# XiYe20/NPVP

Measured on AMD Instinct MI355X. Metric: predictor train frames/sec, higher is better.
Workload: dtype f32 (two-term fp16 split of amax-scaled operands, 3 MFMAs per product, fp32 accumulate: fp32-grade; small GEMMs: three-term bf16 split)

## Files before the change

include/npvp_hip.h:

```cpp
#ifndef NPVP_HIP_H
#define NPVP_HIP_H
#include <stddef.h>
#ifdef __cplusplus
extern "C" {
#endif

typedef struct ihipStream_t* npvp_stream_t;

int npvp_version(void);
const char* npvp_last_error(void);
long long npvp_launch_count(void);
void* npvp_stream_create_low_priority(int* least, int* greatest);
int npvp_stream_destroy(void* stream);
void* npvp_event_create(void);
int npvp_event_record(void* event, void* stream);
float npvp_event_elapsed_ms(void* event0, void* event1);
int npvp_event_destroy(void* event);

long long npvp_graph_node_counts(void* graph, long long* counts, long long* memset_bytes, int max_memsets);

long long npvp_gemm_workspace_bytes(int M, int N, int K);
int npvp_gemm_kernel_id(int a_kc, int b_kc, int M, int N, int K, int precision, int has_planes);
int npvp_gemm_route(int a_kc, int b_kc, int M, int N, int K, int precision, int has_planes, int plain_epilogue, int* out4);
int npvp_gemm_f32(int a_kc, int b_kc, int M, int N, int K, const float* A, long long lda, const float* B, long long ldb,
                  float* C, long long ldc, const float* bias, int act, const float* aux_in, float* aux_out,
                  const float* residual, long long ldr, float drop_p, int drop_mode, int drop_g1, int drop_g2,
                  const unsigned long long* seed, unsigned int salt, float alpha, int precision, float* colsum_a,
                  const void* b_pre, int accumulate, float* rowstats, const float* a_amax, const float* b_amax,
                  float* c_amax, unsigned int* range_flag, float adrop_p, int adrop_g1, int adrop_g2, unsigned int adrop_salt,
                  void* workspace, long long ws_bytes, npvp_stream_t stream);
int npvp_gemm_f32_skip(int a_kc, int b_kc, int M, int N, int K, const float* A, long long lda, const float* B, long long ldb,
                       float* C, long long ldc, const float* bias, int act, const float* aux_in, float* aux_out,
                       const float* residual, long long ldr, float drop_p, int drop_mode, int drop_g1, int drop_g2,
                       const unsigned long long* seed, unsigned int salt, float alpha, int precision, float* colsum_a,
                       const void* b_pre, int accumulate, float* rowstats, const float* a_amax, const float* b_amax,
                       float* c_amax, unsigned int* range_flag, float adrop_p, int adrop_g1, int adrop_g2, unsigned int adrop_salt,
                       float skip_p, int skip_g1, int skip_g2, unsigned int skip_salt, void* workspace, long long ws_bytes,
                       npvp_stream_t stream);
int npvp_frame_stats_finalize(const float* part, int parts_per_frame, float values_per_part, float* mean, float* rstd,
                              int frames, float eps, npvp_stream_t stream);
int npvp_split_weight(const float* w, long long ld, int N, int K, void* F, void* D, npvp_stream_t stream);
int npvp_split_weights_batched(const void* desc, int count, npvp_stream_t stream);
int npvp_amax(const float* x, long long rows, long long cols, long long ld, float* slot, npvp_stream_t stream);

typedef struct npvp_reduce_job {
  const float* ws; float* out; long long ldc; int M, N, splits, accum; float alpha; int blocks; const float* cs_part; float* cs_out;
} npvp_reduce_job_t;
int npvp_wgrad_f16_chainable(int M, int N, int K);
long long npvp_wgrad_f16_chain_workspace_bytes(int M, int N, int K);
int npvp_wgrad_f16_chained(int M, int N, int K, const float* dy, long long lda, const float* x, long long ldb, float* dw,
                           long long ldc, float* db, int accumulate, const float* a_amax, const float* b_amax,
                           unsigned int* range_flag, float adrop_p, int adrop_g1, int adrop_g2, unsigned int adrop_salt,
                           const unsigned long long* seed, const void* prev_job, void* my_job, void* workspace,
                           long long ws_bytes, npvp_stream_t stream);
int npvp_splitk_reduce_job(const void* job, npvp_stream_t stream);
int npvp_splitk_reduce_multi(const void* jobs, int n, npvp_stream_t stream);
int npvp_linear_bwd_f16_takes(int R, int N, int K);
int npvp_linear_bwd_f16(int R, int N, int K, const float* dy, long long ldy, const float* dy_amax, const void* w_planes_d,
                        const float* w_amax, float* dx, long long ldx, int act, const float* aux_in, const float* residual,
                        long long ldr, float drop_p, int drop_mode, int drop_g1, int drop_g2, unsigned int drop_salt, float* dx_amax,
                        const float* x, long long ldxx, const float* x_amax, float* dw, long long ldw, float* db,
                        unsigned int* range_flag, float adrop_p, int adrop_g1, int adrop_g2, unsigned int adrop_salt,
                        const unsigned long long* seed, const void* prev_job, void* my_job, void* workspace, long long ws_bytes,
                        npvp_stream_t stream);
int npvp_linear_bwd_f16_skip(int R, int N, int K, const float* dy, long long ldy, const float* dy_amax, const void* w_planes_d,
                             const float* w_amax, float* dx, long long ldx, int act, const float* aux_in, const float* residual,
                             long long ldr, float drop_p, int drop_mode, int drop_g1, int drop_g2, unsigned int drop_salt,
                             float* dx_amax, const float* x, long long ldxx, const float* x_amax, float* dw, long long ldw, float* db,
                             unsigned int* range_flag, float adrop_p, int adrop_g1, int adrop_g2, unsigned int adrop_salt,
                             float skip_p, int skip_g1, int skip_g2, unsigned int skip_salt, const unsigned long long* seed,
                             const void* prev_job, void* my_job, void* workspace, long long ws_bytes, npvp_stream_t stream);
int npvp_split_weight_f16(const float* w, long long ld, int N, int K, void* F, void* D, float* amax_slot, npvp_stream_t stream);
int npvp_split_weights_f16(const void* desc, int count, void* amax_table, long long amax_bytes, npvp_stream_t stream);

int npvp_layernorm_fwd(const float* x, const float* w, const float* b, float* y, float* mean, float* rstd, long long rows,
                       int C, float eps, int relu, float* y_amax, npvp_stream_t stream);
long long npvp_layernorm_bwd_workspace_bytes(long long rows, int C);
int npvp_layernorm_bwd(const float* dy, const float* x, const float* w, const float* b, const float* mean,
                       const float* rstd, float* dx, float* dw, float* db, long long rows, int C, int relu,
                       const float* dres ,
                       int accumulate , float* dx_amax,
                       void* workspace, long long ws_bytes, npvp_stream_t stream);
int npvp_layernorm_bwd_reduce(const void* workspace, float* dw, float* db, long long rows, int C, int accumulate,
                              npvp_stream_t stream);

int npvp_layernorm_bwd_reduce_job(const void* workspace, float* dw, float* db, long long rows, int C, int accumulate, void* job);
int npvp_frameln_act_bwd_reduce_job(const void* workspace, float* dw, float* db, int frames, int per_frame, int accumulate, void* job);
int npvp_mlpdw_mid_bwd_reduce_job(const void* workspace, float* gw, float* gb, int frames, int Ch, void* job);
int npvp_sum_rows_multi(const void* jobs, int n, npvp_stream_t stream);

int npvp_layernorm_nchw_fwd(const float* x, const float* w, const float* b, float* out_nchw, float* mean, float* rstd, int frames,
                            int P, int C, float eps, int relu, npvp_stream_t stream);

int npvp_frame_stats(const float* x, const float* add, float* mean, float* rstd, int frames, int T, int per_frame,
                     float eps, npvp_stream_t stream);
int npvp_posfuse_fwd(const float* x, const float* add, const float* beta, const float* gamma, float* y, float* mean,
                     float* rstd, int N, int T, int per_frame, float eps, float* y_amax, npvp_stream_t stream);
int npvp_ln_posfuse_fwd(const float* x, const float* lw, const float* lb, float ln_eps, float* y1, float* ln_mean, float* ln_rstd,
                        const float* add, const float* beta, const float* gamma, float* fused, float* pf_mean, float* pf_rstd,
                        int N, int T, int P, int C, float pf_eps, float* y1_amax, float* fused_amax, npvp_stream_t stream);
int npvp_posfuse_bwd_fused(int N, int T, int per_frame);
int npvp_posfuse_bwd(const float* dy, const float* x, const float* add, const float* gamma, const float* mean,
                     const float* rstd, float* du, float* dyxh, float* dbeta, float* dgamma, int N, int T, int per_frame,
                     int accumulate, void* workspace, long long ws_bytes , npvp_stream_t stream);

int npvp_posfuse_instance_fwd(const float* x, const float* add, const float* beta, const float* gamma, float* y, float* mean,
                              float* rstd, int N, int T, int P, int C, float eps, float* y_amax, npvp_stream_t stream);
int npvp_posfuse_instance_bwd(const float* dy, const float* x, const float* add, const float* gamma, const float* mean,
                              const float* rstd, float* du, float* dyxh, int N, int T, int P, int C, npvp_stream_t stream);

int npvp_frameln_act_fwd(const float* h, const float* mean, const float* rstd, const float* w, const float* b,
                         const float* res, float* out, int frames, int per_frame, float drop_p, unsigned int salt,
                         float dp_p, unsigned int dp_salt, int frames_per_sample, const unsigned long long* seed,
                         float* out_amax, npvp_stream_t stream);
long long npvp_frameln_act_bwd_workspace_bytes(int frames, int per_frame);
int npvp_frameln_act_bwd(const float* dout, const float* h, const float* mean, const float* rstd, const float* w,
                         const float* b, float* dh, float* dw, float* db, int frames, int per_frame, float drop_p,
                         unsigned int salt, float dp_p, unsigned int dp_salt, int frames_per_sample,
                         const unsigned long long* seed, int accumulate ,
                         float* dh_amax, void* workspace, long long ws_bytes, npvp_stream_t stream);
int npvp_frameln_act_bwd_reduce(const void* workspace, float* dw, float* db, int frames, int per_frame, int accumulate,
                                npvp_stream_t stream);
int npvp_dwconv3x3(const float* a, const float* wt, const float* bias, float* out, int frames, int H, int W, int Ch,
                   int flip, npvp_stream_t stream);
int npvp_dwconv3x3_stats(const float* a, const float* wt, const float* bias, float* out, float* mean, float* rstd, int frames,
                         int H, int W, int Ch, float eps, void* workspace, long long ws_bytes, npvp_stream_t stream);
int npvp_mlpdw_mid_fwd(const float* h1, const float* mean1, const float* rstd1, const float* w1n, const float* b1n,
                       const float* wt, const float* bias, float* h2, float* mean2, float* rstd2, int frames, int H, int W,
                       int Ch, float eps, void* workspace, long long ws_bytes, npvp_stream_t stream);
int npvp_mlpdw_mid_fwd_parts(const float* h1, const float* part1, int J1, float nb1, float* mean1, float* rstd1, const float* w1n,
                             const float* b1n, const float* wt, const float* bias, float* h2, float* part2, int frames, int H,
                             int W, int Ch, float eps, npvp_stream_t stream);
int npvp_frameln_act_fwd_parts(const float* h, const float* part, int J, float nb, float eps, float* mean, float* rstd,
                               const float* w, const float* b, const float* res, float* out, int frames, int per_frame,
                               float drop_p, unsigned int salt, float dp_p, unsigned int dp_salt, int frames_per_sample,
                               const unsigned long long* seed, float* out_amax, npvp_stream_t stream);
long long npvp_mlpdw_mid_bwd_workspace_bytes(int frames, int Ch);
int npvp_mlpdw_mid_bwd(const float* dh2, const float* h1, const float* mean1, const float* rstd1, const float* w1n,
                       const float* b1n, const float* wt, float* da1, float* dwt_db, float* psum, int frames, int H, int W,
                       int Ch, int accumulate, void* workspace, long long ws_bytes, npvp_stream_t stream);
int npvp_mlpdw_mid_bwd_reduce(const void* workspace, float* dwt_db, int frames, int Ch, int accumulate, npvp_stream_t stream);
int npvp_mlpdw_mid_bwd_reduce_into(const void* workspace, float* gw, float* gb, int frames, int Ch, npvp_stream_t stream);
int npvp_mlpdw_mid_bwd_n2(const float* da2, const float* h2, const float* mean2, const float* rstd2, const float* w2n,
                          const float* b2n, const float* psum2, int nparts2, float drop_p, unsigned int salt,
                          const unsigned long long* seed, const float* h1, const float* mean1, const float* rstd1,
                          const float* w1n, const float* b1n, const float* wt, float* da1, float* dwt_db, float* psum, int frames,
                          int H, int W, int Ch, int accumulate, void* workspace, long long ws_bytes, npvp_stream_t stream);
int npvp_frameln_act_bwd_pgrad(const float* dout, const float* h, const float* mean, const float* rstd, const float* w,
                               const float* b, float* psum, float* dw, float* db, int frames, int per_frame, float drop_p,
                               unsigned int salt, float dp_p, unsigned int dp_salt, int frames_per_sample,
                               const unsigned long long* seed, int accumulate, void* workspace, long long ws_bytes,
                               npvp_stream_t stream);
int npvp_frameln_act_bwd_apply(const float* dout, const float* h, const float* mean, const float* rstd, const float* w,
                               const float* b, const float* psum, int nparts, float* dh, float* dw, float* db, int frames,
                               int per_frame, int accumulate, float* dh_amax, void* workspace, long long ws_bytes,
                               npvp_stream_t stream);
int npvp_mlpdw_mid_fwd_parts_skip(const float* h1, const float* part1, int J1, float nb1, float* mean1, float* rstd1,
                                  const float* w1n, const float* b1n, const float* wt, const float* bias, float* h2, float* part2,
                                  int frames, int H, int W, int Ch, float eps, float skip_p, unsigned int skip_salt, int skip_fps,
                                  const unsigned long long* seed, npvp_stream_t stream);
int npvp_frameln_act_fwd_parts_skip(const float* h, const float* part, int J, float nb, float eps, float* mean, float* rstd,
                                    const float* w, const float* b, const float* res, float* out, int frames, int per_frame,
                                    float drop_p, unsigned int salt, float dp_p, unsigned int dp_salt, int frames_per_sample,
                                    const unsigned long long* seed, float* out_amax, float skip_p, unsigned int skip_salt,
                                    int skip_fps, npvp_stream_t stream);
int npvp_frameln_act_bwd_apply_skip(const float* dout, const float* h, const float* mean, const float* rstd, const float* w,
                                    const float* b, const float* psum, int nparts, float* dh, float* dw, float* db, int frames,
                                    int per_frame, int accumulate, float* dh_amax, void* workspace, long long ws_bytes,
                                    float skip_p, unsigned int skip_salt, int skip_fps, const unsigned long long* seed,
                                    npvp_stream_t stream);

int npvp_im2col3x3(const float* in, float* out, int frames, int H, int W, int C, int col2im, npvp_stream_t stream);
long long npvp_dwconv3x3_wgrad_workspace_bytes(int frames, int Ch);
int npvp_dwconv3x3_wgrad(const float* a, const float* dout, float* dwt_db, int frames, int H, int W, int Ch,
                         void* workspace, long long ws_bytes, npvp_stream_t stream);

int npvp_attn_fwd(const float* q, long long ld_q, const float* k, long long ld_k, const float* v, long long ld_v, float* o,
                  long long ld_o, int mode, int dim0, int P, int W, int ws, int Tq, int Tk, int heads, int head_dim,
                  int mask_mode, float drop_p, const unsigned long long* seed, unsigned int salt, float* o_amax,
                  npvp_stream_t stream);
int npvp_attn_bwd(const float* q, long long ld_q, const float* k, long long ld_k, const float* v, long long ld_v,
                  const float* go, long long ld_o, float* dq, long long ld_dq, float* dk, long long ld_dk, float* dv,
                  long long ld_dv, int mode, int dim0, int P, int W, int ws, int Tq, int Tk, int heads, int head_dim,
                  int mask_mode, float drop_p, const unsigned long long* seed, unsigned int salt, float* dq_amax,
                  float* dk_amax , float* dv_amax,
                  npvp_stream_t stream);
int npvp_attn_long_fwd(const float* q, long long ld_q, const float* k, long long ld_k, const float* v, long long ld_v, float* o,
                       long long ld_o, int mode, int dim0, int P, int W, int ws, int Tq, int Tk, int heads, int head_dim,
                       int mask_mode, float drop_p, const unsigned long long* seed, unsigned int salt, float* o_amax,
                       npvp_stream_t stream);
long long npvp_attn_long_bwd_workspace_bytes(int mode, int dim0, int P, int W, int ws, int Tq, int Tk, int heads);
int npvp_attn_long_bwd(const float* q, long long ld_q, const float* k, long long ld_k, const float* v, long long ld_v,
                       const float* go, long long ld_o, float* dq, long long ld_dq, float* dk, long long ld_dk, float* dv,
                       long long ld_dv, int mode, int dim0, int P, int W, int ws, int Tq, int Tk, int heads, int head_dim,
                       int mask_mode, float drop_p, const unsigned long long* seed, unsigned int salt, float* dq_amax,
                       float* dk_amax , float* dv_amax, void* workspace, long long ws_bytes,
                       npvp_stream_t stream);

int npvp_reparam_samples(const float* mu, const float* logvar, float* z, float* eps_out, long long numel, int S,
                         long long sample_base, const unsigned long long* seed, unsigned int salt, npvp_stream_t stream);
int npvp_attn_samples_fwd(const float* q, long long ld_q, const float* k, long long ld_k, const float* v, long long ld_v, float* o,
                          long long ld_o, int S, int N, int P, int Tq, int Tk, int heads, int head_dim, int sample_chunk,
                          float* o_amax, npvp_stream_t stream);

int npvp_drop_apply(const float* x, float* out, long long rows, int ncols, float p, int mode, int g1, int g2,
                    const unsigned long long* seed, unsigned int salt, float* out_amax, npvp_stream_t stream);
int npvp_transpose(const float* in, float* out, int batch, int R, int C, npvp_stream_t stream);
int npvp_dwtb_accumulate(const float* dwtb, float* gw, float* gb, int C, npvp_stream_t stream);
int npvp_dwtb_build(const float* w, const float* b, float* wtb, int C, npvp_stream_t stream);
int npvp_reduce_mid(const float* in, float* out, int A, int B, long long Cc, float scale, int accumulate, npvp_stream_t stream);
int npvp_broadcast_mid(const float* in, float* out, int A, int B, long long Cc, float scale, npvp_stream_t stream);
int npvp_grid_center_pad(const float* src, long long ld_src, float* dst, long long ld_dst, int F, int H, int W, int Hp, int Wp, int top,
                         int left, int C, long long rows_out, float* dst_amax, npvp_stream_t stream);
int npvp_grid_center_cut(const float* src, long long ld_src, const float* addend, long long ld_add, float* dst, long long ld_dst, int F,
                         int H, int W, int Hp, int Wp, int top, int left, int C, float* dst_amax, npvp_stream_t stream);

long long npvp_colsum_workspace_bytes(long long rows, int N);
int npvp_colsum(const float* x, long long rows, int N, long long ld, float* out, int accumulate ,
                void* workspace, long long ws_bytes, npvp_stream_t stream);

int npvp_l1_mean(const float* a, const float* b, long long n, float lam, float* out, void* workspace, long long ws_bytes,
                 npvp_stream_t stream);
int npvp_l1_mean_bwd(const float* a, const float* b, long long n, const float* gout, float lam, float* da, npvp_stream_t stream);
int npvp_sum_all(const float* x, long long n, float* out, void* workspace, long long ws_bytes, npvp_stream_t stream);
// ... 65 lines not shown
```

npvp_amd/csrc/gemm.h:

```cpp
#pragma once
#include <type_traits>
#include "common.h"

namespace npvp {

typedef float f32x16 __attribute__((ext_vector_type(16)));
typedef __bf16 bf16x8 __attribute__((ext_vector_type(8)));
typedef __bf16 bf16x4 __attribute__((ext_vector_type(4)));

struct ReduceJob {
  const float* ws; float* out; long long ldc; int M, N, splits, accum; float alpha; int blocks; const float* cs_part; float* cs_out;
};

struct GemmParams {
  const float* A; const float* B; float* C;
  const float* bias;
  const float* residual;
  float* aux_out;
  const float* aux_in;
  float* rowstats;
  float* colsum;
  const unsigned long long* seed;
  long long lda, ldb, ldc, ldr;
  int M, N, K;
  int act;
  DropSpec drop;
  DropSpec adrop;
  DropSpec rskip;
  int tiles_m, tiles_n;
  int splits;
  float alpha;
  const void* b_pre;
  long long b_pre_plane;
  int colgroups;
  int accum;
  const float* a_amax; const float* b_amax; float* c_amax;
  unsigned int* range_flag;
  ReduceJob prev;
};

__device__ __forceinline__ void splitk_reduce_body(const ReduceJob& j, int bid, int nblocks, float& cmax) {
  const long long total4 = (long long)j.M * j.N / 4, cs4 = j.cs_out ? j.M / 4 : 0;
  for (long long i = (long long)bid * 256 + threadIdx.x; i < total4 + cs4; i += (long long)nblocks * 256) {
    if (i >= total4) {
      const long long e = (i - total4) * 4;
      float4 s = make_float4(0.f, 0.f, 0.f, 0.f);
      for (int zz = 0; zz < j.splits; ++zz) {
        const float4 v = ld4(j.cs_part + (long long)zz * j.M + e);
        s.x += v.x; s.y += v.y; s.z += v.z; s.w += v.w;
      }
      if (j.accum) { const float4 o = ld4(j.cs_out + e); s.x += o.x; s.y += o.y; s.z += o.z; s.w += o.w; }
      st4(j.cs_out + e, s);
      continue;
    }
    const long long e = i * 4;
    const int m = (int)(e / j.N), n = (int)(e - (long long)m * j.N);
    float4 s = make_float4(0.f, 0.f, 0.f, 0.f);
    for (int zz = 0; zz < j.splits; ++zz) {
      const float4 v = ld4(j.ws + (long long)zz * j.M * j.N + e);
      s.x += v.x; s.y += v.y; s.z += v.z; s.w += v.w;
    }
    s.x *= j.alpha; s.y *= j.alpha; s.z *= j.alpha; s.w *= j.alpha;
    if (j.accum) { const float4 o = ld4(j.out + (long long)m * j.ldc + n); s.x += o.x; s.y += o.y; s.z += o.z; s.w += o.w; }
    st4(j.out + (long long)m * j.ldc + n, s);
    cmax = amax4(cmax, s);
  }
}

__device__ __forceinline__ void store_colsum(const GemmParams& p, long long idx, float v) {
  p.colsum[idx] = (p.accum && p.splits == 1) ? p.colsum[idx] + v : v;
}

constexpr int EPI_LD = 36;
constexpr int EPI_FLOATS = 32 * EPI_LD;

__device__ __forceinline__ void epi_transpose(const f32x16& acc, float* scr, int lane, float4 (&v)[4]) {
  const int r = lane & 31, h = lane >> 5;
#pragma unroll
  for (int g = 0; g < 16; ++g) scr[(((g & 3) + 8 * (g >> 2)) + 4 * h) * EPI_LD + r] = acc[g];
  const int rr = lane >> 3, cq = lane & 7;
#pragma unroll
  for (int k = 0; k < 4; ++k) v[k] = *reinterpret_cast<const float4*>(scr + (rr + 8 * k) * EPI_LD + 4 * cq);
}

__device__ __forceinline__ float4 f4_mad(const float4& a, float s, const float4& b) {
  return make_float4(a.x * s + b.x, a.y * s + b.y, a.z * s + b.z, a.w * s + b.w);
}
__device__ __forceinline__ void f4_add(float4& a, const float4& b) { a.x += b.x; a.y += b.y; a.z += b.z; a.w += b.w; }

template <int I, int N, class F>
__device__ __forceinline__ void static_for(F&& f) {
  if constexpr (I < N) {
    f(std::integral_constant<int, I>{});
    static_for<I + 1, N>(f);
  }
}

__device__ __forceinline__ float4 epilogue_row_scales(const GemmParams& p, unsigned long long seed, int row0, int lane) {
  float4 sc = make_float4(1.f, 1.f, 1.f, 1.f);
  if (p.drop.thresh && p.drop.mode != 0) {
    const int r = row0 + (lane >> 3);
    sc.x = drop_spec_scale(p.drop, seed, r, 0, 1); sc.y = drop_spec_scale(p.drop, seed, r + 8, 0, 1);
    sc.z = drop_spec_scale(p.drop, seed, r + 16, 0, 1); sc.w = drop_spec_scale(p.drop, seed, r + 24, 0, 1);
  }
  return sc;
}

template <bool CHECK>
__device__ __forceinline__ void epilogue_rows(const GemmParams& p, float4 (&v)[4], int row0, int col0, int lane, int z,
                                              unsigned long long seed, float& cmax, float4 rowsc, float alpha) {
  const int rb = row0 + (lane >> 3), col = col0 + 4 * (lane & 7);
  if (CHECK && col >= p.N) return;
#define NPVP_ROW(k) (rb + 8 * (k))
#define NPVP_INB(k) (!CHECK || NPVP_ROW(k) < p.M)
  float* cp = p.C + (p.splits > 1 ? (long long)z * p.M * p.ldc : 0ll) + col;
  const long long ld = p.ldc;
  if (p.splits > 1) {
#pragma unroll
    for (int k = 0; k < 4; ++k) if (NPVP_INB(k)) st4(cp + NPVP_ROW(k) * ld, v[k]);
    return;
  }
  const float4 bv = p.bias ? ld4(p.bias + col) : make_float4(0.f, 0.f, 0.f, 0.f);
#pragma unroll
  for (int k = 0; k < 4; ++k) v[k] = f4_mad(v[k], alpha, bv);
  if (p.aux_out) {
#pragma unroll
    for (int k = 0; k < 4; ++k) if (NPVP_INB(k)) st4(p.aux_out + NPVP_ROW(k) * ld + col, v[k]);
  }
  if (p.act == 1) {
#pragma unroll
    for (int k = 0; k < 4; ++k) v[k] = make_float4(gelu_f(v[k].x), gelu_f(v[k].y), gelu_f(v[k].z), gelu_f(v[k].w));
  } else if (p.act == 2) {
#pragma unroll
    for (int k = 0; k < 4; ++k) v[k] = make_float4(fmaxf(v[k].x, 0.f), fmaxf(v[k].y, 0.f), fmaxf(v[k].z, 0.f), fmaxf(v[k].w, 0.f));
  } else if (p.act == 3 || p.act == 4) {
    float4 u[4];
#pragma unroll
    for (int k = 0; k < 4; ++k) u[k] = NPVP_INB(k) ? ld4(p.aux_in + NPVP_ROW(k) * ld + col) : make_float4(0.f, 0.f, 0.f, 0.f);
    if (p.act == 3) {
#pragma unroll
      for (int k = 0; k < 4; ++k) {
        v[k].x *= gelu_grad_f(u[k].x); v[k].y *= gelu_grad_f(u[k].y); v[k].z *= gelu_grad_f(u[k].z); v[k].w *= gelu_grad_f(u[k].w);
      }
    } else {
#pragma unroll
      for (int k = 0; k < 4; ++k) {
        v[k].x = u[k].x > 0.f ? v[k].x : 0.f; v[k].y = u[k].y > 0.f ? v[k].y : 0.f;
        v[k].z = u[k].z > 0.f ? v[k].z : 0.f; v[k].w = u[k].w > 0.f ? v[k].w : 0.f;
      }
    }
  }
  if (p.drop.thresh) {
    if (p.drop.mode == 0) {
#pragma unroll
      for (int k = 0; k < 4; ++k) {
        const unsigned long long key = (unsigned long long)NPVP_ROW(k) * (unsigned long long)p.N + (unsigned long long)col;
        v[k].x *= drop_scale(seed, p.drop.salt, key + 0, p.drop.thresh, p.drop.inv_keep);
        v[k].y *= drop_scale(seed, p.drop.salt, key + 1, p.drop.thresh, p.drop.inv_keep);
        v[k].z *= drop_scale(seed, p.drop.salt, key + 2, p.drop.thresh, p.drop.inv_keep);
        v[k].w *= drop_scale(seed, p.drop.salt, key + 3, p.drop.thresh, p.drop.inv_keep);
      }
    } else {
#pragma unroll
      for (int k = 0; k < 4; ++k) {
        const float f = k == 0 ? rowsc.x : k == 1 ? rowsc.y : k == 2 ? rowsc.z : rowsc.w;
        v[k].x *= f; v[k].y *= f; v[k].z *= f; v[k].w *= f;
      }
    }
  }
  if (p.residual) {
#pragma unroll
    for (int k = 0; k < 4; ++k) if (NPVP_INB(k)) f4_add(v[k], ld4(p.residual + NPVP_ROW(k) * p.ldr + col));
  }
  if (p.accum) {
#pragma unroll
    for (int k = 0; k < 4; ++k) if (NPVP_INB(k)) f4_add(v[k], ld4(cp + NPVP_ROW(k) * ld));
  }
#pragma unroll
  for (int k = 0; k < 4; ++k) if (NPVP_INB(k)) st4(cp + NPVP_ROW(k) * ld, v[k]);
  if (p.c_amax) {
#pragma unroll
    for (int k = 0; k < 4; ++k) if (NPVP_INB(k)) cmax = amax4(cmax, v[k]);
  }
#undef NPVP_INB
#undef NPVP_ROW
}

__device__ __forceinline__ void epilogue_rows_bias(const GemmParams& p, float4 (&v)[4], int row0, int col0, int lane, float& cmax, float alpha) {
  const int col = col0 + 4 * (lane & 7);
  float* cp = p.C + (long long)(row0 + (lane >> 3)) * p.ldc + col;
  const long long ld8 = 8 * p.ldc;
  const float4 bv = p.bias ? ld4(p.bias + col) : make_float4(0.f, 0.f, 0.f, 0.f);
#pragma unroll
  for (int k = 0; k < 4; ++k) {
    const float4 x = f4_mad(v[k], alpha, bv);
    st4(cp + k * ld8, x);
    if (p.c_amax) cmax = amax4(cmax, x);
  }
}

__device__ __forceinline__ void epilogue_tile(const GemmParams& p, const f32x16& acc, int row0, int col0, int lane, float* scr, int z,
                                              unsigned long long seed, float& cmax, float4 rowsc, float alpha) {
  if (row0 >= p.M || col0 >= p.N) return;
  float4 v[4];
  epi_transpose(acc, scr, lane, v);
  const bool inside = row0 + 32 <= p.M && col0 + 32 <= p.N;
  const bool simple = p.splits == 1 && !p.aux_out && p.act == 0 && !p.drop.thresh && !p.residual && !p.accum;
  if (simple && inside) epilogue_rows_bias(p, v, row0, col0, lane, cmax, alpha);
  else if (inside) epilogue_rows<false>(p, v, row0, col0, lane, z, seed, cmax, rowsc, alpha);
  else epilogue_rows<true>(p, v, row0, col0, lane, z, seed, cmax, rowsc, alpha);
}

__device__ __forceinline__ void epilogue_rowstats_block(const GemmParams& p, const f32x16& a00, const f32x16& a01,
                                                        const f32x16& a10, const f32x16& a11, int row0, int col0, int lane,
                                                        float* scr, float& cmax, float alpha) {
  if (row0 >= p.M || col0 >= p.N) return;
  const int r = lane & 31;
  float shift = 0.f, s1 = 0.f, s2 = 0.f;
#pragma unroll
  for (int tm = 0; tm < 2; ++tm) {
#pragma unroll
    for (int tn = 0; tn < 2; ++tn) {
      const f32x16& acc = tm == 0 ? (tn == 0 ? a00 : a01) : (tn == 0 ? a10 : a11);
      const float bv = p.bias ? p.bias[col0 + tn * 32 + r] : 0.f;
#pragma unroll
      for (int g = 0; g < 16; ++g) {
        const float v = acc[g] * alpha + bv;
        if (tm == 0 && tn == 0 && g == 0) shift = v;
        const float d = v - shift;
        s1 += d; s2 += d * d;
      }
    }
  }
  __builtin_amdgcn_sched_barrier(0);
#pragma unroll
  for (int tm = 0; tm < 2; ++tm) {
#pragma unroll
    for (int tn = 0; tn < 2; ++tn) {
      const f32x16& acc = tm == 0 ? (tn == 0 ? a00 : a01) : (tn == 0 ? a10 : a11);
      float4 v[4];
      epi_transpose(acc, scr, lane, v);
      epilogue_rows_bias(p, v, row0 + tm * 32, col0 + tn * 32, lane, cmax, alpha);
      __builtin_amdgcn_sched_barrier(0);
    }
  }
  const float n = 64.f, m1 = s1 / n, mean_l = shift + m1, m2_l = s2 - s1 * m1;
  const float mean_w = wave_sum(mean_l) * (1.f / 64.f);
  const float dl = mean_l - mean_w;
  const float m2_w = wave_sum(m2_l + n * dl * dl);
  if ((lane & 63) == 0) {
    const long long frame = row0 >> 6;
    const int cb = col0 >> 6, ncb = p.N >> 6;
    p.rowstats[(frame * ncb + cb) * 2] = mean_w;
    p.rowstats[(frame * ncb + cb) * 2 + 1] = m2_w;
  }
}

__device__ __forceinline__ void tile_of_block_unsplit(const GemmParams& p, const int nwg, const int bid, int& tile_m, int& tile_n) {
  const int xcd = bid & 7, loc = bid >> 3;
  if (p.colgroups > 1) {
    const int G = p.colgroups, tn_g = p.tiles_n / G, tm_g = p.tiles_m / (8 / G);
    const int lm = loc / tn_g;
    tile_m = (xcd / G) * tm_g + lm;
    tile_n = (xcd % G) * tn_g + (loc - lm * tn_g);
  } else {
    const int q = nwg >> 3, rr = nwg & 7;
    const int nid = (xcd < rr ? xcd * (q + 1) : rr * (q + 1) + (xcd - rr) * q) + loc;
    tile_m = nid / p.tiles_n;
    tile_n = nid - tile_m * p.tiles_n;
  }
}

__device__ __forceinline__ void tile_of_block_unsplit(const GemmParams& p, int& tile_m, int& tile_n) {
  tile_of_block_unsplit(p, (int)gridDim.x, (int)blockIdx.x, tile_m, tile_n);
}

inline int pick_colgroups(long long b_bytes, int tiles_m, int tiles_n) {
  for (int G = 1; G <= 8; G *= 2) {
    if (b_bytes / G > (2ll << 20)) continue;
    if (G > 1 && (tiles_n % G == 0) && (tiles_m % (8 / G) == 0) && ((tiles_m * tiles_n) % 8 == 0)) return G;
    break;
  }
  return 1;
}

inline long long splitk_workspace_bytes(int splits, int M, int N) {
  return ((long long)splits * M * N + (long long)splits * M) * 4;
}

inline void aim_at_workspace(GemmParams& p, int K, int splits, void* workspace, bool colsum) {
  p.K = K / splits; p.C = (float*)workspace; p.ldc = p.N;
  p.colsum = colsum ? (float*)workspace + (long long)splits * p.M * p.N : nullptr;
}

inline int wgrad_splits(int M, int N, int K, int min_rows) {
  if ((K & 15) || M < 64 || N < 128 || K < min_rows) return 0;
  const int tiles = ((M + 127) / 128) * ((N + 255) / 256);
  int s = (512 + tiles - 1) / tiles;
  const int maxs = K / 256;
  if (s > maxs) s = maxs;
  if (s > 64) s = 64;
  if (s >= 8) s &= ~7;
  while (s > 1 && (K % (s * 16)) != 0) --s;
  return s < 1 ? 1 : s;
}
inline int wide_wgrad_splits(int M, int N, int K) { return wgrad_splits(M, N, K, 32768); }
inline int f16_wgrad_splits(int M, int N, int K) { return wgrad_splits(M, N, K, 1024); }

inline bool adrop_args_ok(float p, int g1, int g2, const unsigned long long* seed, bool rows16) {
  return p >= 0.f && p < 0.5f && (p == 0.f || (seed && g1 > 0 && g2 > 0 && (!rows16 || g1 % 16 == 0)));
}

int wide_variant(int M, int N, int K);
void launch_gemm_wide(GemmParams& p, int variant, hipStream_t stream);
void launch_gemm_wgrad_wide(GemmParams& p, hipStream_t stream);
int gemm_f16_variant(int M, int N, int K);
void launch_gemm_f16(GemmParams& p, int variant, hipStream_t stream);
void launch_gemm_wgrad_f16(GemmParams& p, hipStream_t stream);

}
```

npvp_amd/csrc/gemm.hip:

```cpp
#include "gemm.h"
#include "partials.h"
#include <type_traits>

namespace npvp {

constexpr int BM = 128, BN = 128, BK = 32, GEMM_THREADS = 256;

template <bool KC> struct Stager;

template <> struct Stager<true> {
  static constexpr int LD = 129;
  float4 r[4];
  __device__ __forceinline__ void load(const float* src, long long ld, int row0, int nrows, int k0) {
    const int t = threadIdx.x;
    const int kc = (t & 7) * 4;
#pragma unroll
    for (int i = 0; i < 4; ++i) {
      const int row = row0 + (t >> 3) + 32 * i;
      r[i] = (row < nrows) ? ld4(src + (long long)row * ld + k0 + kc) : make_float4(0.f, 0.f, 0.f, 0.f);
    }
  }
  __device__ __forceinline__ void store(float* s) const {
    const int t = threadIdx.x;
    const int kc = (t & 7) * 4;
// ... 343 lines not shown
  if constexpr (ROWSTATS) {
    float cmax = 0.f;
    epilogue_rowstats_block(p, acc00, acc01, acc10, acc11, m0 + wm * 64, n0 + wn * 64, lane, scr0 + wave * EPI_FLOATS, cmax, p.alpha);
    amax_slot_commit(p.c_amax, cmax, 0u);
  } else gemm_epilogue(p, acc00, acc01, acc10, acc11, m0, n0, wm, wn, scr0, z);
}

struct SplitDesc { const float* w; long long ld; long long N; long long K; __bf16* F; __bf16* D; };
__global__ void split_weights_batched_kernel(const SplitDesc* __restrict__ desc) {
  const SplitDesc d = desc[blockIdx.y];
  const int N = (int)d.N, K = (int)d.K;
  const long long slots = (long long)N * K / 8, plane = (long long)N * K;
  for (long long i = (long long)blockIdx.x * blockDim.x + threadIdx.x; i < 2 * slots; i += (long long)gridDim.x * blockDim.x) {
    float v[8];
    __bf16* out;
    if (i < slots) {
      const int n = (int)(i % N), kb = (int)(i / N);
      const float4 a = ld4(d.w + (long long)n * d.ld + kb * 8), b = ld4(d.w + (long long)n * d.ld + kb * 8 + 4);
      v[0] = a.x; v[1] = a.y; v[2] = a.z; v[3] = a.w; v[4] = b.x; v[5] = b.y; v[6] = b.z; v[7] = b.w;
      out = d.F + i * 8;
    } else {
      const long long j = i - slots;
      const int k = (int)(j % K), nb = (int)(j / K);
#pragma unroll
      for (int e = 0; e < 8; ++e) v[e] = d.w[(long long)(nb * 8 + e) * d.ld + k];
      out = d.D + j * 8;
    }
#pragma unroll
    for (int s_ = 0; s_ < 3; ++s_) {
      bf16x8 q;
#pragma unroll
      for (int e = 0; e < 8; ++e) { q[e] = (__bf16)v[e]; v[e] -= (float)q[e]; }
      *reinterpret_cast<bf16x8*>(out + (long long)s_ * plane) = q;
    }
  }
}

__global__ void splitk_reduce_kernel(const float* __restrict__ ws, float* __restrict__ out, int M, int N,
                                     long long ldc, int splits, float alpha, int accum, const float* __restrict__ cs_part,
                                     float* __restrict__ cs_out, float* c_amax) {
  __shared__ float ared[4];
  const unsigned int cpeek = amax_peek_block(c_amax);
  float cmax = 0.f;
  const ReduceJob j = {ws, out, ldc, M, N, splits, accum, alpha, 0, cs_part, cs_out};
  splitk_reduce_body(j, blockIdx.x, gridDim.x, cmax);
  amax_slot_commit_block(c_amax, cmax, ared, cpeek);
}

static int pick_splits(int M, int N, int K) {
  const int tiles = ((M + BM - 1) / BM) * ((N + BN - 1) / BN);
  if (tiles >= 256 || K < 2048) return 1;
  int s = (512 + tiles - 1) / tiles;
  const int maxs = K / (BK * 8);
  if (s > maxs) s = maxs;
  if (s > 64) s = 64;
  while (s > 1 && (K % (s * BK)) != 0) --s;
  return s < 1 ? 1 : s;
}

}

using namespace npvp;

extern "C" long long npvp_gemm_workspace_bytes(int M, int N, int K) {
  const int s = pick_splits(M, N, K), sw = wide_wgrad_splits(M, N, K), sh = f16_wgrad_splits(M, N, K);
  const int m = (s > sw ? s : sw) > sh ? (s > sw ? s : sw) : sh;
  return m > 1 ? splitk_workspace_bytes(m, M, N) : 0;
}

extern "C" int npvp_split_weight(const float* w, long long ld, int N, int K, void* F, void* D, hipStream_t stream) {
  NPVP_CHECK_ARG(N > 0 && K > 0 && N % 8 == 0 && K % 8 == 0 && ld % 4 == 0, "split_weight: N, K must be multiples of 8");
  NPVP_CHECK_ARG(((uintptr_t)w % 16) == 0, "split_weight: w must be 16-byte aligned");
  const long long total = (long long)N * K / 8;
  int blocks = (int)((total + 255) / 256); if (blocks > 4096) blocks = 4096;
  if (F) { NPVP_LAUNCH(split_weight_fwd_kernel, dim3(blocks), dim3(256), 0, stream, w, ld, N, K, (__bf16*)F); NPVP_CHECK_LAUNCH(); }
  if (D) { NPVP_LAUNCH(split_weight_dgrad_kernel, dim3(blocks), dim3(256), 0, stream, w, ld, N, K, (__bf16*)D); NPVP_CHECK_LAUNCH(); }
  return NPVP_OK;
}

extern "C" int npvp_split_weights_batched(const void* desc, int count, hipStream_t stream) {
  NPVP_CHECK_ARG(desc && count > 0, "split_weights_batched: empty table");
  NPVP_LAUNCH(split_weights_batched_kernel, dim3(128, count), dim3(256), 0, stream, (const SplitDesc*)desc);
  NPVP_CHECK_LAUNCH();
  return NPVP_OK;
}

struct GemmFacts {
  int a_kc, b_kc, M, N, K, precision;
  bool planes;
  bool plain;
  bool amax;
  bool rowstats;
  long long ws_bytes;
};
struct GemmPlan {
  int id, variant, splits, steps;
  bool planes;
};

static GemmPlan plan_gemm(const GemmFacts& f) {
  const int M = f.M, N = f.N, K = f.K;
  const bool want_h = f.precision == 6;
  const int precision = want_h ? 4 : f.precision;
  int s128 = pick_splits(M, N, K);
  if (s128 > 1 && (!f.plain || f.ws_bytes < npvp_gemm_workspace_bytes(M, N, K))) s128 = 1;
  const bool planes_ok = f.planes && f.a_kc && K % 16 == 0 && N % 8 == 0;
  const bool wgrad = !f.a_kc && !f.b_kc && f.plain && !f.rowstats;
  auto fits = [&](int s) { return s == 1 || (s > 1 && f.ws_bytes >= splitk_workspace_bytes(s, M, N)); };
  GemmPlan pl = {precision == 0 ? 0 : 1, 0, s128, 0, false};
  int v = 0, s = 0;
  if (want_h && planes_ok && f.amax && (v = gemm_f16_variant(M, N, K)) != 0) {
    pl.id = v == 1 ? 5 : 7; pl.variant = v; pl.splits = 1; pl.planes = true;
  } else if (want_h && wgrad && f.amax && fits(s = f16_wgrad_splits(M, N, K))) {
    pl.id = 6; pl.splits = s;
  } else if (!want_h && precision == 4 && planes_ok && s128 == 1 && (v = wide_variant(M, N, K)) != 0) {
    pl.id = v == 1 ? 2 : 4; pl.variant = v; pl.planes = true;
  } else if (precision == 4 && wgrad && fits(s = wide_wgrad_splits(M, N, K))) {
    pl.id = 3; pl.splits = s;
  } else {
    pl.planes = !want_h && precision == 4 && planes_ok && s128 == 1 && !f.rowstats;
  }
  pl.steps = K / pl.splits / (precision == 0 ? BK : 16);
  return pl;
}

static GemmPlan plan_query(int a_kc, int b_kc, int M, int N, int K, int precision, int has_planes, bool plain) {
  return plan_gemm(GemmFacts{a_kc, b_kc, M, N, K, precision, has_planes != 0, plain, true, false, npvp_gemm_workspace_bytes(M, N, K)});
}

extern "C" int npvp_gemm_kernel_id(int a_kc, int b_kc, int M, int N, int K, int precision, int has_planes) {
  return plan_query(a_kc, b_kc, M, N, K, precision, has_planes, true).id;
}

extern "C" int npvp_gemm_route(int a_kc, int b_kc, int M, int N, int K, int precision, int has_planes, int plain_epilogue, int* out4) {
  NPVP_CHECK_ARG(out4 && M > 0 && N > 0 && K > 0, "gemm_route: empty problem or no result array");
  NPVP_CHECK_ARG(precision == 0 || precision == 4 || precision == 5 || precision == 6, "gemm_route: precision must be 0, 4, 5 or 6");
  NPVP_CHECK_ARG(K % BK == 0 && M % 4 == 0 && N % 4 == 0 && !(a_kc == 0 && b_kc == 1), "gemm_route: not a problem npvp_gemm_f32 accepts");
  const GemmPlan r = plan_query(a_kc, b_kc, M, N, K, precision, has_planes, plain_epilogue != 0);
  out4[0] = r.id; out4[1] = r.variant; out4[2] = r.splits; out4[3] = r.steps;
  return NPVP_OK;
}

static int finish_splitk(const GemmParams& p, float* C, long long ldc, float* colsum_a, hipStream_t stream) {
  const long long total4 = (long long)p.M * p.N / 4;
  int blocks = (int)((total4 + 255) / 256); if (blocks > 2048) blocks = 2048;
  const bool cs_here = colsum_a && ((uintptr_t)colsum_a % 16) == 0;
  NPVP_LAUNCH(splitk_reduce_kernel, dim3(blocks), dim3(256), 0, stream, (const float*)p.C, C, p.M, p.N, ldc, p.splits, p.alpha,
              p.accum, cs_here ? (const float*)p.colsum : nullptr, cs_here ? colsum_a : nullptr, p.c_amax);
  NPVP_CHECK_LAUNCH();
  if (!colsum_a || cs_here) return NPVP_OK;
  return finish_partials(make_partials(p.colsum, 0, p.splits, p.splits, p.M, colsum_a, p.accum).job, 0, stream, "gemm: column-sum reduce launch failed");
}

extern "C" int npvp_gemm_f32_skip(int a_kc, int b_kc, int M, int N, int K, const float* A, long long lda, const float* B,
                                  long long ldb, float* C, long long ldc, const float* bias, int act, const float* aux_in,
                                  float* aux_out, const float* residual, long long ldr, float drop_p, int drop_mode,
                                  int drop_g1, int drop_g2, const unsigned long long* seed, unsigned int salt, float alpha,
                                  int precision, float* colsum_a, const void* b_pre, int accumulate, float* rowstats,
                                  const float* a_amax, const float* b_amax, float* c_amax, unsigned int* range_flag,
                                  float adrop_p, int adrop_g1, int adrop_g2, unsigned int adrop_salt,
                                  float skip_p, int skip_g1, int skip_g2, unsigned int skip_salt,
                                  void* workspace, long long ws_bytes, hipStream_t stream) {
  NPVP_CHECK_ARG(skip_p >= 0.f && skip_p < 1.f && (skip_p == 0.f || (seed && skip_g1 > 0 && skip_g2 > 0 && a_kc)),
                 "gemm: the row skip needs a device seed, row groups and a row-major A");
  NPVP_CHECK_ARG(M > 0 && N > 0 && K > 0, "gemm: empty problem");
  NPVP_CHECK_ARG(precision == 0 || precision == 4 || precision == 5 || precision == 6,
                 "gemm: precision must be 0 (exact fp32-input MFMA), 4 (three-term bf16 split, 6 MFMAs per product: "
                 "fp32-grade), 5 (two-term bf16 split, 3 MFMAs per product, ~2^-16) or 6 (two-term fp16 split with amax-scaled "
                 "operands, 3 MFMAs per product: fp32-grade; shapes it does not take run as 4)");
  const bool want_h = precision == 6;
  NPVP_CHECK_ARG(K % BK == 0, "gemm: K must be a multiple of 32");
  NPVP_CHECK_ARG(M % 4 == 0 && N % 4 == 0, "gemm: M and N must be multiples of 4");
  NPVP_CHECK_ARG(((uintptr_t)A % 16) == 0 && ((uintptr_t)B % 16) == 0 && ((uintptr_t)C % 16) == 0, "gemm: pointers must be 16-byte aligned");
  NPVP_CHECK_ARG(lda % 4 == 0 && ldb % 4 == 0, "gemm: lda/ldb must be multiples of 4 floats");
  NPVP_CHECK_ARG(ldc % 4 == 0 && (!residual || (ldr % 4 == 0 && ((uintptr_t)residual % 16) == 0)) && (!bias || ((uintptr_t)bias % 16) == 0) &&
                 (!aux_in || ((uintptr_t)aux_in % 16) == 0) && (!aux_out || ((uintptr_t)aux_out % 16) == 0),
                 "gemm: ldc / ldr must be multiples of 4 floats and bias / aux / residual 16-byte aligned (float4 epilogue)");
  NPVP_CHECK_ARG(!(a_kc == 0 && b_kc == 1), "gemm: (a_kc=0,b_kc=1) is not used by the path");
  NPVP_CHECK_ARG((act != 3 && act != 4) || aux_in, "gemm: act 3/4 need aux_in");
  NPVP_CHECK_ARG(drop_p >= 0.f && drop_p < 1.f, "gemm: dropout p out of range");
  NPVP_CHECK_ARG(drop_p == 0.f || seed, "gemm: dropout needs a device seed");
  NPVP_CHECK_ARG(!colsum_a || a_kc == 0, "gemm: colsum_a is the column sum of a [K][M] operand (a_kc = 0)");
  NPVP_CHECK_ARG(!b_pre || ((uintptr_t)b_pre % 16) == 0, "gemm: b_pre must be 16-byte aligned");

  NPVP_CHECK_ARG(adrop_p >= 0.f && adrop_p < 0.5f, "gemm: adrop_p must be in [0, 0.5) (the masked operand must stay inside its amax scale)");
  NPVP_CHECK_ARG(adrop_p == 0.f || (want_h && adrop_args_ok(adrop_p, adrop_g1, adrop_g2, seed, !a_kc)),
                 "gemm: adrop needs precision 6, a device seed and (for a weight gradient) groups of a multiple of 16 rows");
  NPVP_CHECK_ARG(!rowstats || ((precision == 4 || want_h) && a_kc && b_kc && M % 64 == 0 && N % 128 == 0 && act == 0 && !aux_out && !residual &&
                               drop_p == 0.f && !accumulate),
                 "gemm: rowstats needs the default (bf16x6) forward layout, M % 64 == 0, N % 128 == 0 and a bias-only epilogue");

  const bool plain = !bias && act == 0 && !aux_out && !residual && drop_p == 0.f;
  const GemmPlan plan = plan_gemm(GemmFacts{a_kc, b_kc, M, N, K, precision, b_pre != nullptr, plain,
                                            a_amax && b_amax, rowstats != nullptr, workspace ? ws_bytes : 0});
  NPVP_CHECK_ARG(adrop_p == 0.f || plan.id >= 5, "gemm: adrop was requested but this shape does not run on the fp16 kernels (npvp_gemm_kernel_id tells)");

  GemmParams p;
  p.A = A; p.B = B; p.bias = bias; p.residual = residual; p.aux_out = aux_out; p.aux_in = aux_in;
  p.seed = seed; p.lda = lda; p.ldb = ldb; p.ldr = ldr; p.M = M; p.N = N; p.act = act;
  p.drop = make_drop_spec(drop_p, salt, drop_mode, drop_g1, drop_g2);
  p.adrop = make_drop_spec(adrop_p, adrop_salt, 1, adrop_g1, adrop_g2);
  p.rskip = make_drop_spec(skip_p, skip_salt, 1, skip_g1, skip_g2);
  p.alpha = alpha;
  p.rowstats = rowstats;
  p.a_amax = a_amax; p.b_amax = b_amax; p.c_amax = c_amax; p.range_flag = range_flag;
  p.prev = ReduceJob{};
  p.accum = accumulate ? 1 : 0;
  p.b_pre = plan.planes ? b_pre : nullptr;
  p.b_pre_plane = (long long)N * K;
  p.splits = plan.splits;
  if (plan.splits > 1) aim_at_workspace(p, K, plan.splits, workspace, colsum_a != nullptr);
  else { p.K = K; p.C = C; p.ldc = ldc; p.colsum = colsum_a; }
  p.tiles_m = (M + BM - 1) / BM; p.tiles_n = (N + BN - 1) / BN;
  p.colgroups = (plan.id <= 1 && plan.splits == 1) ? pick_colgroups((long long)N * K * 4, p.tiles_m, p.tiles_n) : 1;

  const dim3 grid(p.tiles_m * p.tiles_n, plan.splits), block(GEMM_THREADS);
  switch (plan.id) {
    case 5: case 7: launch_gemm_f16(p, plan.variant, stream); break;
    case 6: launch_gemm_wgrad_f16(p, stream); break;
    case 2: case 4: launch_gemm_wide(p, plan.variant, stream); break;
    case 3: launch_gemm_wgrad_wide(p, stream); break;
    case 0:
      if (a_kc && b_kc) NPVP_LAUNCH((gemm_f32_kernel<true, true>), grid, block, 0, stream, p);
      else if (a_kc) NPVP_LAUNCH((gemm_f32_kernel<true, false>), grid, block, 0, stream, p);
      else NPVP_LAUNCH((gemm_f32_kernel<false, false>), grid, block, 0, stream, p);
      break;
    default:
      if (precision == 5) {
        if (a_kc && b_kc) NPVP_LAUNCH((gemm_split_db_kernel<2, true, true, false>), grid, block, 0, stream, p);
        else if (a_kc) NPVP_LAUNCH((gemm_split_db_kernel<2, true, false, false>), grid, block, 0, stream, p);
        else NPVP_LAUNCH((gemm_split_db_kernel<2, false, false, false>), grid, block, 0, stream, p);
      } else if (rowstats) NPVP_LAUNCH((gemm_split_db_kernel<3, true, true, false, true>), grid, block, 0, stream, p);
      else if (plan.planes) NPVP_LAUNCH((gemm_split_db_kernel<3, true, true, true>), grid, block, 0, stream, p);
      else if (a_kc && b_kc) NPVP_LAUNCH((gemm_split_db_kernel<3, true, true, false>), grid, block, 0, stream, p);
      else if (a_kc) NPVP_LAUNCH((gemm_split_db_kernel<3, true, false, false>), grid, block, 0, stream, p);
      else NPVP_LAUNCH((gemm_split_db_kernel<3, false, false, false>), grid, block, 0, stream, p);
  }
  NPVP_CHECK_LAUNCH();
  return plan.splits > 1 ? finish_splitk(p, C, ldc, colsum_a, stream) : NPVP_OK;
}

extern "C" int npvp_gemm_f32(int a_kc, int b_kc, int M, int N, int K, const float* A, long long lda, const float* B,
                             long long ldb, float* C, long long ldc, const float* bias, int act, const float* aux_in,
                             float* aux_out, const float* residual, long long ldr, float drop_p, int drop_mode,
                             int drop_g1, int drop_g2, const unsigned long long* seed, unsigned int salt, float alpha,
                             int precision, float* colsum_a, const void* b_pre, int accumulate, float* rowstats,
                             const float* a_amax, const float* b_amax, float* c_amax, unsigned int* range_flag,
                             float adrop_p, int adrop_g1, int adrop_g2, unsigned int adrop_salt,
                             void* workspace, long long ws_bytes, hipStream_t stream) {
  return npvp_gemm_f32_skip(a_kc, b_kc, M, N, K, A, lda, B, ldb, C, ldc, bias, act, aux_in, aux_out, residual, ldr, drop_p, drop_mode,
                            drop_g1, drop_g2, seed, salt, alpha, precision, colsum_a, b_pre, accumulate, rowstats, a_amax, b_amax, c_amax,
                            range_flag, adrop_p, adrop_g1, adrop_g2, adrop_salt, 0.f, 1, 1, 0u, workspace, ws_bytes, stream);
}
```

npvp_amd/csrc/gemm_f16.hip:

```cpp
#include "gemm.h"
#include <cstdio>
#include <cstdlib>

namespace npvp {

typedef _Float16 f16x8 __attribute__((ext_vector_type(8)));
typedef _Float16 f16x4 __attribute__((ext_vector_type(4)));
typedef __attribute__((address_space(1))) const void* gptr_t;
typedef __attribute__((address_space(3))) void* lptr_t;
typedef float f32x4 __attribute__((ext_vector_type(4)));

__device__ __forceinline__ void split_f16_scaled(const f32x4 v, const float s, f16x4& hi, f16x4& lo) {
  unsigned int h01, h23, l01, l23;
  asm("v_fma_mixlo_f16 %0, %1, %2, 0" : "=v"(h01) : "v"(v[0]), "v"(s));
  asm("v_fma_mixlo_f16 %0, %1, %2, 0" : "=v"(h23) : "v"(v[2]), "v"(s));
  asm("v_fma_mixhi_f16 %0, %1, %2, 0" : "+v"(h01) : "v"(v[1]), "v"(s));
  asm("v_fma_mixhi_f16 %0, %1, %2, 0" : "+v"(h23) : "v"(v[3]), "v"(s));
  asm("v_fma_mixlo_f16 %0, %1, %2, -%3 op_sel_hi:[0,0,1]" : "=v"(l01) : "v"(v[0]), "v"(s), "v"(h01));
  asm("v_fma_mixlo_f16 %0, %1, %2, -%3 op_sel_hi:[0,0,1]" : "=v"(l23) : "v"(v[2]), "v"(s), "v"(h23));
  asm("v_fma_mixhi_f16 %0, %1, %2, -%3 op_sel:[0,0,1] op_sel_hi:[0,0,1]" : "+v"(l01) : "v"(v[1]), "v"(s), "v"(h01));
  asm("v_fma_mixhi_f16 %0, %1, %2, -%3 op_sel:[0,0,1] op_sel_hi:[0,0,1]" : "+v"(l23) : "v"(v[3]), "v"(s), "v"(h23));
  typedef unsigned int u32x2 __attribute__((ext_vector_type(2)));
  const u32x2 hp = {h01, h23}, lp = {l01, l23};
  hi = __builtin_bit_cast(f16x4, hp);
// ... 137 lines not shown
    const char* st_ = lds + (CUR) * STAGE;                                                                 \
    char* nx_ = lds + (NXT) * STAGE;                                                                       \
    NPVP_H_BLOAD(lds + (B2) * STAGE, (KT) + (NST - 1))                                                     \
    f16x8 fb_[2][TN];                                                                                      \
    _Pragma("unroll") for (int s_ = 0; s_ < 2; ++s_)                                                       \
      _Pragma("unroll") for (int j_ = 0; j_ < TN; ++j_)                                                    \
        fb_[s_][j_] = *reinterpret_cast<const f16x8*>(st_ + fb_off + s_ * B_PLANE + j_ * 512);             \
    _Pragma("unroll") for (int i_ = 0; i_ < TM; ++i_) {                                                    \
      f16x8 fa_[2];                                                                                        \
      _Pragma("unroll") for (int s_ = 0; s_ < 2; ++s_)                                                     \
        fa_[s_] = *reinterpret_cast<const f16x8*>(st_ + fa_off + s_ * A_PLANE + i_ * 512);                 \
      if (i_ == 0) { NPVP_H_ASTORE(nx_, R0, 0) if constexpr (APASS == 2) NPVP_H_ASTORE(nx_, R1, (BM / 2) * 16) } \
      if (i_ == TM - 1) { NPVP_H_ALOAD(R0, R1, (KT) + 3) }                                                 \
                                                                                 \
      _Pragma("unroll") for (int j_ = 0; j_ < TN; ++j_) acc[i_][j_] = __builtin_amdgcn_mfma_f32_32x32x16_f16(fa_[1], fb_[0][j_], (FIRST) ? zero16 : acc[i_][j_], 0, 0, 0); \
      _Pragma("unroll") for (int j_ = 0; j_ < TN; ++j_) acc[i_][j_] = __builtin_amdgcn_mfma_f32_32x32x16_f16(fa_[0], fb_[1][j_], acc[i_][j_], 0, 0, 0); \
      _Pragma("unroll") for (int j_ = 0; j_ < TN; ++j_) acc[i_][j_] = __builtin_amdgcn_mfma_f32_32x32x16_f16(fa_[0], fb_[0][j_], acc[i_][j_], 0, 0, 0); \
    }                                                                                                      \
    __builtin_amdgcn_sched_barrier(0);        \
    if constexpr (NST == 3) { NPVP_H_WAIT_BUT_THIS_STEP("+v"(RN0), "+v"(RN1)) }                            \
    else { NPVP_H_WAIT_BUT_NEWEST("+v"(RN0), "+v"(RN1)) }                                                  \
    __builtin_amdgcn_s_barrier();                                                                          \
  }

  if constexpr (NST == 2) {
  NPVP_H_STEP_(0, 0, 1, 1, ea0, ea1, eb0, eb1, true)
  int kt = 1;
  for (; kt + 1 < nk; kt += 2) {
    NPVP_H_STEP(kt, 1, 0, eb0, eb1, ea0, ea1)
    NPVP_H_STEP(kt + 1, 0, 1, ea0, ea1, eb0, eb1)
  }
  if (kt < nk) NPVP_H_STEP(kt, 1, 0, eb0, eb1, ea0, ea1)
  } else {
  NPVP_H_STEP_(0, 0, 1, 2, ea0, ea1, eb0, eb1, true)
  int kt = 1;
  for (; kt + 5 < nk; kt += 6) {
    NPVP_H_STEP3(kt, 1, 2, 0, eb0, eb1, ea0, ea1)
    NPVP_H_STEP3(kt + 1, 2, 0, 1, ea0, ea1, eb0, eb1)
    NPVP_H_STEP3(kt + 2, 0, 1, 2, eb0, eb1, ea0, ea1)
    NPVP_H_STEP3(kt + 3, 1, 2, 0, ea0, ea1, eb0, eb1)
    NPVP_H_STEP3(kt + 4, 2, 0, 1, eb0, eb1, ea0, ea1)
    NPVP_H_STEP3(kt + 5, 0, 1, 2, ea0, ea1, eb0, eb1)
  }
  if (kt < nk) NPVP_H_STEP3(kt, 1, 2, 0, eb0, eb1, ea0, ea1)
  if (kt + 1 < nk) NPVP_H_STEP3(kt + 1, 2, 0, 1, ea0, ea1, eb0, eb1)
  if (kt + 2 < nk) NPVP_H_STEP3(kt + 2, 0, 1, 2, eb0, eb1, ea0, ea1)
  if (kt + 3 < nk) NPVP_H_STEP3(kt + 3, 1, 2, 0, ea0, ea1, eb0, eb1)
  if (kt + 4 < nk) NPVP_H_STEP3(kt + 4, 2, 0, 1, eb0, eb1, ea0, ea1)
  }
  asm volatile("s_waitcnt vmcnt(0)" : "+v"(ea0), "+v"(ea1), "+v"(eb0), "+v"(eb1) :: "memory");
  if constexpr (NST == 3) __builtin_amdgcn_s_barrier();
  };
  if (skipped) {
#pragma unroll
    for (int i = 0; i < TM; ++i)
#pragma unroll
      for (int j = 0; j < TN; ++j) acc[i][j] = zero16;
  } else {
  run_tile();
    rm0 = fmaxf(rm0, __shfl_xor(rm0, 1)); rm0 = fmaxf(rm0, __shfl_xor(rm0, 2));
    rm1 = fmaxf(rm1, __shfl_xor(rm1, 1)); rm1 = fmaxf(rm1, __shfl_xor(rm1, 2));
    const int et = (int)((__float_as_uint(sa) >> 23) & 0xffu);
    const int e0 = (int)((__float_as_uint(rm0) >> 23) & 0xffu), e1 = (int)((__float_as_uint(rm1) >> 23) & 0xffu);
    const int d0 = 268 - et - e0, d1 = 268 - et - e1;
    const bool ok0 = e0 >= 16 && e0 != 255 && d0 > 0 && d0 <= 120, ok1 = e1 >= 16 && e1 != 255 && d1 > 0 && d1 <= 120;
    if (block_any<NW>((ok0 && d0 >= 18) || (ok1 && d1 >= 18), guard_flags, wave)) {
      const float g0 = sa0 * pow2_recip(sa), g1 = sa1 * pow2_recip(sa);
      rf0 = ok0 ? __uint_as_float((unsigned int)(127 - d0) << 23) : 1.f;
      rf1 = ok1 ? __uint_as_float((unsigned int)(127 - d1) << 23) : 1.f;
      sa0 = (ok0 ? amax_scale(rm0) : sa) * g0;
      sa1 = (ok1 ? amax_scale(rm1) : sa) * g1;
      rescued = true;
      run_tile();
    }
  }
#undef NPVP_H_STEP
#undef NPVP_H_STEP3
#undef NPVP_H_WAIT_BUT_THIS_STEP
#undef NPVP_H_STEP_
#undef NPVP_H_BLOAD
#undef NPVP_H_ASTORE
#undef NPVP_H_ALOAD
#undef NPVP_H_WAIT_BUT_NEWEST

  const float ia = pow2_recip(sa), ib = pow2_recip(amax_scale(amax_slot_read(p.b_amax)));
  float alpha = p.alpha;
  {
    const float f = ia * ib, af = p.alpha * f, mag = fabsf(af);
    const bool fold = f >= 1.17549435e-38f && f <= 3.0e38f && ((mag >= 1.17549435e-38f && mag <= 3.0e38f) || p.alpha == 0.f);
    if (fold) alpha = af;
    else {
#pragma unroll
      for (int i = 0; i < TM; ++i)
#pragma unroll
        for (int j = 0; j < TN; ++j)
#pragma unroll
          for (int g = 0; g < 16; ++g) acc[i][j][g] = acc[i][j][g] * ia * ib;
    }
  }

  const int row_base = m0 + wm * TM * 32, col_base = n0 + wn * TN * 32;
  float cmax = 0.f;
  float* scr = reinterpret_cast<float*>(lds) + 4 + wave * EPI_FLOATS;
  if (rescued) {
    float* rowfac = reinterpret_cast<float*>(lds) + 4 + NW * EPI_FLOATS;
    if (quad == 0) { rowfac[rl] = rf0; if (APASS == 2) rowfac[rl + BM / 2] = rf1; }
    __syncthreads();
#pragma unroll
    for (int i = 0; i < TM; ++i)
#pragma unroll
      for (int g = 0; g < 16; ++g) {
        const float f = rowfac[wm * TM * 32 + i * 32 + (g & 3) + 8 * (g >> 2) + 4 * h];
#pragma unroll
        for (int j = 0; j < TN; ++j) acc[i][j][g] *= f;
      }
  }
  if constexpr (ROWSTATS) {
    static_assert(!ROWSTATS || (TN % 2 == 0 && TM % 2 == 0), "frame statistics ride on 64 x 64 accumulator blocks");
#pragma unroll
    for (int i = 0; i < TM; i += 2)
#pragma unroll
      for (int j = 0; j < TN; j += 2)
        epilogue_rowstats_block(p, acc[i][j], acc[i][j + 1], acc[i + 1][j], acc[i + 1][j + 1], row_base + i * 32, col_base + j * 32, lane, scr, cmax, alpha);
  } else {
    const unsigned long long seed = (p.seed && p.drop.thresh) ? *p.seed : 0ull;
    static_for<0, TM>([&](auto i) __attribute__((always_inline)) {
      const float4 rowsc = epilogue_row_scales(p, seed, row_base + i * 32, lane);
      static_for<0, TN>([&](auto j) __attribute__((always_inline)) {
        epilogue_tile(p, acc[i][j], row_base + i * 32, col_base + j * 32, lane, scr, 0, seed, cmax, rowsc, alpha);
      });
    });
  }
  amax_slot_commit_block(p.c_amax, cmax, reinterpret_cast<float*>(lds), cpeek);
}

template <int TM, int TN, int WM, int WN, bool ROWSTATS, int MINB = 2, int NST = 2>
__global__ __launch_bounds__(64 * WM * WN, MINB) void gemm_f16_kernel(GemmParams p) {
  __shared__ __attribute__((aligned(16))) char lds[gemm_f16_lds_bytes<TM, TN, WM, WN, NST>()];
  gemm_f16_body<TM, TN, WM, WN, ROWSTATS, NST>(p, lds, blockIdx.x, gridDim.x);
}

typedef short s16x4 __attribute__((ext_vector_type(4)));

__device__ __forceinline__ f16x8 lds_read_tr_pair_h(const char* a, int second_off) {
  const s16x4 lo = __builtin_amdgcn_ds_read_tr16_b64_v4i16((__attribute__((address_space(3))) s16x4*)(a));
  const s16x4 hi = __builtin_amdgcn_ds_read_tr16_b64_v4i16((__attribute__((address_space(3))) s16x4*)(a + second_off));
  typedef short s16x8 __attribute__((ext_vector_type(8)));
  const s16x8 v = __builtin_shufflevector(lo, hi, 0, 1, 2, 3, 4, 5, 6, 7);
  return __builtin_bit_cast(f16x8, v);
}

constexpr int GEMM_WGRAD_F16_LDS_BYTES = 2 * (2 * 16 * 128 * 2 + 2 * 16 * 256 * 2);

template <int TM, int TN, int WM, int WN>
__device__ __forceinline__ void gemm_wgrad_f16_body(const GemmParams& p, char* lds, const int bx, const int by, const int gx) {
  constexpr int NW = WM * WN, THREADS = 64 * NW;
  constexpr int BM = WM * TM * 32, BN = WN * TN * 32;
  static_assert(THREADS == 256 && BM == 128 && BN == 256, "staging maps are written for 256 threads on a 128 x 256 tile");
  constexpr int ROWA = BM * 2, ROWB = BN * 2;
  constexpr int A_PLANE = 16 * ROWA, B_PLANE = 16 * ROWB, A_BYTES = 2 * A_PLANE, B_BYTES = 2 * B_PLANE;
  constexpr int STAGE = A_BYTES + B_BYTES;
  static_assert(2 * STAGE == GEMM_WGRAD_F16_LDS_BYTES, "lds size formula");

  if (by >= p.splits) {
    float cm = 0.f;
    splitk_reduce_body(p.prev, (by - p.splits) * gx + bx, p.prev.blocks, cm);
    return;
  }
  int z, tl;
  {
    const int tiles = gx;
    if (p.splits > 1 && (p.splits & 7) == 0) {
      const int lin = bx + tiles * by, xcd = lin & 7, slot = lin >> 3;
      const int g = slot / tiles;
      tl = slot - g * tiles; z = g * 8 + xcd;
    } else { z = by; tl = bx; }
  }
  const int tile_m = tl / p.tiles_n, tile_n = tl - tile_m * p.tiles_n;
  const int m0 = tile_m * BM, n0 = tile_n * BN;
  const float* A = p.A + (long long)z * p.K * p.lda;
  const float* B = p.B + (long long)z * p.K * p.ldb;
  const int t = threadIdx.x, lane = t & 63, wave = __builtin_amdgcn_readfirstlane(t >> 6);
  const int wm = wave / WN, wn = wave % WN, r = lane & 31, h = lane >> 5;
  const int nk = p.K >> 4;
  const float sa = amax_scale(amax_slot_read(p.a_amax)), sb = amax_scale(amax_slot_read(p.b_amax));

  f32x16 acc[TM][TN];
#pragma unroll
  for (int i = 0; i < TM; ++i)
#pragma unroll
    for (int j = 0; j < TN; ++j)
#pragma unroll
      for (int g = 0; g < 16; ++g) acc[i][j][g] = 0.f;

  const int ka = t >> 5, cqa = t & 31, kb = t >> 6, cqb = t & 63;
  const char* a_base = reinterpret_cast<const char*>(A);
  const char* b_base = reinterpret_cast<const char*>(B);
  const unsigned int a_voff = (unsigned int)(((long long)ka * p.lda + min(m0 + 4 * cqa, p.M - 4)) * 4);
  const unsigned int b_voff = (unsigned int)(((long long)kb * p.ldb + min(n0 + 4 * cqb, p.N - 4)) * 4);
  const long long a_row8 = 32 * p.lda, b_row4 = 16 * p.ldb, a_step = 64 * p.lda, b_step = 64 * p.ldb;
  const int a_dst = ka * ROWA + ((8 * cqa) ^ ((ka & 3) << 6));
  const int b_dst = A_BYTES + kb * ROWB + ((8 * cqb) ^ ((kb & 3) << 6));
  const int q = (lane >> 2) & 3, pp = lane & 3, cg = 16 * ((lane >> 4) & 1) + 4 * pp;
  int fa[TM], fb[TN];
#pragma unroll
  for (int i = 0; i < TM; ++i) fa[i] = (8 * h + q) * ROWA + (((wm * TM * 32 + i * 32 + cg) * 2) ^ (q << 6));
#pragma unroll
  for (int j = 0; j < TN; ++j) fb[j] = A_BYTES + (8 * h + q) * ROWB + (((wn * TN * 32 + j * 32 + cg) * 2) ^ (q << 6));

  const bool want_cs = p.colsum && tile_n == 0;
  f32x4 cs = {0.f, 0.f, 0.f, 0.f};
  f32x4 cm4 = {0.f, 0.f, 0.f, 0.f};
  f32x4 ra[2], rb[4];
#define NPVP_G_LOAD(KT)                                                                                     \
  { const int kt_ = min((KT), nk - 1);                                                                      \
    const char* pa_ = a_base + (long long)kt_ * a_step; const char* pb_ = b_base + (long long)kt_ * b_step;  \
    asm volatile("global_load_dwordx4 %0, %1, %2" : "=v"(ra[0]) : "v"(a_voff), "s"(pa_) : "memory");        \
    asm volatile("global_load_dwordx4 %0, %1, %2" : "=v"(ra[1]) : "v"(a_voff), "s"(pa_ + a_row8) : "memory"); \
    _Pragma("unroll") for (int i_ = 0; i_ < 4; ++i_)                                                        \
      asm volatile("global_load_dwordx4 %0, %1, %2" : "=v"(rb[i_]) : "v"(b_voff), "s"(pb_ + i_ * b_row4) : "memory"); }
#define NPVP_G_WAIT(N, ...) asm volatile("s_waitcnt vmcnt(" #N ")" : __VA_ARGS__ :: "memory");
#define NPVP_G_STORE(DST, V, SC, PLANE)                                                                     \
  { f16x4 hi_, lo_; split_f16_scaled((V), (SC), hi_, lo_);                                                  \
    *reinterpret_cast<f16x4*>(DST) = hi_; *reinterpret_cast<f16x4*>((DST) + (PLANE)) = lo_; }
  const unsigned long long aseed = p.adrop.thresh ? *p.seed : 0ull;
  const long long arow0 = (long long)z * p.K;
  float am_ = 1.f;
#define NPVP_G_AMASK(KT) { if (p.adrop.thresh) am_ = drop_spec_scale(p.adrop, aseed, arow0 + 16ll * min((KT), nk - 1), 0, 1); }
#define NPVP_G_STORE_A(ST) { const float sam_ = sa * am_;                                                                        \
    if (p.range_flag) cm4 = __builtin_elementwise_max(cm4, __builtin_elementwise_max(__builtin_elementwise_abs(ra[0]), __builtin_elementwise_abs(ra[1]))); \
    NPVP_G_STORE((ST) + a_dst, ra[0], sam_, A_PLANE) NPVP_G_STORE((ST) + a_dst + 8 * ROWA, ra[1], sam_, A_PLANE) }
#define NPVP_G_STORE_B(ST, I) NPVP_G_STORE((ST) + b_dst + (I) * 4 * ROWB, rb[I], sb, B_PLANE)

  NPVP_G_LOAD(0)
  NPVP_G_AMASK(0)
  NPVP_G_WAIT(0, "+v"(ra[0]), "+v"(ra[1]), "+v"(rb[0]), "+v"(rb[1]), "+v"(rb[2]), "+v"(rb[3]))
  if (want_cs) cs += (ra[0] + ra[1]) * am_;
  NPVP_G_STORE_A(lds)
  NPVP_G_STORE_B(lds, 0) NPVP_G_STORE_B(lds, 1) NPVP_G_STORE_B(lds, 2) NPVP_G_STORE_B(lds, 3)
  NPVP_G_LOAD(1)
  __syncthreads();

#define NPVP_G_STEP(KT, CUR, NXT)                                                                            \
  {                                                                                                          \
    const char* st_ = lds + (CUR) * STAGE;                                                                   \
    char* nx_ = lds + (NXT) * STAGE;                                                                         \
    NPVP_G_WAIT(3, "+v"(ra[0]), "+v"(ra[1]), "+v"(rb[0]))                                                    \
    NPVP_G_AMASK((KT) + 1)                                                         \
    if (want_cs && (KT) + 1 < nk) { asm volatile("" ::: "memory"); cs += (ra[0] + ra[1]) * am_; }   \
    f16x8 fa_[TM][2];                                                                                        \
    _Pragma("unroll") for (int i_ = 0; i_ < TM; ++i_)                                                        \
      _Pragma("unroll") for (int s_ = 0; s_ < 2; ++s_) fa_[i_][s_] = lds_read_tr_pair_h(st_ + fa[i_] + s_ * A_PLANE, 4 * ROWA); \
    _Pragma("unroll") for (int j_ = 0; j_ < TN; ++j_) {                                                      \
      f16x8 fb_[2];                                                                                          \
      _Pragma("unroll") for (int s_ = 0; s_ < 2; ++s_) fb_[s_] = lds_read_tr_pair_h(st_ + fb[j_] + s_ * B_PLANE, 4 * ROWB); \
      if (j_ == 0) { NPVP_G_STORE_A(nx_) NPVP_G_STORE_B(nx_, 0) }                                            \
      if (j_ == 1) { NPVP_G_WAIT(1, "+v"(rb[1]), "+v"(rb[2])) NPVP_G_STORE_B(nx_, 1) NPVP_G_STORE_B(nx_, 2) } \
      if (j_ == 2) { NPVP_G_WAIT(0, "+v"(rb[3])) NPVP_G_STORE_B(nx_, 3) NPVP_G_LOAD((KT) + 2) __builtin_amdgcn_sched_barrier(0); } \
      _Pragma("unroll") for (int i_ = 0; i_ < TM; ++i_) acc[i_][j_] = __builtin_amdgcn_mfma_f32_32x32x16_f16(fa_[i_][1], fb_[0], acc[i_][j_], 0, 0, 0); \
      _Pragma("unroll") for (int i_ = 0; i_ < TM; ++i_) acc[i_][j_] = __builtin_amdgcn_mfma_f32_32x32x16_f16(fa_[i_][0], fb_[1], acc[i_][j_], 0, 0, 0); \
      _Pragma("unroll") for (int i_ = 0; i_ < TM; ++i_) acc[i_][j_] = __builtin_amdgcn_mfma_f32_32x32x16_f16(fa_[i_][0], fb_[0], acc[i_][j_], 0, 0, 0); \
    }                                                                                                        \
     \
    __builtin_amdgcn_sched_barrier(0);                                                                       \
    asm volatile("s_waitcnt lgkmcnt(0)" ::: "memory");                                                       \
    __builtin_amdgcn_s_barrier();                                                                            \
  }

  int kt = 0;
  for (; kt + 1 < nk; kt += 2) {
    NPVP_G_STEP(kt, 0, 1)
    NPVP_G_STEP(kt + 1, 1, 0)
  }
  if (kt < nk) NPVP_G_STEP(kt, 0, 1)
  asm volatile("s_waitcnt vmcnt(0)" : "+v"(ra[0]), "+v"(ra[1]), "+v"(rb[0]), "+v"(rb[1]), "+v"(rb[2]), "+v"(rb[3]) :: "memory");
  if (p.range_flag) {
    float* red = reinterpret_cast<float*>(lds);
    *reinterpret_cast<f32x4*>(red + ka * BM + 4 * cqa) = cm4;
    __syncthreads();
    bool flag = false;
    if (t < BM) {
      float m = red[t];
#pragma unroll
      for (int i = 1; i < 8; ++i) m = fmaxf(m, red[i * BM + t]);
      const int et = (int)((__float_as_uint(sa) >> 23) & 0xffu), e = (int)((__float_as_uint(m) >> 23) & 0xffu);
      const int d = 268 - et - e;
      flag = e >= 16 && e != 255 && d >= 18 && m0 + t < p.M;
    }
    const bool any = __builtin_amdgcn_ballot_w64(flag) != 0ull;
    if (any && lane == 0) atomicAdd(p.range_flag, 1u);
    __syncthreads();
  }
#undef NPVP_G_STEP
#undef NPVP_G_WAIT
#undef NPVP_G_STORE_B
#undef NPVP_G_STORE_A
#undef NPVP_G_AMASK
#undef NPVP_G_STORE
#undef NPVP_G_LOAD

  if (want_cs) {
    float* red = reinterpret_cast<float*>(lds);
    *reinterpret_cast<f32x4*>(red + (t >> 5) * 128 + cqa * 4) = cs;
    __syncthreads();
    if (t < 128 && m0 + t < p.M) {
      float sum = 0.f;
#pragma unroll
      for (int i = 0; i < 8; ++i) sum += red[i * 128 + t];
      store_colsum(p, (long long)z * p.M + m0 + t, sum);
    }
    __syncthreads();
  }
  float* scr = reinterpret_cast<float*>(lds) + wave * EPI_FLOATS;
  static_assert(2 * STAGE >= NW * EPI_FLOATS * 4, "scratch");
  const float ia = pow2_recip(sa), ib = pow2_recip(sb);
#pragma unroll
  for (int i = 0; i < TM; ++i)
#pragma unroll
    for (int j = 0; j < TN; ++j)
#pragma unroll
      for (int g = 0; g < 16; ++g) acc[i][j][g] = acc[i][j][g] * ia * ib;
  const unsigned long long seed = 0ull;
  const int row_base = m0 + wm * TM * 32, col_base = n0 + wn * TN * 32;
  float cmax = 0.f;
  const float4 no_rowsc = make_float4(1.f, 1.f, 1.f, 1.f);
  static_for<0, TM>([&](auto i) __attribute__((always_inline)) {
    static_for<0, TN>([&](auto j) __attribute__((always_inline)) {
      epilogue_tile(p, acc[i][j], row_base + i * 32, col_base + j * 32, lane, scr, z, seed, cmax, no_rowsc, p.alpha);
    });
  });
}

template <int TM, int TN, int WM, int WN>
__global__ __launch_bounds__(64 * WM * WN, (WM * WN) / 2) void gemm_wgrad_f16_kernel(GemmParams p) {
  __shared__ __attribute__((aligned(16))) char lds[GEMM_WGRAD_F16_LDS_BYTES];
  gemm_wgrad_f16_body<TM, TN, WM, WN>(p, lds, blockIdx.x, blockIdx.y, gridDim.x);
}

struct GemmGroup { GemmParams p[2]; int first[3]; int count[2]; int gx; };

template <int TM, int TN>
__global__ __launch_bounds__(256, 2) void gemm_f16_group_kernel(GemmGroup g) {
  constexpr int L0 = gemm_f16_lds_bytes<TM, TN, 2, 2, 3>();
  __shared__ __attribute__((aligned(16))) char lds[L0 > GEMM_WGRAD_F16_LDS_BYTES ? L0 : GEMM_WGRAD_F16_LDS_BYTES];
  const int b = blockIdx.x;
  if (b < g.first[1]) {
    if (b < g.count[0]) gemm_f16_body<TM, TN, 2, 2, false, 3>(g.p[0], lds, b, g.count[0]);
  } else {
    const int lb = b - g.first[1];
    if (lb < g.count[1]) {
      const int by = lb / g.gx;
      gemm_wgrad_f16_body<2, 4, 2, 2>(g.p[1], lds, lb - by * g.gx, by, g.gx);
    }
  }
}

static int reduce_rows_for(const ReduceJob& j, int tiles) {
  if (!j.ws) return 0;
  const long long total4 = (long long)j.M * j.N / 4;
  long long want = (total4 + 255) / 256;
  if (want > 256) want = 256;
  if (want < 1) want = 1;
  return (int)((want + tiles - 1) / tiles);
}

static dim3 size_gemm_wgrad_f16(GemmParams& p) {
  p.tiles_m = (p.M + 127) / 128;
  p.tiles_n = (p.N + 255) / 256;
  const int tiles = p.tiles_m * p.tiles_n, rr = reduce_rows_for(p.prev, tiles);
  p.prev.blocks = rr * tiles;
  return dim3(tiles, p.splits + rr);
}

void launch_gemm_wgrad_f16(GemmParams& p, hipStream_t stream) {
  const dim3 grid = size_gemm_wgrad_f16(p);
  NPVP_LAUNCH((gemm_wgrad_f16_kernel<2, 4, 2, 2>), grid, dim3(256), 0, stream, p);
}

static bool deferred_wgrad_args_ok(const char* who, const float* dy, long long lda, const float* x, long long ldb, const float* dw, long long ldc, float adrop_p,
                                   int adrop_g1, int adrop_g2, const unsigned long long* seed, const void* workspace, long long ws_bytes, long long ws_need) {
  const char* what = ((((uintptr_t)dy | (uintptr_t)x | (uintptr_t)dw) & 15) || ((lda | ldb | ldc) & 3)) ? "operands must be 16-byte aligned with leading dimensions that are multiples of 4"
                     : !adrop_args_ok(adrop_p, adrop_g1, adrop_g2, seed, true) ? "adrop needs a device seed and groups of a multiple of 16 rows"
                     : (!workspace || ws_bytes < ws_need) ? "workspace too small" : nullptr;
  char msg[192];
  if (what) { snprintf(msg, sizeof(msg), "%s: %s", who, what); npvp_set_error(msg); }
  return !what;
}

static GemmParams deferred_wgrad_params(int M, int N, int K, const float* dy, long long lda, const float* x, long long ldb, const float* a_amax, const float* b_amax,
                                        unsigned int* range_flag, const DropSpec& adrop, const unsigned long long* seed, const void* prev_job, void* workspace,
                                        bool want_db, int accumulate) {
  GemmParams p = {};
  p.A = dy; p.B = x; p.lda = lda; p.ldb = ldb; p.M = M; p.N = N; p.alpha = 1.f;
  p.splits = f16_wgrad_splits(M, N, K); p.colgroups = 1; p.accum = accumulate ? 1 : 0;
  aim_at_workspace(p, K, p.splits, workspace, want_db);
  p.seed = seed; p.drop = make_drop_spec(0.f, 0u, 0, 1, 1); p.adrop = adrop;
  p.a_amax = a_amax; p.b_amax = b_amax; p.range_flag = range_flag;
  if (prev_job) p.prev = *reinterpret_cast<const ReduceJob*>(prev_job);
  return p;
}

static void leave_reduce_job(const GemmParams& p, float* dw, long long ldc, float* db, void* my_job) {
  const ReduceJob mine = {(const float*)p.C, dw, ldc, p.M, p.N, p.splits, p.accum, 1.f, 0, p.colsum, db};
  *reinterpret_cast<ReduceJob*>(my_job) = mine;
}

int gemm_f16_variant(int M, int N, int K) {
  if ((K & 15) || (N & 7) || M < 128) return 0;
  const int tw = ((M + 127) / 128) * ((N + 255) / 256);
  if (N % 128 != 0 || tw >= 512) return 1;
  if (M % 64 == 0 && ((M + 127) / 128) * (N / 128) <= 256) return 4;
  if (N % 64 == 0 && ((M + 127) / 128) * (N / 128) <= 128) return 3;
  return 2;
}

static void prep_gemm_f16(GemmParams& p, int v) {
  const int bn = v == 1 ? 256 : (v == 3 ? 64 : 128);
  p.tiles_m = v == 4 ? (p.M + 63) / 64 : (p.M + 127) / 128;
  p.tiles_n = (p.N + bn - 1) / bn;
  p.colgroups = pick_colgroups((long long)p.N * p.K * 4, p.tiles_m, p.tiles_n);
}

void launch_gemm_f16(GemmParams& p, int v, hipStream_t stream) {
  if (p.rowstats && v != 1) v = 2;
  prep_gemm_f16(p, v);
  dim3 grid(p.tiles_m * p.tiles_n), block(256);
  if (v == 1) {
    if (p.rowstats) NPVP_LAUNCH((gemm_f16_kernel<2, 4, 2, 2, true>), grid, block, 0, stream, p);
    else NPVP_LAUNCH((gemm_f16_kernel<2, 4, 2, 2, false>), grid, block, 0, stream, p);
  } else if (v == 3) {
    NPVP_LAUNCH((gemm_f16_kernel<2, 1, 2, 2, false, 2, 3>), grid, block, 0, stream, p);
  } else if (v == 4) {
    NPVP_LAUNCH((gemm_f16_kernel<1, 2, 2, 2, false, 2, 3>), grid, block, 0, stream, p);
  } else {
    if (p.rowstats) NPVP_LAUNCH((gemm_f16_kernel<2, 2, 2, 2, true, 2, 3>), grid, block, 0, stream, p);
    else NPVP_LAUNCH((gemm_f16_kernel<2, 2, 2, 2, false, 2, 3>), grid, block, 0, stream, p);
  }
}

__global__ __launch_bounds__(256) void amax_kernel(const float* __restrict__ x, long long n4, long long ldq, long long cols4, float* slot) {
  __shared__ float ared[4];
  const unsigned int peek = amax_peek_block(slot);
  float m = 0.f;
  for (long long i = (long long)blockIdx.x * blockDim.x + threadIdx.x; i < n4; i += (long long)gridDim.x * blockDim.x) {
    const long long row = i / cols4, c = i - row * cols4;
    m = amax4(m, ld4(x + 4 * (row * ldq + c)));
  }
  amax_slot_commit_block(slot, m, ared, peek);
}

struct SplitDescH { const float* w; long long ld; long long N; long long K; _Float16* F; _Float16* D; float* amax; long long pad; };

__global__ __launch_bounds__(256) void weights_amax_kernel(const SplitDescH* __restrict__ desc, SplitDescH one) {
  const SplitDescH d = desc ? desc[blockIdx.y] : one;
  const int K4 = (int)d.K / 4;
  const long long total = d.N * K4;
  __shared__ float ared[4];
  const unsigned int peek = amax_peek_block(d.amax);
  float m = 0.f;
  for (long long i = (long long)blockIdx.x * blockDim.x + threadIdx.x; i < total; i += (long long)gridDim.x * blockDim.x) {
    const long long n = i / K4; const int k4 = (int)(i - n * K4);
    m = amax4(m, ld4(d.w + n * d.ld + 4 * k4));
  }
  amax_slot_commit_block(d.amax, m, ared, peek);
}

__global__ __launch_bounds__(256) void split_weights_f16_kernel(const SplitDescH* __restrict__ desc, SplitDescH one) {
  const SplitDescH d = desc ? desc[blockIdx.y] : one;
  const int N = (int)d.N, K = (int)d.K;
  const long long slots = (long long)N * K / 8, plane = (long long)N * K;
  const float s = amax_scale(amax_slot_read(d.amax));
  for (long long i = (long long)blockIdx.x * blockDim.x + threadIdx.x; i < 2 * slots; i += (long long)gridDim.x * blockDim.x) {
    float v[8];
    _Float16* out;
    if (i < slots) {
      if (!d.F) continue;
      const int n = (int)(i % N), kb = (int)(i / N);
      const float4 a = ld4(d.w + (long long)n * d.ld + kb * 8), b = ld4(d.w + (long long)n * d.ld + kb * 8 + 4);
      v[0] = a.x; v[1] = a.y; v[2] = a.z; v[3] = a.w; v[4] = b.x; v[5] = b.y; v[6] = b.z; v[7] = b.w;
      out = d.F + i * 8;
    } else {
      if (!d.D) continue;
      const long long j = i - slots;
      const int k = (int)(j % K), nb = (int)(j / K);
#pragma unroll
      for (int e = 0; e < 8; ++e) v[e] = d.w[(long long)(nb * 8 + e) * d.ld + k];
      out = d.D + j * 8;
    }
    f16x8 hi, lo;
#pragma unroll
    for (int e = 0; e < 8; ++e) { const float x = v[e] * s; hi[e] = (_Float16)x; lo[e] = (_Float16)(x - (float)hi[e]); }
    *reinterpret_cast<f16x8*>(out) = hi;
    *reinterpret_cast<f16x8*>(out + plane) = lo;
  }
}

}

using namespace npvp;

extern "C" int npvp_amax(const float* x, long long rows, long long cols, long long ld, float* slot, hipStream_t stream) {
  NPVP_CHECK_ARG(x && slot && rows > 0 && cols > 0 && cols % 4 == 0 && ld % 4 == 0 && ld >= cols, "amax: cols and ld must be multiples of 4");
  NPVP_CHECK_ARG(((uintptr_t)x % 16) == 0, "amax: x must be 16-byte aligned");
  const long long n4 = rows * (cols / 4);
  long long blocks = (n4 + 256 * 8 - 1) / (256 * 8);
  if (blocks > 2048) blocks = 2048;
  if (blocks < 1) blocks = 1;
  NPVP_LAUNCH(amax_kernel, dim3((unsigned)blocks), dim3(256), 0, stream, x, n4, ld / 4, cols / 4, slot);
  NPVP_CHECK_LAUNCH();
  return NPVP_OK;
}

namespace npvp {
__global__ __launch_bounds__(256) void zero_words_kernel(unsigned* __restrict__ p, long long n) {
  for (long long i = (long long)blockIdx.x * 256 + threadIdx.x; i < n; i += (long long)gridDim.x * 256) p[i] = 0u;
}
}

static hipError_t zero_fill(void* p, size_t bytes, hipStream_t stream) {
  const long long n = (long long)(bytes / 4);
  long long blocks = (n + 255) / 256; if (blocks > 1024) blocks = 1024; if (blocks < 1) blocks = 1;
  NPVP_LAUNCH(zero_words_kernel, dim3((unsigned)blocks), dim3(256), 0, stream, (unsigned*)p, n);
  return hipGetLastError();
}

extern "C" int npvp_split_weights_f16(const void* desc, int count, void* amax_table, long long amax_bytes, hipStream_t stream) {
  NPVP_CHECK_ARG(desc && count > 0, "split_weights_f16: empty table");
  if (amax_table && amax_bytes > 0) {
    if (zero_fill(amax_table, (size_t)amax_bytes, stream) != hipSuccess) { npvp_set_error("split_weights_f16: zero fill failed"); return NPVP_ERR_LAUNCH; }
  }
  SplitDescH none = {};
  NPVP_LAUNCH(weights_amax_kernel, dim3(16, count), dim3(256), 0, stream, (const SplitDescH*)desc, none);
  NPVP_CHECK_LAUNCH();
  NPVP_LAUNCH(split_weights_f16_kernel, dim3(128, count), dim3(256), 0, stream, (const SplitDescH*)desc, none);
  NPVP_CHECK_LAUNCH();
  return NPVP_OK;
}

extern "C" int npvp_split_weight_f16(const float* w, long long ld, int N, int K, void* F, void* D, float* amax_slot, hipStream_t stream) {
  NPVP_CHECK_ARG(N > 0 && K > 0 && N % 8 == 0 && K % 8 == 0 && ld % 4 == 0, "split_weight_f16: N, K must be multiples of 8");
  NPVP_CHECK_ARG(((uintptr_t)w % 16) == 0 && amax_slot, "split_weight_f16: w must be 16-byte aligned, amax_slot non-null");
  if (zero_fill(amax_slot, AMAX_WORDS * AMAX_STRIDE * 4, stream) != hipSuccess) { npvp_set_error("split_weight_f16: zero fill failed"); return NPVP_ERR_LAUNCH; }
  SplitDescH one = {w, ld, N, K, (_Float16*)F, (_Float16*)D, amax_slot, 0};
  NPVP_LAUNCH(weights_amax_kernel, dim3(16, 1), dim3(256), 0, stream, (const SplitDescH*)nullptr, one);
  NPVP_CHECK_LAUNCH();
  NPVP_LAUNCH(split_weights_f16_kernel, dim3(128, 1), dim3(256), 0, stream, (const SplitDescH*)nullptr, one);
  NPVP_CHECK_LAUNCH();
  return NPVP_OK;
}

static_assert(sizeof(ReduceJob) == sizeof(npvp_reduce_job_t), "npvp_reduce_job_t (include/npvp_hip.h) mirrors this layout");

extern "C" int npvp_wgrad_f16_chainable(int M, int N, int K) {
  return (M % 4 == 0 && N % 4 == 0 && f16_wgrad_splits(M, N, K) > 1) ? 1 : 0;
}

extern "C" long long npvp_wgrad_f16_chain_workspace_bytes(int M, int N, int K) {
  const int s = f16_wgrad_splits(M, N, K);
  return s > 1 ? splitk_workspace_bytes(s, M, N) : 0;
}

extern "C" int npvp_wgrad_f16_chained(int M, int N, int K, const float* dy, long long lda, const float* x, long long ldb, float* dw,
                                      long long ldc, float* db, int accumulate, const float* a_amax, const float* b_amax,
                                      unsigned int* range_flag, float adrop_p, int adrop_g1, int adrop_g2, unsigned int adrop_salt,
                                      const unsigned long long* seed, const void* prev_job, void* my_job, void* workspace,
                                      long long ws_bytes, hipStream_t stream) {
  NPVP_CHECK_ARG(npvp_wgrad_f16_chainable(M, N, K), "wgrad_f16_chained: shape not taken (npvp_wgrad_f16_chainable tells)");
  NPVP_CHECK_ARG(dy && x && dw && a_amax && b_amax && my_job, "wgrad_f16_chained: null operand / amax slot / job");
  if (!deferred_wgrad_args_ok("wgrad_f16_chained", dy, lda, x, ldb, dw, ldc, adrop_p, adrop_g1, adrop_g2, seed, workspace, ws_bytes,
                              npvp_wgrad_f16_chain_workspace_bytes(M, N, K))) return NPVP_ERR_ARG;
  NPVP_CHECK_ARG(!db || ((uintptr_t)db % 16) == 0, "wgrad_f16_chained: the bias gradient must be 16-byte aligned");
  GemmParams p = deferred_wgrad_params(M, N, K, dy, lda, x, ldb, a_amax, b_amax, range_flag, make_drop_spec(adrop_p, adrop_salt, 1, adrop_g1, adrop_g2),
                                       seed, prev_job, workspace, db != nullptr, accumulate);
  launch_gemm_wgrad_f16(p, stream);
  NPVP_CHECK_LAUNCH();
  leave_reduce_job(p, dw, ldc, db, my_job);
  return NPVP_OK;
}

extern "C" int npvp_linear_bwd_f16_takes(int R, int N, int K) {
  const int v = gemm_f16_variant(R, K, N);
  return ((v == 2 || v == 3 || v == 4) && npvp_wgrad_f16_chainable(N, K, R)) ? 1 : 0;
}

extern "C" int npvp_linear_bwd_f16_skip(int R, int N, int K, const float* dy, long long ldy, const float* dy_amax, const void* w_planes_d,
                                        const float* w_amax, float* dx, long long ldx, int act, const float* aux_in, const float* residual,
                                        long long ldr, float drop_p, int drop_mode, int drop_g1, int drop_g2, unsigned int drop_salt,
                                        float* dx_amax, const float* x, long long ldxx, const float* x_amax, float* dw, long long ldw, float* db,
                                        unsigned int* range_flag, float adrop_p, int adrop_g1, int adrop_g2, unsigned int adrop_salt,
                                        float skip_p, int skip_g1, int skip_g2, unsigned int skip_salt,
                                        const unsigned long long* seed, const void* prev_job, void* my_job, void* workspace,
                                        long long ws_bytes, hipStream_t stream) {
  NPVP_CHECK_ARG(skip_p >= 0.f && skip_p < 1.f && (skip_p == 0.f || (seed && skip_g1 > 0 && skip_g2 > 0)),
                 "linear_bwd_f16: the row skip needs a device seed and row groups");
  NPVP_CHECK_ARG(npvp_linear_bwd_f16_takes(R, N, K), "linear_bwd_f16: shape not taken (npvp_linear_bwd_f16_takes tells)");
  NPVP_CHECK_ARG(dy && dy_amax && w_planes_d && w_amax && dx && x && x_amax && dw && my_job, "linear_bwd_f16: null operand / amax slot / job");
  if (!deferred_wgrad_args_ok("linear_bwd_f16", dy, ldy, x, ldxx, dw, ldw, adrop_p, adrop_g1, adrop_g2, seed, workspace, ws_bytes,
                              npvp_wgrad_f16_chain_workspace_bytes(N, K, R))) return NPVP_ERR_ARG;
  NPVP_CHECK_ARG(((uintptr_t)dx % 16) == 0 && ((uintptr_t)w_planes_d % 16) == 0 && ldx % 4 == 0,
                 "linear_bwd_f16: operands must be 16-byte aligned with leading dimensions that are multiples of 4");
  NPVP_CHECK_ARG((!db || ((uintptr_t)db % 16) == 0) && (!residual || (((uintptr_t)residual % 16) == 0 && ldr % 4 == 0)) &&
                 (!aux_in || ((uintptr_t)aux_in % 16) == 0), "linear_bwd_f16: db / residual / aux_in must be 16-byte aligned");
  NPVP_CHECK_ARG(act == 0 || ((act == 3 || act == 4) && aux_in), "linear_bwd_f16: act must be 0, or 3 / 4 with aux_in");
  NPVP_CHECK_ARG(drop_p >= 0.f && drop_p < 1.f && (drop_p == 0.f || seed), "linear_bwd_f16: dropout p out of range or no seed");
  GemmGroup g = {};
  GemmParams& d = g.p[0];
  d.A = dy; d.lda = ldy; d.C = dx; d.ldc = ldx; d.M = R; d.N = K; d.K = N; d.alpha = 1.f; d.act = act; d.aux_in = aux_in;
  d.residual = residual; d.ldr = ldr; d.seed = seed; d.splits = 1;
  d.drop = make_drop_spec(drop_p, drop_salt, drop_mode, drop_g1, drop_g2);
  d.adrop = make_drop_spec(adrop_p, adrop_salt, 1, adrop_g1, adrop_g2);
  d.rskip = make_drop_spec(skip_p, skip_salt, 1, skip_g1, skip_g2);
  d.b_pre = w_planes_d; d.b_pre_plane = (long long)N * K;
  d.a_amax = dy_amax; d.b_amax = w_amax; d.c_amax = dx_amax;
  GemmParams& w = g.p[1] = deferred_wgrad_params(N, K, R, dy, ldy, x, ldxx, dy_amax, x_amax, range_flag, d.adrop, seed, prev_job, workspace, db != nullptr, 1);
  const dim3 wgrid = size_gemm_wgrad_f16(w);
  const int t128 = ((R + 127) / 128) * ((K + 127) / 128), wwg = (int)wgrid.x * w.splits;
  int v = gemm_f16_variant(R, K, N);
  if (v == 4 && 2 * t128 + wwg > 512) v = 2;
  prep_gemm_f16(d, v);
  g.count[0] = d.tiles_m * d.tiles_n;
  g.first[0] = 0; g.first[1] = (g.count[0] + 7) & ~7;
  g.count[1] = wgrid.x * wgrid.y;
  g.first[2] = g.first[1] + ((g.count[1] + 7) & ~7);
  g.gx = wgrid.x;
  if (v == 2) NPVP_LAUNCH((gemm_f16_group_kernel<2, 2>), dim3(g.first[2]), dim3(256), 0, stream, g);
  else if (v == 4) NPVP_LAUNCH((gemm_f16_group_kernel<1, 2>), dim3(g.first[2]), dim3(256), 0, stream, g);
  else NPVP_LAUNCH((gemm_f16_group_kernel<2, 1>), dim3(g.first[2]), dim3(256), 0, stream, g);
  NPVP_CHECK_LAUNCH();
  leave_reduce_job(w, dw, ldw, db, my_job);
  return NPVP_OK;
}

extern "C" int npvp_linear_bwd_f16(int R, int N, int K, const float* dy, long long ldy, const float* dy_amax, const void* w_planes_d,
                                   const float* w_amax, float* dx, long long ldx, int act, const float* aux_in, const float* residual,
                                   long long ldr, float drop_p, int drop_mode, int drop_g1, int drop_g2, unsigned int drop_salt,
                                   float* dx_amax, const float* x, long long ldxx, const float* x_amax, float* dw, long long ldw, float* db,
                                   unsigned int* range_flag, float adrop_p, int adrop_g1, int adrop_g2, unsigned int adrop_salt,
                                   const unsigned long long* seed, const void* prev_job, void* my_job, void* workspace,
                                   long long ws_bytes, hipStream_t stream) {
  return npvp_linear_bwd_f16_skip(R, N, K, dy, ldy, dy_amax, w_planes_d, w_amax, dx, ldx, act, aux_in, residual, ldr, drop_p, drop_mode,
                                  drop_g1, drop_g2, drop_salt, dx_amax, x, ldxx, x_amax, dw, ldw, db, range_flag, adrop_p, adrop_g1, adrop_g2,
                                  adrop_salt, 0.f, 1, 1, 0u, seed, prev_job, my_job, workspace, ws_bytes, stream);
}

__global__ __launch_bounds__(256) void splitk_reduce_job_kernel(ReduceJob j) {
  float cm = 0.f;
  splitk_reduce_body(j, blockIdx.x, gridDim.x, cm);
}

constexpr int RJ_MAX = 32;
struct ReduceBatch { ReduceJob j[RJ_MAX]; int first[RJ_MAX + 1]; int n; };
__global__ __launch_bounds__(256) void splitk_reduce_multi_kernel(ReduceBatch b) {
  int lo = 0, hi = b.n - 1;
  while (lo < hi) { const int mid = (lo + hi + 1) >> 1; if (b.first[mid] <= (int)blockIdx.x) lo = mid; else hi = mid - 1; }
  float cm = 0.f;
  splitk_reduce_body(b.j[lo], (int)blockIdx.x - b.first[lo], b.first[lo + 1] - b.first[lo], cm);
}

extern "C" int npvp_splitk_reduce_multi(const void* jobs, int n, hipStream_t stream) {
  NPVP_CHECK_ARG(jobs && n > 0, "splitk_reduce_multi: no jobs");
  const ReduceJob* J = reinterpret_cast<const ReduceJob*>(jobs);
  for (int at = 0; at < n; at += RJ_MAX) {
    ReduceBatch b;
    b.n = n - at < RJ_MAX ? n - at : RJ_MAX;
    int blocks = 0;
    for (int i = 0; i < b.n; ++i) {
      b.j[i] = J[at + i];
      NPVP_CHECK_ARG(b.j[i].ws && b.j[i].out && b.j[i].M > 0 && b.j[i].N > 0 && b.j[i].splits > 0, "splitk_reduce_multi: empty job");
      const long long total4 = (long long)b.j[i].M * b.j[i].N / 4;
      int nb = (int)((total4 + 255) / 256); if (nb > 256) nb = 256;
      b.first[i] = blocks; blocks += nb;
    }
    b.first[b.n] = blocks;
    NPVP_LAUNCH(splitk_reduce_multi_kernel, dim3(blocks), dim3(256), 0, stream, b);
    NPVP_CHECK_LAUNCH();
  }
  return NPVP_OK;
}

extern "C" int npvp_splitk_reduce_job(const void* job, hipStream_t stream) {
  NPVP_CHECK_ARG(job, "splitk_reduce_job: null job");
  const ReduceJob j = *reinterpret_cast<const ReduceJob*>(job);
  NPVP_CHECK_ARG(j.ws && j.out && j.M > 0 && j.N > 0 && j.splits > 0, "splitk_reduce_job: empty job");
  const long long total4 = (long long)j.M * j.N / 4;
  int blocks = (int)((total4 + 255) / 256); if (blocks > 2048) blocks = 2048;
  NPVP_LAUNCH(splitk_reduce_job_kernel, dim3(blocks), dim3(256), 0, stream, j);
  NPVP_CHECK_LAUNCH();
  return NPVP_OK;
}
```

npvp_amd/ops.py:

```python
import functools
import os
from collections import namedtuple

import torch

from ._lib import lib, check
from . import sched as _S
from .sched import (_p, _ptr, _stream, _ws, AmaxSlot, GemmProbe, HbmProbe, ProbeEvent, AuxStream, StepContext, current, use, scoped,
                    remember, rng, GradSink, WgradStream, WgradChain, ReduceQueue, RangeGuard)


def amax_of(t, slot=None):
    if slot is not None:
        return slot
    for cand in (t, t._base):
        tag = getattr(cand, "_npvp_amax", None) if cand is not None else None
        if tag is not None and tag[1] == cand._version:
            return tag[0]
    s = AmaxSlot.new(t.device)
    t2 = t if t.dim() == 2 else t.reshape(-1, t.shape[-1])
    if t2.stride(1) != 1:
        t2 = t2.contiguous()
    check(lib().npvp_amax(_ptr(t2), t2.shape[0], t2.shape[1], t2.stride(0), _ptr(s), _stream()), "npvp_amax")
    t._npvp_amax = (s, t._version)
    return s


def tag_amax(t, slot):
    if slot is not None:
        t._npvp_amax = (slot, t._version)
    return t


def _row(t, i):
    return t.data_ptr() + 4 * i * t.stride(0)


def _chk(*ts):
    for t in ts:
        if t is None:
            continue
        if not t.is_cuda:
            raise RuntimeError("npvp_amd ops need tensors on an MI355X device (no CPU fallback)")
        if t.dtype != torch.float32:
            raise RuntimeError("npvp_amd ops are fp32")


def _c(t):
    return t if t.is_contiguous() else t.contiguous()


class Drop:
    __slots__ = ("p", "mode", "g1", "g2", "salt")

    def __init__(self, p=0.0, mode=0, g1=1, g2=1):
        self.p, self.mode, self.g1, self.g2 = float(p), mode, g1, g2
        self.salt = _S._cur.rng.next_salt() if p > 0 else 0

    @property
    def on(self):
        return self.p > 0.0

    @classmethod
    def _like(cls, other, mode, g1, g2):
        d = cls.__new__(cls)
        d.p, d.mode, d.g1, d.g2, d.salt = other.p, mode, g1, g2, other.salt
        return d


NO_DROP = Drop(0.0)


class DropRecorder:
    sites = None

    @classmethod
    def note(cls, drop, kind, count):
        if cls.sites is not None and drop.on:
            cls.sites.append((drop, kind, int(count)))

    @staticmethod
    def mask(site, dev):
        drop, kind, count = site
        if kind == "elem":
            pad = (-count) % 4
            ones = torch.ones((count + pad) // 4, 4, dtype=torch.float32, device=dev)
            return drop_apply(ones, Drop._like(drop, 0, 1, 1)).reshape(-1)[:count]
        ones = torch.ones(count, 4, dtype=torch.float32, device=dev)
        return drop_apply(ones, Drop._like(drop, 1, 1, count))[:, 0].contiguous()


GEMM_MODES = {"f32": 0, "bf16x6": 4, "bf16x6db": 4, "bf16x3": 5, "bf16x3db": 5, "f16x3": 6}
GEMM_PRECISION = GEMM_MODES[os.environ.get("NPVP_GEMM", "f16x3")]


WGRAD_PRECISION = {"": None, "bf16x6": None, "same": None, "bf16x3": 5}[os.environ.get("NPVP_WGRAD", "")]


def set_gemm_precision(name):
    global GEMM_PRECISION
    GEMM_PRECISION = GEMM_MODES[name]


class WeightPlanes:
    enabled = True
    _owners = []
    _tables = None
    _group_tensors = {}
    _dirty = True
    _gen = object()

    class Entry:
        __slots__ = ("fmt", "version", "planes", "w", "amax", "amax_t", "F", "D")

    @classmethod
    def _owner_died(cls, _ref):
        cls._dirty = True

    @classmethod
    def invalidate(cls, owner=None):
        cls.refresh_all(owner)

    @classmethod
    def forget(cls, owner):
        if owner.__dict__.pop("_npvp_planes", None) is not None:
            cls._dirty = True
            cls._gen = object()

    @staticmethod
    def _split(ent):
        w = ent.w
        N, K = w.shape
        F, D = _p(ent.planes[0].data_ptr()), _p(ent.planes[1].data_ptr())
        if ent.fmt == 6:
            check(lib().npvp_split_weight_f16(_ptr(w), w.stride(0), N, K, F, D, _ptr(ent.amax), _stream()), "npvp_split_weight_f16")
        else:
            check(lib().npvp_split_weight(_ptr(w), w.stride(0), N, K, F, D, _stream()), "npvp_split_weight")
        ent.version = w._version

    @classmethod
    def get(cls, w, want):
        fmt = GEMM_PRECISION
        hit = w.__dict__.get("_npvp_ent")
        if hit is not None:
            ent = hit[0]
            if ent.fmt == fmt and hit[1] == w.data_ptr() and ent.version == w._version and hit[2] is cls._gen and cls.enabled:
                return (ent.F if want == "F" else ent.D), ent.amax
        if not cls.enabled or fmt not in (4, 6) or w.dim() != 2 or w.shape[0] % 8 or w.shape[1] % 8 or w.stride(1) != 1:
            return None
        owner = w._base if w._base is not None else w
        if not owner.is_leaf and owner.grad_fn is not None:
            return None
        store = owner.__dict__.get("_npvp_planes")
        if store is None:
            import weakref
            store = owner.__dict__["_npvp_planes"] = {}
            cls._owners.append(weakref.ref(owner, cls._owner_died))
        key = (fmt, w.data_ptr(), tuple(w.shape), w.stride(0))
        ent = store.get(key)
        if ent is None:
            live = owner.untyped_storage().data_ptr()
            for k in [k for k, e in store.items() if e.w.untyped_storage().data_ptr() != live]:
                del store[k]
            N, K = w.shape
            ent = cls.Entry()
            ent.fmt, ent.w = fmt, w.detach()
            if fmt == 6:
                ent.planes = torch.empty(2, 2 * N * K, dtype=torch.float16, device=w.device)
                ent.amax_t = torch.zeros(AmaxSlot.FLOATS, dtype=torch.float32, device=w.device)
                ent.amax = AmaxSlot(ent.amax_t.data_ptr(), ent.amax_t)
            else:
                ent.planes = torch.empty(2, 3 * N * K, dtype=torch.bfloat16, device=w.device)
                ent.amax = ent.amax_t = None
            ent.F, ent.D = ent.planes[0], ent.planes[1]
            cls._split(ent)
            store[key] = ent
            cls._dirty = True
        elif ent.version != w._version:
            cls._split(ent)
        if w._base is None and tuple(w.shape) == tuple(ent.w.shape):
            w.__dict__["_npvp_ent"] = (ent, w.data_ptr(), cls._gen)
        return (ent.F if want == "F" else ent.D), ent.amax

    @classmethod
    def _entries(cls):
        live = []
        for ref in cls._owners:
            owner = ref()
            if owner is None:
                continue
            live.append(ref)
            for ent in owner.__dict__.get("_npvp_planes", {}).values():
                yield ent
        cls._owners = live

    @classmethod
    def refresh_if_stale(cls):
        if any(ent.version != ent.w._version for ent in cls._entries()):
            cls.refresh_all()

    epoch = 0

    @classmethod
    def refresh_all(cls, owner=None):
        cls.epoch += 1
        if not cls.enabled:
            return
        if cls._dirty or cls._tables is None:
            owner = None
            groups = {}
            for ent in cls._entries():
                if ent.w.is_cuda:
                    groups.setdefault((ent.w.untyped_storage().data_ptr(), ent.fmt, ent.w.device), []).append(ent)
            cls._tables = []
            kept = {}
            for gkey, ents in groups.items():
                own_id, fmt, dev = gkey
                ids = tuple(id(e) for e in ents)
                old = cls._group_tensors.get(gkey)
                if old is not None and old[0] == ids and (fmt != 6 or all(e.amax_t is old[2] for e in ents)):
                    table, amax_t = old[1], old[2]
                else:
                    amax_t = None
                    if fmt == 6:
                        amax_t = torch.zeros(len(ents), AmaxSlot.FLOATS, dtype=torch.float32, device=dev)
                        for i, ent in enumerate(ents):
                            ent.amax_t = amax_t
                            ent.amax.ptr, ent.amax.chunk = amax_t.data_ptr() + AmaxSlot.BYTES * i, amax_t
                    rows = []
                    for ent in ents:
                        N, K = ent.w.shape
                        r = [ent.w.data_ptr(), ent.w.stride(0), N, K, ent.planes[0].data_ptr(), ent.planes[1].data_ptr()]
                        rows.append(r + [ent.amax.ptr, 0] if fmt == 6 else r)
                    table = torch.tensor(rows, dtype=torch.int64).to(dev)
                kept[gkey] = (ids, table, amax_t)
                cls._tables.append((fmt, table, amax_t, ents, own_id))
            cls._group_tensors = kept
            cls._dirty = False
        only = None if owner is None else owner.untyped_storage().data_ptr()
        for fmt, table, amax_t, ents, own_id in cls._tables:
            if only is not None and own_id != only:
                continue
            with torch.cuda.device(table.device):
                if fmt == 6:
                    check(lib().npvp_split_weights_f16(_p(table.data_ptr()), table.shape[0], _p(amax_t.data_ptr()),
                                                       amax_t.numel() * 4, _stream()), "npvp_split_weights_f16")
                else:
                    check(lib().npvp_split_weights_batched(_p(table.data_ptr()), table.shape[0], _stream()), "npvp_split_weights_batched")
            for ent in ents:
                ent.version = ent.w._version




def gemm(a_kc, b_kc, M, N, K, A, lda, B, ldb, out, bias=None, act=0, aux_in=None, aux_out=None, residual=None,
         drop=NO_DROP, alpha=1.0, colsum_a=None, b_pre=None, accumulate=False, rowstats=None, precision=None,
         replay=False, a_amax=None, b_amax=None, c_amax=None, a_drop=NO_DROP, range_flag=None, row_skip=NO_DROP):
    for t in (A, B, out, bias, aux_in, aux_out, residual, colsum_a):
        if t is not None and not (t.is_cuda and t.dtype is torch.float32):
            _chk(t)
    prec = GEMM_PRECISION if precision is None else precision
    planes = None
    if b_pre is not None:
        planes, b_amax = b_pre
    if prec == 6:
        kid = _gemm_kernel_id(a_kc, b_kc, M, N, K, 6, planes is not None)
        if kid == 5 or kid == 7:
            if a_amax is None:
                a_amax = amax_of(A)
        elif kid == 6:
            if a_amax is None:
                a_amax = amax_of(A)
            if b_amax is None:
                b_amax = amax_of(B)
        else:
            planes = None
    wsb = _gemm_ws_bytes(M, N, K)
    ws, wsn = (None, 0)
    if wsb > 0:
        ws, wsn = _ws(wsb, A.device)
    masked = drop.p > 0.0 or a_drop.p > 0.0 or row_skip.p > 0.0
    seed = _S._cur.rng.seed_tensor(A.device) if masked else None
    if DropRecorder.sites is not None and not replay:
        DropRecorder.note(drop, "elem" if drop.mode == 0 else "group", M * N if drop.mode == 0 else drop.g2)
    pe = None
    if GemmProbe.armed:
        kid = _gemm_kernel_id(a_kc, b_kc, M, N, K, prec, planes is not None)
        pe = GemmProbe.begin(kid)
    rc = lib().npvp_gemm_f32_skip(
        a_kc, b_kc, M, N, K, A.data_ptr(), lda, B.data_ptr(), ldb, out.data_ptr(), out.stride(0),
        None if bias is None else bias.data_ptr(), act, None if aux_in is None else aux_in.data_ptr(),
        None if aux_out is None else aux_out.data_ptr(), None if residual is None else residual.data_ptr(),
        0 if residual is None else residual.stride(0), drop.p, drop.mode, drop.g1, drop.g2,
        None if seed is None else seed.data_ptr(), drop.salt, alpha, prec, None if colsum_a is None else colsum_a.data_ptr(),
        None if planes is None else planes.data_ptr(), 1 if accumulate else 0, None if rowstats is None else rowstats.data_ptr(),
        None if a_amax is None else a_amax.data_ptr(), None if b_amax is None else b_amax.data_ptr(),
        None if c_amax is None else c_amax.data_ptr(), None if range_flag is None else range_flag.data_ptr(),
        a_drop.p, a_drop.g1, a_drop.g2, a_drop.salt, row_skip.p, row_skip.g1, row_skip.g2, row_skip.salt,
        None if ws is None else ws.data_ptr(), wsn, _stream())
    if rc:
        check(rc, "npvp_gemm_f32_skip")
    if pe is not None:
        GemmProbe.end(pe, 2.0 * M * N * K, 4.0 * (M * K + N * K + M * N), (a_kc, b_kc), kid)
    return out


@functools.lru_cache(maxsize=None)
def _gemm_kernel_id(a_kc, b_kc, M, N, K, prec, has_planes):
    return lib().npvp_gemm_kernel_id(a_kc, b_kc, M, N, K, prec, int(has_planes))


@functools.lru_cache(maxsize=None)
def _gemm_ws_bytes(M, N, K):
    return lib().npvp_gemm_workspace_bytes(M, N, K)


def _planes(w, want, R):
    return WeightPlanes.get(w, want) if R >= 256 else None


def _new_slot(dev, want=True):
    return AmaxSlot.new(dev) if (want and GEMM_PRECISION == 6) else None


def _sunk(sk, want_b):
    return bool(sk) and want_b == (sk[1] is not None)


def _h16(N, K, R, precision):
    return precision == 6 and _gemm_kernel_id(0, 0, N, K, R, 6, False) == 6


LinearBwdPlan = namedtuple("LinearBwdPlan", "fused reduction sunk on_grad_stream urgent fill_slots")
WgradPlan = namedtuple("WgradPlan", "route precision watch")


@functools.lru_cache(maxsize=None)
def linear_bwd_plan(R, N, K, precision, sunk, grad_stream, guard_quiet=True, unit_strides=True, planes=False, fused_on=False,
                    fused_with_stream=False, max_rows=0):
    if (fused_on and precision == 6 and sunk and R <= max_rows and (fused_with_stream or not grad_stream) and guard_quiet
            and unit_strides and planes and lib().npvp_linear_bwd_f16_takes(R, N, K) and WgradChain.takes(N, K, R)):
        return LinearBwdPlan(True, "queued" if grad_stream else "chained", False, False, False, False)
    on_side = sunk and grad_stream
    return LinearBwdPlan(False, None, sunk, on_side, on_side and 2.0 * R * N * K >= 3e10, sunk and _h16(N, K, R, precision))


@functools.lru_cache(maxsize=None)
def wgrad_plan(N, K, R, precision, wgrad_precision, accumulate, masked, fallback, strict, in_flush, grad_stream, listener,
               chain_on, unit_strides):
    prec = wgrad_precision if precision == 4 else None
    watch = _h16(N, K, R, precision)
    if watch and fallback and not masked:
        prec, watch = 4, False
    if watch and strict and not masked:
        return WgradPlan("strict", None, True)
    if (watch and accumulate and prec is None and chain_on and WgradChain.takes(N, K, R)
            and (in_flush or (not grad_stream and not listener)) and unit_strides):
        return WgradPlan("chained", None, True)
    return WgradPlan("gemm", prec, watch)


def linear_fwd(x, w, b, act=0, aux_out=None, residual=None, drop=NO_DROP, rowstats=None, x_amax=None, y_amax=None):
    R, K = x.shape
    N = w.shape[0]
    y = torch.empty(R, N, dtype=torch.float32, device=x.device)
    return gemm(1, 1, R, N, K, x, x.stride(0), w, w.stride(0), y, bias=b, act=act, aux_out=aux_out, residual=residual,
                drop=drop, b_pre=_planes(w, "F", R), rowstats=rowstats, a_amax=x_amax, c_amax=y_amax)


def linear_frame_stats_supported(R, N):
    return GEMM_PRECISION in (4, 6) and R % 64 == 0 and N % 128 == 0


def linear_dgrad(dy, w, act=0, aux_in=None, drop=NO_DROP, residual=None, dy_amax=None, dx_amax=None, a_drop=NO_DROP, out=None,
                 accumulate=False, row_skip=NO_DROP):
    R, N = dy.shape
    K = w.shape[1]
    dx = torch.empty(R, K, dtype=torch.float32, device=dy.device) if out is None else out
    return gemm(1, 0, R, K, N, dy, dy.stride(0), w, w.stride(0), dx, act=act, aux_in=aux_in, drop=drop, residual=residual,
                b_pre=_planes(w, "D", R), replay=True, a_amax=dy_amax, c_amax=dx_amax, a_drop=a_drop, accumulate=accumulate,
                row_skip=row_skip)


def masked_grad(dy2, drop, w):
    if not drop.on:
        return dy2, NO_DROP
    R, N = dy2.shape
    K = w.shape[1]
    if (drop.mode == 1 and drop.g1 % 16 == 0 and drop.p < 0.5 and GEMM_PRECISION == 6 and R <= DROP_PATH_IN_GEMM_ROWS
            and _planes(w, "D", R) is not None and _gemm_kernel_id(1, 0, R, K, N, 6, True) in (5, 7) and _h16(N, K, R, 6)):
        return dy2, drop
    return drop_apply(dy2, drop), NO_DROP


DROP_PATH_IN_GEMM_ROWS = 1 << 30


def linear_wgrad(dy, x, with_bias_grad=False, into=None, into_b=None, dy_amax=None, x_amax=None, a_drop=NO_DROP):
    R, N = dy.shape
    K = x.shape[1]
    acc = into is not None
    dw = into if acc else torch.empty(N, K, dtype=torch.float32, device=dy.device)
    db = (into_b if acc else torch.empty(N, dtype=torch.float32, device=dy.device)) if with_bias_grad else None
    c = _S._cur
    g = c.range_guard
    plan = wgrad_plan(N, K, R, GEMM_PRECISION, WGRAD_PRECISION, acc, a_drop.on, g.fallback, g.strict, c.wgrad.in_flush, c.wgrad.enabled,
                      c.grad_sink.listener is not None, c.chain.enabled, dy.stride(1) == 1 and x.stride(1) == 1 and dw.stride(1) == 1)
    flag = g.flag(dy.device) if plan.watch else None
    if plan.route == "strict":
        tw = torch.empty(N, K, dtype=torch.float32, device=dy.device)
        tb = torch.empty(N, dtype=torch.float32, device=dy.device) if with_bias_grad else None
        gemm(0, 0, N, K, R, dy, dy.stride(0), x, x.stride(0), tw, colsum_a=tb, a_amax=dy_amax, b_amax=x_amax, range_flag=flag)
        if g.poll(dy.device):
            g.fallback = False
            gemm(0, 0, N, K, R, dy, dy.stride(0), x, x.stride(0), tw, colsum_a=tb, precision=4)
        if acc:
            dw.add_(tw)
            if tb is not None:
                db.add_(tb)
        else:
            dw, db = tw, tb
    elif plan.route == "chained":
        c.chain.launch(dy, x, dw, db, amax_of(dy, dy_amax), amax_of(x, x_amax), a_drop, flag)
    else:
        gemm(0, 0, N, K, R, dy, dy.stride(0), x, x.stride(0), dw, colsum_a=db, accumulate=acc, precision=plan.precision, a_amax=dy_amax,
             b_amax=x_amax, a_drop=a_drop, range_flag=flag)
    return (dw, db) if with_bias_grad else dw


class FusedLinearBwd:
    enabled = True
    MAX_ROWS = 16384
    with_gradient_stream = False

    @classmethod
    def takes(cls, R, N, K):
        return linear_bwd_plan(R, N, K, 6, True, False, True, True, True, True, False, cls.MAX_ROWS).fused


def linear_bwd(dy, x, w, b, sk, act=0, aux_in=None, drop=NO_DROP, residual=None, dy_amax=None, dx_amax=None, a_drop=NO_DROP,
               row_skip=NO_DROP):
    R, N = dy.shape
    K = w.shape[1]
    has_b = b is not None
    c = _S._cur
    sunk = _sunk(sk, has_b)
    pl = _planes(w, "D", R)
    plan = linear_bwd_plan(R, N, K, GEMM_PRECISION, sunk, c.wgrad.enabled, not (c.range_guard.fallback or c.range_guard.strict),
                           dy.stride(1) == 1 and x.stride(1) == 1 and (not sunk or sk[0][0].stride(1) == 1), pl is not None,
                           FusedLinearBwd.enabled, FusedLinearBwd.with_gradient_stream, FusedLinearBwd.MAX_ROWS)
    if not plan.fused:
        dx = linear_dgrad(dy, w, act=act, aux_in=aux_in, drop=drop, residual=residual, dy_amax=dy_amax, dx_amax=dx_amax, a_drop=a_drop,
                          row_skip=row_skip)
        gw, gb = _lin_grads(dy, x, w, b, sk, a_drop=a_drop, plan=plan)
        return dx, gw, gb
    planes, w_amax = pl
    gw, gb = sk[0][0], (sk[1][0] if has_b else None)
    dev = dy.device
    dy_amax, x_amax = amax_of(dy, dy_amax), amax_of(x)
    dx = torch.empty(R, K, dtype=torch.float32, device=dev)
    ws, wsn = _ws(c.chain.workspace_bytes(N, K, R), dev)
    st = _stream()
    seed = c.rng.seed_tensor(dev) if (drop.on or a_drop.on or row_skip.on) else None
    outs = (gw.data_ptr(),) if gb is None else (gw.data_ptr(), gb.data_ptr())
    later = c.chain if plan.reduction == "chained" else c.reduce
    job_addr, prev_addr = later.job_slot(st, outs)
    pe = GemmProbe.begin(8)
    head = (R, N, K, dy.data_ptr(), dy.stride(0), dy_amax.data_ptr(), planes.data_ptr(), w_amax.data_ptr(), dx.data_ptr(), dx.stride(0),
            act, _ptr(aux_in), _ptr(residual), 0 if residual is None else residual.stride(0), drop.p, drop.mode, drop.g1, drop.g2,
            drop.salt, _ptr(dx_amax), x.data_ptr(), x.stride(0), x_amax.data_ptr(), gw.data_ptr(), gw.stride(0), _ptr(gb),
            _ptr(c.range_guard.flag(dev)), a_drop.p, a_drop.g1, a_drop.g2, a_drop.salt)
    tail = (_ptr(seed), prev_addr, job_addr, ws.data_ptr(), wsn, st)
    if row_skip.on:
        check(lib().npvp_linear_bwd_f16_skip(*head, row_skip.p, row_skip.g1, row_skip.g2, row_skip.salt, *tail), "npvp_linear_bwd_f16_skip")
    else:
        check(lib().npvp_linear_bwd_f16(*head, *tail), "npvp_linear_bwd_f16")
    GemmProbe.end(pe, 4.0 * R * N * K, 4.0 * (2 * R * N + 2 * R * K + 2 * N * K), (1, 0), 8)
    later.job_added(st, outs, (ws, gw, gb), sk)
    return dx, None, None


def colsum(x):
    R, N = x.shape
    L = lib()
    out = torch.empty(N, dtype=torch.float32, device=x.device)
    ws, wsn = _ws(L.npvp_colsum_workspace_bytes(R, N), x.device)
    check(L.npvp_colsum(_ptr(x), R, N, x.stride(0), _ptr(out), 0, _ptr(ws), wsn, _stream()), "npvp_colsum")
    return out


def drop_apply(x2d, drop):
    out = torch.empty_like(x2d)
    slot = _new_slot(x2d.device)
    check(lib().npvp_drop_apply(_ptr(x2d), _ptr(out), x2d.shape[0], x2d.shape[1], drop.p, drop.mode, drop.g1, drop.g2,
                                _ptr(_S._cur.rng.seed_tensor(x2d.device)), drop.salt, _ptr(slot), _stream()), "npvp_drop_apply")
    return tag_amax(out, slot)


def transpose(x):
    _chk(x)
    x = _c(x)
    B, R, C = x.shape
    out = torch.empty(B, C, R, dtype=torch.float32, device=x.device)
    check(lib().npvp_transpose(_ptr(x), _ptr(out), B, R, C, _stream()), "npvp_transpose")
    return out


def reduce_mid(x, scale=1.0, out=None, accumulate=False):
    _chk(x)
    x = _c(x)
    A, B, C = x.shape
    if out is None:
        out = torch.empty(A, C, dtype=torch.float32, device=x.device)
    check(lib().npvp_reduce_mid(_ptr(x), _ptr(out), A, B, C, scale, 1 if accumulate else 0, _stream()), "npvp_reduce_mid")
    return out


class ActSink:
    __slots__ = ("buf",)
    enabled = True

    def __init__(self):
        self.buf = None

    def target(self, shape, dev):
        if self.buf is None:
            self.buf = torch.empty(shape, dtype=torch.float32, device=dev)
            return self.buf, False
        if self.buf.numel() != torch.Size(shape).numel():
            raise RuntimeError(f"ActSink: a consumer contributes a gradient of shape {tuple(shape)} to a buffer of shape {tuple(self.buf.shape)}")
        return self.buf, True

    @staticmethod
    def of(t):
        return None if t is None else getattr(t, "_npvp_sink", None)


class _FanOut(torch.autograd.Function):
    @staticmethod
    def forward(ctx, t, sink):
        ctx.sink = sink
        ctx.set_materialize_grads(False)
        return t.view_as(t)

    @staticmethod
    def backward(ctx, g):
        buf, ctx.sink.buf = ctx.sink.buf, None
        if buf is None:
            return g, None
        if g is not None:
            buf.add_(g.reshape(buf.shape))
        return buf, None


def fan_out(t):
    if t is None or not (ActSink.enabled and t.is_cuda and t.requires_grad and torch.is_grad_enabled()):
        return t
    sink = ActSink()
    out = _FanOut.apply(t, sink)
    out._npvp_sink = sink
    return out


def broadcast_mid(x, B, scale=1.0):
    _chk(x)
    x = _c(x)
    A, C = x.shape
    out = torch.empty(A, B, C, dtype=torch.float32, device=x.device)
    check(lib().npvp_broadcast_mid(_ptr(x), _ptr(out), A, B, C, scale, _stream()), "npvp_broadcast_mid")
    return out


class _Transpose(torch.autograd.Function):
    @staticmethod
    def forward(ctx, x):
        remember(ctx)
        return transpose(x)

    @scoped
    def backward(ctx, g):
        return transpose(g)


class _MeanMid(torch.autograd.Function):

    @staticmethod
    def forward(ctx, x):
        remember(ctx)
        ctx.B = x.shape[1]
        return reduce_mid(x, 1.0 / x.shape[1])

    @scoped
    def backward(ctx, g):
        return broadcast_mid(g, ctx.B, 1.0 / ctx.B)


class _L1Mean(torch.autograd.Function):

    @staticmethod
    def forward(ctx, a, b, lam):
        remember(ctx)
        _chk(a, b)
        if a.shape != b.shape:
            raise RuntimeError(f"l1_mean: shapes differ: {tuple(a.shape)} / {tuple(b.shape)}")
        a, b = _c(a), _c(b)
        out = torch.empty((), dtype=torch.float32, device=a.device)
        ws, wsn = _ws(4096, a.device)
        check(lib().npvp_l1_mean(_ptr(a), _ptr(b), a.numel(), float(lam), _ptr(out), _ptr(ws), wsn, _stream()), "npvp_l1_mean")
        ctx.save_for_backward(a, b)
        ctx.lam = float(lam)
        return out

    @scoped
    def backward(ctx, g):
        a, b = ctx.saved_tensors
        _chk(g)
        da = torch.empty_like(a)
        check(lib().npvp_l1_mean_bwd(_ptr(a), _ptr(b), a.numel(), _ptr(_c(g)), ctx.lam, _ptr(da), _stream()), "npvp_l1_mean_bwd")
        return da, None, None


def l1_mean(a, b, lam=1.0):
    if b.requires_grad:
        raise RuntimeError("l1_mean: only the first operand takes a gradient (the Stage-2 losses compare against ground truth)")
    return _L1Mean.apply(a, b, lam)


# ... 122 lines not shown
        return dx.reshape(ctx.shape), dw, db, None


def layernorm_res(x, w, b, eps=1e-5):
    return _LayerNormRes.apply(x, w, b, eps)


class _PosFuse(torch.autograd.Function):

    @staticmethod
    def forward(ctx, x, add, beta, gamma, N, T):
        remember(ctx)
        _chk(x, add, beta, gamma)
        x = _c(x)
        beta = _c(beta)
        add_c = None if add is None else _c(add)
        gamma_c = None if gamma is None else _c(gamma)
        y, st = _raw_posfuse_fwd(x, add_c, beta, gamma_c, N, T)
        ctx.save_for_backward(x, add_c, gamma_c, st)
        ctx.N, ctx.T, ctx.PF = N, T, x.numel() // (N * T)
        ctx.beta_shape = beta.shape
        return y

    @scoped
    def backward(ctx, dy):
        x, add, gamma, st = ctx.saved_tensors
        N, T, PF = ctx.N, ctx.T, ctx.PF
        dy = _c(dy)
        du, dbeta, dgamma = _posfuse_bwd_call(dy, x, add, gamma, st, N, T, PF, ctx.beta_shape, ctx.needs_input_grad[2],
                                              gamma is not None and ctx.needs_input_grad[3])
        dadd = reduce_mid(du.view(N, T, PF)).view(add.shape) if (add is not None and ctx.needs_input_grad[1]) else None
        return du, dadd, dbeta, dgamma, None, None


def _posfuse_bwd_call(dy, x, add, gamma, st, N, T, PF, beta_shape, want_beta, want_gamma, beta_sink=None, gamma_sink=None):
    L = lib()
    du = torch.empty_like(x)
    acc = False
    sunk = beta_sink is not None and want_beta and (not want_gamma or gamma_sink is not None)
    if sunk:
        dbeta, acc = beta_sink.target(beta_shape, x.device)
        dgamma = None
        if want_gamma:
            dgamma, acc_g = gamma_sink.target(gamma.shape, x.device)
            if acc_g != acc:
                (dgamma if not acc_g else dbeta).zero_()
                acc = True
    else:
        dbeta = torch.empty(beta_shape, dtype=torch.float32, device=x.device) if want_beta else None
        dgamma = torch.empty(gamma.shape, dtype=torch.float32, device=x.device) if want_gamma else None
    dyxh = torch.empty_like(x) if (want_gamma and not L.npvp_posfuse_bwd_fused(N, T, PF)) else None
    ws, wsn = _ws(8 * N * T, x.device)
    check(L.npvp_posfuse_bwd(_ptr(dy), _ptr(x), _ptr(add), _ptr(gamma), _row(st, 0), _row(st, 1), _ptr(du), _ptr(dyxh), _ptr(dbeta),
                             _ptr(dgamma), N, T, PF, 1 if acc else 0, _ptr(ws), wsn, _stream()), "npvp_posfuse_bwd")
    return (du, None, None) if sunk else (du, dbeta, dgamma)


def posfuse(x, add, beta, gamma, N, T):
    return _PosFuse.apply(x, add, beta, gamma, N, T)


class _PosFuseInstance(torch.autograd.Function):

    @staticmethod
    def forward(ctx, x, add, beta, gamma, N, T):
        remember(ctx)
        _chk(x, add, beta, gamma)
        x = _c(x)
        C = x.shape[-1]
        P = x.numel() // (N * T * C)
        beta = _c(beta)
        add_c = None if add is None else _c(add)
        gamma_c = None if gamma is None else _c(gamma)
        y = torch.empty_like(x)
        st = torch.empty(2, N * T, C, dtype=torch.float32, device=x.device)
        slot = _new_slot(x.device)
        check(lib().npvp_posfuse_instance_fwd(_ptr(x), _ptr(add_c), _ptr(beta), _ptr(gamma_c), _ptr(y), _row(st, 0), _row(st, 1), N, T, P,
                                              C, 1e-5, _ptr(slot), _stream()), "npvp_posfuse_instance_fwd")
        tag_amax(y, slot)
        ctx.save_for_backward(x, add_c, gamma_c, st)
        ctx.cfg = (N, T, P, C, beta.shape)
        return y

    @scoped
    def backward(ctx, dy):
        x, add, gamma, st = ctx.saved_tensors
        N, T, P, C, beta_shape = ctx.cfg
        dy = _c(dy)
        du = torch.empty_like(x)
        dyxh = torch.empty_like(x) if (gamma is not None and ctx.needs_input_grad[3]) else None
        check(lib().npvp_posfuse_instance_bwd(_ptr(dy), _ptr(x), _ptr(add), _ptr(gamma), _row(st, 0), _row(st, 1), _ptr(du), _ptr(dyxh),
                                              N, T, P, C, _stream()), "npvp_posfuse_instance_bwd")
        PF = P * C
        dadd = reduce_mid(du.view(N, T, PF)).view(add.shape) if (add is not None and ctx.needs_input_grad[1]) else None
        dbeta = reduce_mid(dy.view(1, N, T * PF)).view(beta_shape) if ctx.needs_input_grad[2] else None
        dgamma = reduce_mid(dyxh.view(1, N, T * PF)).view(gamma.shape) if dyxh is not None else None
        return du, dadd, dbeta, dgamma, None, None


def posfuse_instance(x, add, beta, gamma, N, T):
    return _PosFuseInstance.apply(x, add, beta, gamma, N, T)


class _Linear(torch.autograd.Function):

    @staticmethod
    def forward(ctx, x, w, b, residual, drop, frame_stats=False):
        remember(ctx)
        _chk(x, w, b, residual)
        K = x.shape[-1]
        x2 = x.reshape(-1, K)
        if x2.stride(1) != 1 or x2.stride(0) % 4 != 0:
            x2 = x2.contiguous()
        w = w if (w.stride(1) == 1 and w.stride(0) % 4 == 0) else w.contiguous()
        r2 = None if residual is None else _c(residual).reshape(-1, w.shape[0])
        ctx.save_for_backward(x2, w)
        ctx.drop, ctx.has_b, ctx.has_r, ctx.xshape = drop, b is not None, residual is not None, x.shape
        ctx.sink = _wb_sink(w, b)
        if frame_stats:
            R, N = x2.shape[0], w.shape[0]
            frames = R // 64
            part = torch.empty(frames * (N // 64) * 2, dtype=torch.float32, device=x.device)
            y = linear_fwd(x2, w, b, rowstats=part)
            mean = torch.empty(frames, dtype=torch.float32, device=x.device)
            rstd = torch.empty_like(mean)
            check(lib().npvp_frame_stats_finalize(_ptr(part), N // 64, 4096.0, _ptr(mean), _ptr(rstd), frames, 1e-5, _stream()),
                  "npvp_frame_stats_finalize")
            ctx.mark_non_differentiable(mean, rstd)
            ctx.set_materialize_grads(False)
            return y.reshape(*x.shape[:-1], N), mean, rstd
        y = linear_fwd(x2, w, b, residual=r2, drop=drop)
        return y.reshape(*x.shape[:-1], w.shape[0])

    @scoped
    def backward(ctx, dy, *_stats_grads):
        x2, w = ctx.saved_tensors
        N = w.shape[0]
        dy2 = _c(dy).reshape(-1, N)
        if ctx.needs_input_grad[0] and ctx.needs_input_grad[1]:
            dz, ad = masked_grad(dy2, ctx.drop, w)
        else:
            dz, ad = (drop_apply(dy2, ctx.drop) if ctx.drop.on else dy2), NO_DROP
        dx = linear_dgrad(dz, w, a_drop=ad).reshape(ctx.xshape) if ctx.needs_input_grad[0] else None
        dw = db = None
        want_b = ctx.has_b and ctx.needs_input_grad[2]
        if ctx.needs_input_grad[1]:
            dw, db = _lin_grads(dz, x2, w, True if want_b else None, ctx.sink, a_drop=ad)
        elif want_b:
            db = colsum(dz)
        dres = dy if ctx.has_r else None
        return dx, dw, db, dres, None, None


def _lin_grads(dy, x, w, b, sk, a_drop=NO_DROP, plan=None):
    has_b = b is not None
    if plan is None:
        plan = linear_bwd_plan(dy.shape[0], dy.shape[1], x.shape[1], GEMM_PRECISION, _sunk(sk, has_b), _S._cur.wgrad.enabled)
    if not plan.sunk:
        g = linear_wgrad(dy, x, has_b, a_drop=a_drop)
        return (g[0], g[1]) if has_b else (g, None)
    a1, a2 = (amax_of(dy), amax_of(x)) if plan.fill_slots else (None, None)
    fn = lambda dy=dy, x=x, gw=sk[0][0], gb=(sk[1][0] if has_b else None), a1=a1, a2=a2, ad=a_drop: \
        linear_wgrad(dy, x, has_b, into=gw, into_b=gb, dy_amax=a1, x_amax=a2, a_drop=ad)
    if plan.on_grad_stream:
        _S._cur.wgrad.run(fn, dy, x, wrote=sk, urgent=plan.urgent)
    else:
        fn()
        _S._cur.grad_sink.wrote(*sk)
    return None, None


def _wb_sink(w, b):
    sw = _S._cur.grad_sink.slot(w)
    if sw is None:
        return None
    if b is None or not b.requires_grad:
        return (sw, None)
    sb = _S._cur.grad_sink.slot(b)
    return (sw, sb) if sb is not None else None


def linear(x, w, b=None, residual=None, drop=NO_DROP, frame_stats=False):
    if frame_stats:
        assert residual is None and not drop.on
    return _Linear.apply(x, w, b, residual, drop, bool(frame_stats))


class _FFN(torch.autograd.Function):

    @staticmethod
    def forward(ctx, xn, x, w1, b1, w2, b2, p):
        remember(ctx)
        _chk(xn, x, w1, b1, w2, b2)
        C = xn.shape[-1]
        xn2, x2 = _c(xn).reshape(-1, C), _c(x).reshape(-1, C)
        h, a, y, d2, d3 = _ffn_fwd(xn2, x2, w1, b1, w2, b2, p)
        ctx.save_for_backward(xn2, h, a, w1, w2)
        ctx.d2, ctx.d3, ctx.shape = d2, d3, x.shape
        s1, s2 = _wb_sink(w1, b1), _wb_sink(w2, b2)
        ctx.sink = (s1, s2) if (_sunk(s1, True) and _sunk(s2, True)) else None
        return y.reshape(x.shape)

    @scoped
    def backward(ctx, dy):
        xn2, h, a, w1, w2 = ctx.saved_tensors
        C = xn2.shape[1]
        dy2 = _c(dy).reshape(-1, C)
        dz2, ad = masked_grad(dy2, ctx.d3, w2)
        sk = ctx.sink
        if sk:
            dh = linear_dgrad(dz2, w2, act=3, aux_in=h, drop=ctx.d2, a_drop=ad)
            _lin_grads(dz2, a, w2, True, sk[1], a_drop=ad)
            dxn = linear_dgrad(dh, w1)
            _lin_grads(dh, xn2, w1, True, sk[0])
            return dxn.reshape(ctx.shape), dy, None, None, None, None, None
        dw2, db2 = linear_wgrad(dz2, a, True, a_drop=ad)
        dh = linear_dgrad(dz2, w2, act=3, aux_in=h, drop=ctx.d2, a_drop=ad)
        dw1, db1 = linear_wgrad(dh, xn2, True)
        dxn = linear_dgrad(dh, w1)
        return dxn.reshape(ctx.shape), dy, dw1, db1, dw2, db2, None


def _ffn_fwd(xn2, x2, w1, b1, w2, b2, p):
    d2, d3 = Drop(p), Drop(p)
    h = torch.empty(xn2.shape[0], w1.shape[0], dtype=torch.float32, device=xn2.device)
    a_slot = _new_slot(xn2.device)
    a = tag_amax(linear_fwd(xn2, w1, b1, act=1, aux_out=h, drop=d2, y_amax=a_slot), a_slot)
    return h, a, linear_fwd(a, w2, b2, residual=x2, drop=d3), d2, d3


def ffn(xn, x, w1, b1, w2, b2, p):
    return _FFN.apply(xn, x, w1, b1, w2, b2, p)


def window_pad_geometry(H, W, ws):
    Hp, Wp = -(-H // ws) * ws, -(-W // ws) * ws
    return Hp, Wp, (Hp - H) // 2, (Wp - W) // 2


class AttnCfg:
    __slots__ = ("mode", "dim0", "P", "W", "ws", "Tq", "Tk", "heads", "mask_mode", "drop", "grid")

    def __init__(self, mode, dim0, P, W, ws, Tq, Tk, heads, mask_mode, p_drop, grid=None):
        self.mode, self.dim0, self.P, self.W, self.ws, self.Tq, self.Tk = mode, dim0, P, W, ws, Tq, Tk
        self.heads, self.mask_mode = heads, mask_mode
        self.drop = Drop(p_drop)
        self.grid = grid

    @property
    def tiles(self):
        return self.grid is None

    @classmethod
    def spatial(cls, frames, H, W, ws, heads, p_drop):
        Hp, Wp, top, left = window_pad_geometry(H, W, ws)
        grid = None if (Hp, Wp) == (H, W) else (H, W, top, left)
        return cls(0, frames, Hp * Wp, Wp, ws, 0, 0, heads, 0, p_drop, grid)

    def pad_args(self):
        H, W, top, left = self.grid
        return self.dim0, H, W, self.P // self.W, self.W, top, left

    @property
    def padded_rows(self):
        return -(-self.dim0 * self.P // 32) * 32


ATTN_LONG_MIN = 129


def _attn_len(cfg):
    return (cfg.ws * cfg.ws, cfg.ws * cfg.ws) if cfg.mode == 0 else (cfg.Tq, cfg.Tk)


def _attn_long(cfg):
    return max(_attn_len(cfg)) >= ATTN_LONG_MIN


def _attn_fwd(q, k, v, o, cfg):
    hd = o.shape[1] // cfg.heads
    seed = _S._cur.rng.seed_tensor(q.device) if cfg.drop.on else None
    if DropRecorder.sites is not None and cfg.drop.on:
        L_, S_ = _attn_len(cfg)
        groups = cfg.dim0 * (cfg.P // (cfg.ws * cfg.ws)) if cfg.mode == 0 else cfg.dim0 * cfg.P
        DropRecorder.note(cfg.drop, "elem", groups * cfg.heads * L_ * S_)
    slot = _new_slot(q.device)
    fn, what = (lib().npvp_attn_long_fwd, "npvp_attn_long_fwd") if _attn_long(cfg) else (lib().npvp_attn_fwd, "npvp_attn_fwd")
    check(fn(_ptr(q), q.stride(0), _ptr(k), k.stride(0), _ptr(v), v.stride(0), _ptr(o), o.stride(0),
             cfg.mode, cfg.dim0, cfg.P, cfg.W, cfg.ws, cfg.Tq, cfg.Tk, cfg.heads, hd, cfg.mask_mode,
             cfg.drop.p, _ptr(seed), cfg.drop.salt, _ptr(slot), _stream()), what)
    tag_amax(o, slot)


ATTN_SAMPLES_MAX = 32


def _attn_samples_fwd(q, k, v, o, cfg, S, sample_chunk=0):
    if cfg.mode != 1 or cfg.mask_mode != 0 or cfg.drop.on:
        raise ValueError("_attn_samples_fwd: temporal geometry without mask and dropout only")
    hd = o.shape[1] // cfg.heads
    slot = _new_slot(q.device)
    if max(cfg.Tq, cfg.Tk) <= ATTN_SAMPLES_MAX:
        check(lib().npvp_attn_samples_fwd(_ptr(q), q.stride(0), _ptr(k), k.stride(0), _ptr(v), v.stride(0), _ptr(o), o.stride(0),
                                          S, cfg.dim0, cfg.P, cfg.Tq, cfg.Tk, cfg.heads, hd, sample_chunk, _ptr(slot), _stream()),
              "npvp_attn_samples_fwd")
    else:
        fn, what = (lib().npvp_attn_long_fwd, "npvp_attn_long_fwd") if _attn_long(cfg) else (lib().npvp_attn_fwd, "npvp_attn_fwd")
        rows = cfg.dim0 * cfg.Tq * cfg.P
# ... 182 lines not shown
        out = torch.empty_like(a)
        ctx.save_for_backward(a, wtb)
        ctx.cfg = (frames, H, W, Ch)
        if want_stats:
            mean = torch.empty(frames, dtype=torch.float32, device=a.device)
            rstd = torch.empty_like(mean)
            ws, wsn = _ws(frames * (Ch // 1024) * 8, a.device)
            check(lib().npvp_dwconv3x3_stats(_ptr(a), _ptr(wtb), _row(wtb, 9), _ptr(out), _ptr(mean), _ptr(rstd), frames, H, W,
                                             Ch, 1e-5, _ptr(ws), wsn, _stream()), "npvp_dwconv3x3_stats")
            ctx.mark_non_differentiable(mean, rstd)
            ctx.set_materialize_grads(False)
            return out, mean, rstd
        check(lib().npvp_dwconv3x3(_ptr(a), _ptr(wtb), _row(wtb, 9), _ptr(out), frames, H, W, Ch, 0, _stream()),
              "npvp_dwconv3x3")
        return out

    @scoped
    def backward(ctx, dout, *_unused):
        a, wtb = ctx.saved_tensors
        frames, H, W, Ch = ctx.cfg
        dout = _c(dout)
        L = lib()
        da = torch.empty_like(a)
        check(L.npvp_dwconv3x3(_ptr(dout), _ptr(wtb), _p(0), _ptr(da), frames, H, W, Ch, 1, _stream()), "npvp_dwconv3x3(bwd)")
        dwtb = torch.empty_like(wtb)
        ws, wsn = _ws(L.npvp_dwconv3x3_wgrad_workspace_bytes(frames, Ch), a.device)
        check(L.npvp_dwconv3x3_wgrad(_ptr(a), _ptr(dout), _ptr(dwtb), frames, H, W, Ch, _ptr(ws), wsn, _stream()),
              "npvp_dwconv3x3_wgrad")
        return da, dwtb, None, None, None, None


def dwconv3x3(a, wtb, frames, H, W, want_stats=False):
    return _DwConv.apply(a, wtb, frames, H, W, bool(want_stats))


class _MlpDwbn(torch.autograd.Function):

    @staticmethod
    def forward(ctx, x, res, w1, b1, n1w, n1b, dww, dwb, n2w, n2b, w2, b2, n3w, n3b, frames, T, p_drop, p_dp):
        remember(ctx)
        _chk(x, res, w1, b1, w2, b2)
        L = lib()
        R, C = x.shape
        hid, Co = w1.shape[0], w2.shape[0]
        dev, f32 = x.device, torch.float32
        st = _stream()
        PFh, PFo = 64 * hid, 64 * Co
        d2, d3, dp = Drop(p_drop), Drop(p_drop), Drop(p_dp, 1)
        sk = dp if (DROP_PATH_SKIP and dp.on) else NO_DROP
        rs = Drop._like(dp, 1, T * 64, frames // T) if (sk.on and frames % T == 0) else NO_DROP
        seed = _S._cur.rng.seed_tensor(dev) if (d2.on or dp.on) else None
        h1 = torch.empty(R, hid, dtype=f32, device=dev)
        part = torch.empty(frames * (hid // 64) * 2, dtype=f32, device=dev)
        gemm(1, 1, R, hid, C, x, x.stride(0), w1, w1.stride(0), h1, bias=b1, b_pre=_planes(w1, "F", R),
             rowstats=part, row_skip=rs)
        stats = torch.empty(6, frames, dtype=f32, device=dev)
        key = (WeightPlanes.epoch, dww._version, dwb._version, dww.data_ptr(), dwb.data_ptr())
        hit = dww.__dict__.get("_npvp_wtb")
        if hit is not None and hit[0] == key:
            wtb = hit[1]
        else:
            wtb = torch.empty(10, hid, dtype=f32, device=dev)
            check(L.npvp_dwtb_build(_ptr(_c(dww)), _ptr(dwb), _ptr(wtb), hid, st), "npvp_dwtb_build")
            dww.__dict__["_npvp_wtb"] = (key, wtb)
        h2 = torch.empty(R, hid, dtype=f32, device=dev)
        part2 = torch.empty(frames * (hid // 512) * 2, dtype=f32, device=dev)
        check(L.npvp_mlpdw_mid_fwd_parts_skip(_ptr(h1), _ptr(part), hid // 64, 4096.0, _row(stats, 0), _row(stats, 1), _ptr(n1w),
                                              _ptr(n1b), _ptr(wtb), _row(wtb, 9), _ptr(h2), _ptr(part2), frames, 8, 8, hid, 1e-5, sk.p,
                                              sk.salt, T, _ptr(seed), st), "npvp_mlpdw_mid_fwd_parts_skip")
        DropRecorder.note(d2, "elem", R * hid)
        a2 = torch.empty(R, hid, dtype=f32, device=dev)
        a2_slot = _new_slot(dev)
        check(L.npvp_frameln_act_fwd_parts_skip(_ptr(h2), _ptr(part2), hid // 512, 32768.0, 1e-5, _row(stats, 2), _row(stats, 3),
                                                _ptr(n2w), _ptr(n2b), None, _ptr(a2), frames, PFh, d2.p, d2.salt, 0.0, 0, 1, _ptr(seed),
                                                _ptr(a2_slot), sk.p, sk.salt, T, st), "npvp_frameln_act_fwd_parts_skip")
        tag_amax(a2, a2_slot)
        h3 = torch.empty(R, Co, dtype=f32, device=dev)
        part3 = torch.empty(frames * (Co // 64) * 2, dtype=f32, device=dev)
        gemm(1, 1, R, Co, hid, a2, hid, w2, w2.stride(0), h3, bias=b2, b_pre=_planes(w2, "F", R),
             rowstats=part3, row_skip=rs)
        DropRecorder.note(d3, "elem", R * Co)
        DropRecorder.note(dp, "group", frames // max(1, T))
        out = torch.empty(R, Co, dtype=f32, device=dev)
        check(L.npvp_frameln_act_fwd_parts_skip(_ptr(h3), _ptr(part3), Co // 64, 4096.0, 1e-5, _row(stats, 4), _row(stats, 5),
                                                _ptr(n3w), _ptr(n3b), _ptr(res), _ptr(out), frames, PFo, d3.p, d3.salt, dp.p, dp.salt, T,
                                                _ptr(seed), None, sk.p, sk.salt, T, st), "npvp_frameln_act_fwd_parts_skip")
        ctx.save_for_backward(x, h1, h2, a2, h3, stats, wtb, w1, w2, n1w, n1b, n2w, n2b, n3w, n3b)
        ctx.cfg = (frames, T, d2, d3, dp, res is not None, b1 is not None, b2 is not None)
        ctx.skip = (sk, T, rs) if sk.on else None
        ctx.sinks = (_wb_sink(w1, b1), _wb_sink(w2, b2), _ln_sink(n1w, n1b), _ln_sink(n2w, n2b), _ln_sink(n3w, n3b))
        sd = _wb_sink(dww, dwb) if (dww.is_contiguous() and dwb is not None) else None
        ctx.sink_dw = sd if (sd and sd[1] is not None) else None
        return out

    @scoped
    def backward(ctx, dout):
        x, h1, h2, a2, h3, stats, wtb, w1, w2, n1w, n1b, n2w, n2b, n3w, n3b = ctx.saved_tensors
        frames, T, d2, d3, dp, has_res, has_b1, has_b2 = ctx.cfg
        s_fc1, s_fc2, s_n1, s_n2, s_n3 = ctx.sinks
        L = lib()
        R, hid = h1.shape
        Co = h3.shape[1]
        dev = x.device
        sk, sT, rs = ctx.skip if ctx.skip else (NO_DROP, 1, NO_DROP)
        skip = (sk, sT) if sk.on else None
        dout = _c(dout)
        dh3, gn3w, gn3b = _fln_bwd(dout, h3, stats[4], stats[5], n3w, n3b, frames, 64 * Co, d3, dp, T, s_n3)
        da2, gw2, gb2 = linear_bwd(dh3, a2, w2, True if has_b2 else None, s_fc2, row_skip=rs)
        fuse_n2 = MID_BWD_N2 and hid // 16 <= 256
        if fuse_n2:
            psum2, gn2w, gn2b = _fln_pgrad(da2, h2, _row(stats, 2), _row(stats, 3), n2w, n2b, frames, 64 * hid, d2, s_n2)
        else:
            dh2, gn2w, gn2b = _fln_bwd(da2, h2, stats[2], stats[3], n2w, n2b, frames, 64 * hid, d2, NO_DROP, 1, s_n2,
                                          want_amax=False)
            del da2
        da1 = torch.empty_like(h1)
        dwtb = torch.empty(10, hid, dtype=torch.float32, device=dev)
        nparts = hid // 256
        psum = torch.empty(frames * nparts * 2, dtype=torch.float32, device=dev)
        ws, wsn = _ws(L.npvp_mlpdw_mid_bwd_workspace_bytes(frames, hid), dev)
        sk_dw = ctx.sink_dw if ctx.needs_input_grad[6] and ctx.needs_input_grad[7] else None
        wmode = 2 if sk_dw else 0
        if fuse_n2:
            seed = _S._cur.rng.seed_tensor(dev) if d2.on else None
            pe = HbmProbe.begin()
            check(L.npvp_mlpdw_mid_bwd_n2(_ptr(da2), _ptr(h2), _row(stats, 2), _row(stats, 3), _ptr(n2w), _ptr(n2b), _ptr(psum2),
                                          hid // 16, d2.p, d2.salt, _ptr(seed), _ptr(h1), _row(stats, 0), _row(stats, 1), _ptr(n1w),
                                          _ptr(n1b), _ptr(wtb), _ptr(da1), _ptr(dwtb), _ptr(psum), frames, 8, 8, hid, wmode, _ptr(ws), wsn,
                                          _stream()), "npvp_mlpdw_mid_bwd_n2")
            HbmProbe.end(pe, "npvp::mlpdw_mid_bwd_kernel<1, true>", 4.0 * 4 * frames * 64 * hid)
            del da2, psum2
        else:
            check(L.npvp_mlpdw_mid_bwd(_ptr(dh2), _ptr(h1), _row(stats, 0), _row(stats, 1), _ptr(n1w), _ptr(n1b), _ptr(wtb), _ptr(da1),
                                       _ptr(dwtb), _ptr(psum), frames, 8, 8, hid, wmode, _ptr(ws), wsn, _stream()), "npvp_mlpdw_mid_bwd")
            del dh2
        if sk_dw:
            _reduce_partials(sk_dw, ws, sk_dw[0][0], sk_dw[1][0], L.npvp_mlpdw_mid_bwd_reduce_into, L.npvp_mlpdw_mid_bwd_reduce_job,
                             "npvp_mlpdw_mid_bwd_reduce_into", (frames, hid), False)
            gdww = gdwb = None
        else:
            gdww = torch.empty(hid, 1, 3, 3, dtype=torch.float32, device=dev)
            check(L.npvp_transpose(_ptr(dwtb), _ptr(gdww), 1, 9, hid, _stream()), "npvp_transpose")
            gdwb = dwtb[9]
        dh1, gn1w, gn1b = _fln_bwd(da1, h1, stats[0], stats[1], n1w, n1b, frames, 64 * hid, NO_DROP, NO_DROP, 1, s_n1,
                                      psum=psum, nparts=nparts, skip=skip)
        del da1
        dx, gw1, gb1 = linear_bwd(dh1, x, w1, True if has_b1 else None, s_fc1, row_skip=rs)
        return (dx, dout if has_res else None, gw1, gb1, gn1w, gn1b, gdww, gdwb, gn2w, gn2b, gw2, gb2, gn3w, gn3b,
                None, None, None, None)


MID_BWD_N2 = True
DROP_PATH_SKIP = True


def mlpdwbn_fused_supported(R, C, hid, Co, H, W):
    return (GEMM_PRECISION in (4, 6) and H == 8 and W == 8 and R % 64 == 0 and hid % 512 == 0 and Co % 128 == 0 and hid % 128 == 0
            and C % 32 == 0)


def mlpdwbn(x, res, w1, b1, n1w, n1b, dww, dwb, n2w, n2b, w2, b2, n3w, n3b, frames, T, p_drop, p_dp):
    return _MlpDwbn.apply(x, res, w1, b1, n1w, n1b, dww, dwb, n2w, n2b, w2, b2, n3w, n3b, frames, T, p_drop, p_dp)


def _raw_ln_fwd(x2, w, b, eps, relu=0):
    rows, C = x2.shape
    y = torch.empty_like(x2)
    st = torch.empty(2, rows, dtype=torch.float32, device=x2.device)
    slot = _new_slot(x2.device)
    check(lib().npvp_layernorm_fwd(_ptr(x2), _ptr(w), _ptr(b), _ptr(y), _row(st, 0), _row(st, 1), rows, C, eps, relu, _ptr(slot),
                                   _stream()), "npvp_layernorm_fwd")
    return tag_amax(y, slot), st


def _raw_ln_bwd(dy2, x2, w, b, st, dres, sk, relu=0, probe=False):
    L = lib()
    rows, C = x2.shape
    dx = torch.empty_like(x2)
    dw, db = (sk[0][0], sk[1][0]) if sk else (torch.empty_like(w), torch.empty_like(b))
    ws, wsn = _ws(L.npvp_layernorm_bwd_workspace_bytes(rows, C), x2.device)
    slot = _new_slot(x2.device)
    pe = HbmProbe.begin() if probe else None
    check(L.npvp_layernorm_bwd(_ptr(dy2), _ptr(x2), _ptr(w), _ptr(b), _row(st, 0), _row(st, 1), _ptr(dx), _ptr(dw), _ptr(db), rows, C,
                               relu, _ptr(dres), _sink_mode(sk), _ptr(slot), _ptr(ws), wsn, _stream()), "npvp_layernorm_bwd")
    HbmProbe.end(pe, "npvp::ln_bwd_kernel<2>", 4.0 * (3 + (dres is not None)) * rows * C)
    tag_amax(dx, slot)
    if sk:
        _reduce_partials(sk, ws, dw, db, L.npvp_layernorm_bwd_reduce, L.npvp_layernorm_bwd_reduce_job, "npvp_layernorm_bwd_reduce",
                         (rows, C, 1), True)
        return dx, None, None
    return dx, dw, db


def _raw_posfuse_fwd(x, add, beta, gamma, N, T):
    PF = x.numel() // (N * T)
    y = torch.empty_like(x)
    st = torch.empty(2, N * T, dtype=torch.float32, device=x.device)
    slot = _new_slot(x.device)
    check(lib().npvp_posfuse_fwd(_ptr(x), _ptr(add), _ptr(beta), _ptr(gamma), _ptr(y), _row(st, 0), _row(st, 1), N, T, PF, 1e-5,
                                 _ptr(slot), _stream()), "npvp_posfuse_fwd")
    return tag_amax(y, slot), st


LN_POSFUSE_ONE_KERNEL = True


def _raw_ln_posfuse_fwd(x2, lw, lb, eps, add, beta, gamma, N, T):
    rows, C = x2.shape
    if not (LN_POSFUSE_ONE_KERNEL and C == 512 and rows == N * T * 64):
        x1, lst = _raw_ln_fwd(x2, lw, lb, eps)
        fused, pst = _raw_posfuse_fwd(x1, add, beta, gamma, N, T)
        return x1, lst, fused, pst
    x1, fused = torch.empty_like(x2), torch.empty_like(x2)
    lst = torch.empty(2, rows, dtype=torch.float32, device=x2.device)
    pst = torch.empty(2, N * T, dtype=torch.float32, device=x2.device)
    s1, s2 = _new_slot(x2.device), _new_slot(x2.device)
    check(lib().npvp_ln_posfuse_fwd(_ptr(x2), _ptr(lw), _ptr(lb), eps, _ptr(x1), _row(lst, 0), _row(lst, 1), _ptr(add), _ptr(beta),
                                    _ptr(gamma), _ptr(fused), _row(pst, 0), _row(pst, 1), N, T, 64, C, 1e-5, _ptr(s1), _ptr(s2),
                                    _stream()), "npvp_ln_posfuse_fwd")
    return tag_amax(x1, s1), lst, tag_amax(fused, s2), pst


def _raw_posfuse_bwd(dy, x, add, beta_shape, gamma, st, N, T, want_add, sinks=(None, None, None)):
    PF = x.numel() // (N * T)
    du, dbeta, dgamma = _posfuse_bwd_call(dy, x, add, gamma, st, N, T, PF, beta_shape, True, gamma is not None,
                                          sinks[0], sinks[1])
    dadd = None
    if add is not None and want_add:
        if sinks[2] is not None:
            buf, acc = sinks[2].target(add.shape, x.device)
            reduce_mid(du.view(N, T, PF), out=buf.view(N, PF), accumulate=acc)
        else:
            dadd = reduce_mid(du.view(N, T, PF)).view(add.shape)
    return du, dadd, dbeta, dgamma


def _raw_grid_pad(x2, cfg, want_amax=True, out=None):
    F_, H, W, Hp, Wp, top, left = cfg.pad_args()
    rows = cfg.padded_rows
    if out is None:
        out = torch.empty(rows, x2.shape[1], dtype=torch.float32, device=x2.device)
    C = out.shape[1]
    if (0 if x2 is None else x2.shape[0]) != F_ * H * W or (x2 is not None and x2.stride(1) != 1) or out.shape[0] != rows or out.stride(1) != 1:
        raise RuntimeError(f"grid pad: {None if x2 is None else tuple(x2.shape)} -> {tuple(out.shape)} is not {F_} frames of {H} x {W} "
                           f"unit-stride token rows -> {rows} rows")
    slot = _new_slot(out.device, want_amax)
    check(lib().npvp_grid_center_pad(_ptr(x2), C if x2 is None else x2.stride(0), _ptr(out), out.stride(0), F_, H, W, Hp, Wp, top, left, C,
                                     rows, _ptr(slot), _stream()), "npvp_grid_center_pad")
    return tag_amax(out, slot)


def _raw_grid_cut(xp, cfg, addend=None, want_amax=False):
    F_, H, W, Hp, Wp, top, left = cfg.pad_args()
    C = xp.shape[1]
    if xp.shape[0] < F_ * Hp * Wp or xp.stride(1) != 1 or (addend is not None and (addend.shape != (F_ * H * W, C) or addend.stride(1) != 1)):
        raise RuntimeError(f"grid cut: {tuple(xp.shape)} does not hold {F_} frames of {Hp} x {Wp} unit-stride token rows")
    out = torch.empty(F_ * H * W, C, dtype=torch.float32, device=xp.device)
    slot = _new_slot(xp.device, want_amax)
    check(lib().npvp_grid_center_cut(_ptr(xp), xp.stride(0), _ptr(addend), 0 if addend is None else addend.stride(0), _ptr(out),
                                     out.stride(0), F_, H, W, Hp, Wp, top, left, C, _ptr(slot), _stream()), "npvp_grid_center_cut")
    return tag_amax(out, slot)


class _ZeroRows:
    __slots__ = ("padded_rows",)

    def __init__(self, rows):
        self.padded_rows = rows

    def pad_args(self):
        return 0, 1, 1, 1, 1, 0, 0


def _zero_tail(cfg, *ts):
    body = cfg.dim0 * cfg.P
    for t in ts:
        if t.shape[0] > body:
            _raw_grid_pad(None, _ZeroRows(t.shape[0] - body), want_amax=False, out=t[body:])


class _GridPad(torch.autograd.Function):
    @staticmethod
    def forward(ctx, x2, cfg):
        remember(ctx)
        _chk(x2)
        ctx.cfg = cfg
        return _raw_grid_pad(_c(x2), cfg)

    @scoped
    def backward(ctx, g):
        return _raw_grid_cut(_c(g), ctx.cfg), None


class _GridCut(torch.autograd.Function):
    @staticmethod
    def forward(ctx, xp, cfg):
        remember(ctx)
        _chk(xp)
        ctx.cfg = cfg
        return _raw_grid_cut(_c(xp), cfg, want_amax=True)

    @scoped
    def backward(ctx, g):
        return _raw_grid_pad(_c(g), ctx.cfg), None


# ... 520 lines not shown
```

npvp_amd/sched.py:

```python
import contextlib
import ctypes
import functools
import os

import torch

from ._lib import lib, check

_p = ctypes.c_void_p


def _ptr(t):
    return None if t is None else t.data_ptr()


_raw_stream = getattr(torch._C, "_cuda_getCurrentRawStream", None)
_cur_dev = getattr(torch._C, "_cuda_getDevice", None) or torch.cuda.current_device


def _stream():
    if _raw_stream is not None:
        return _raw_stream(_cur_dev())
    return torch.cuda.current_stream().cuda_stream

# ... 311 lines not shown
        if self._pending is not None:
            self.flush()
            dev, side = self._pending
            c = self.ctx
            if c.reduce.pending():
                side.wait_stream(torch.cuda.current_stream(dev))
            with torch.cuda.stream(side):
                c.chain.flush()
                if c.reduce.pending():
                    c.reduce._launch(side)
            torch.cuda.current_stream(dev).wait_stream(side)
            self._pending = None
            self._held, self._held_bytes, self._held_storages = [], 0, set()


class ReduceQueueState:
    enabled = True
    JOB, CAP, LAUNCH = 48, 480, 40
    SKJOB, SKCAP, SKLAUNCH = 64, 256, 16
    DP_LAUNCH = 8
    LAUNCH_BYTES = 192 << 20

    def __init__(self, ctx):
        self.ctx = ctx
        self._buf, self._skbuf = ctypes.create_string_buffer(self.JOB * self.CAP), ctypes.create_string_buffer(self.SKJOB * self.SKCAP)
        self._addr, self._skaddr = ctypes.addressof(self._buf), ctypes.addressof(self._skbuf)
        self._n = self._skn = 0
        self._bytes = 0
        self._keep, self._wrote, self._outs = [], [], set()
        self._armed = False

    def pending(self):
        return self._n + self._skn

    def due(self):
        return self._n >= self.LAUNCH or self._skn >= self.SKLAUNCH or self._bytes >= self.LAUNCH_BYTES

    def job_slot(self, st, out_ptrs):
        if self._skn == self.SKCAP or not self._outs.isdisjoint(out_ptrs):
            self.run_pending()
        return self._skaddr + self.SKJOB * self._skn, None

    def job_added(self, st, out_ptrs, keep, wrote):
        self._skn += 1
        self._added(out_ptrs, keep[0], wrote)

    def _added(self, out_ptrs, keep, wrote):
        self._bytes += keep.numel() * 4
        self._keep.append(keep)
        self._outs.update(out_ptrs)
        if wrote is not None:
            self._wrote.append(wrote)
        self.arm()
        self._dp_progress()

    def _dp_progress(self):
        if self.ctx.grad_sink.listener is not None and self._n + self._skn >= self.DP_LAUNCH:
            self.run_pending()

    def arm(self):
        if not self._armed:
            self._armed = True
            try:
                torch.autograd.Variable._execution_engine.queue_callback(self.finish)
            except RuntimeError:
                self._armed = False

    def add(self, filler, name, args, out_ptrs, keep, wrote):
        if self._n == self.CAP or not self._outs.isdisjoint(out_ptrs):
            self.run_pending()
        check(filler(*args, self._addr + self.JOB * self._n), name)
        self._n += 1
        self._added(out_ptrs, keep, wrote)

    def run_pending(self):
        if self._n + self._skn == 0:
            return
        w = self.ctx.wgrad
        if w.enabled and not w.in_flush:
            w.begin(torch.device("cuda", torch.cuda.current_device()))
            dev, side = w._pending
            side.wait_stream(torch.cuda.current_stream(dev))
            with torch.cuda.stream(side):
                self._launch(side)
        else:
            self._launch(None)

    def _launch(self, side):
        n, skn, keep, wrote = self._n, self._skn, self._keep, self._wrote
        self._n, self._skn, self._bytes, self._keep, self._wrote, self._outs = 0, 0, 0, [], [], set()
        if n:
            check(lib().npvp_sum_rows_multi(self._addr, n, _stream()), "npvp_sum_rows_multi")
        if skn:
            check(lib().npvp_splitk_reduce_multi(self._skaddr, skn, _stream()), "npvp_splitk_reduce_multi")
        w = self.ctx.wgrad
        if side is not None or w.in_flush:
            for t in keep:
                w.hold(t)
        for sk in wrote:
            self.ctx.grad_sink.wrote(*sk)

    def finish(self):
        self._armed = False
        w = self.ctx.wgrad
        if not w.enabled:
            self.ctx.chain.flush()
        if self._n + self._skn == 0:
            return
        if w.enabled:
            w.begin(torch.device("cuda", torch.cuda.current_device()))
            w.join()
        else:
            self._launch(None)


class WgradChainState:
    enabled = True

    def __init__(self, ctx):
        self.ctx = ctx
        self._pending = {}
        self._open = None

    @staticmethod
    @functools.lru_cache(maxsize=None)
    def takes(M, N, K):
        return bool(lib().npvp_wgrad_f16_chainable(M, N, K))

    @staticmethod
    @functools.lru_cache(maxsize=None)
    def workspace_bytes(M, N, K):
        return lib().npvp_wgrad_f16_chain_workspace_bytes(M, N, K)

    def job_slot(self, st, out_ptrs=None):
        self._open = job, prev = ctypes.create_string_buffer(64), self._pending.pop(st, None)
        return ctypes.addressof(job), (ctypes.addressof(prev[0]) if prev is not None else None)

    def job_added(self, st, out_ptrs, keep, wrote):
        job, prev = self._open
        if prev is not None and prev[2] is not None:
            self.ctx.grad_sink.wrote(*prev[2])
        self._pending[st] = (job, keep, wrote)
        if not self.ctx.wgrad.in_flush:
            self.ctx.reduce.arm()

    def launch(self, dy, x, dw, db, dy_amax, x_amax, a_drop, flag):
        R, N = dy.shape
        K = x.shape[1]
        st = _stream()
        ws, wsn = _ws(self.workspace_bytes(N, K, R), dy.device)
        job_addr, prev_addr = self.job_slot(st)
        seed = self.ctx.rng.seed_tensor(dy.device) if a_drop.on else None
        pe = GemmProbe.begin(6)
        check(lib().npvp_wgrad_f16_chained(N, K, R, _ptr(dy), dy.stride(0), _ptr(x), x.stride(0), _ptr(dw), dw.stride(0), _ptr(db), 1,
                                           _ptr(dy_amax), _ptr(x_amax), _ptr(flag), a_drop.p, a_drop.g1, a_drop.g2, a_drop.salt,
                                           _ptr(seed), prev_addr, job_addr, _ptr(ws), wsn, st), "npvp_wgrad_f16_chained")
        GemmProbe.end(pe, 2.0 * N * K * R, 4.0 * (N * R + K * R + N * K), (0, 0), 6)
        self.job_added(st, None, (ws, dw, db), None)

    def flush(self):
        st = _stream()
        prev = self._pending.pop(st, None)
        if prev is not None:
            check(lib().npvp_splitk_reduce_job(ctypes.addressof(prev[0]), st), "npvp_splitk_reduce_job")
            if prev[2] is not None:
                self.ctx.grad_sink.wrote(*prev[2])


class RangeGuardState:
    mode = os.environ.get("NPVP_RANGE_GUARD", "on")
    strict = mode == "strict"
    RETRY_AFTER, RETRY_MAX, PROBATION = 512, 1 << 16, 64

    def __init__(self, ctx):
        self.ctx = ctx
        self.fallback = False
        self.events = 0
        self.retry_after = self.RETRY_AFTER
        self._polls_in_fallback = self._probation = 0
        self._flags = {}
        self._async = None

    def flag(self, dev):
        if self.mode == "off":
            return None
        f = self._flags.get(dev)
        if f is None:
            f = self._flags[dev] = torch.zeros(1, dtype=torch.int32, device=dev)
            if WgradStreamState.enabled:
                f.record_stream(WgradStreamState.stream(dev))
        return f

    def _note(self, f, n):
        if n:
            f.zero_()
            self.events += n
            if self._probation > 0:
                self.retry_after = min(2 * self.retry_after, self.RETRY_MAX)
            self.fallback, self._polls_in_fallback, self._probation = True, 0, 0
        elif self.fallback:
            self._polls_in_fallback += 1
            if self._polls_in_fallback >= self.retry_after:
                self.fallback, self._polls_in_fallback, self._probation = False, 0, self.PROBATION
        elif self._probation > 0:
            self._probation -= 1
            if self._probation == 0:
                self.retry_after = self.RETRY_AFTER
        return n

    def poll(self, dev):
        f = self._flags.get(torch.device(dev) if not isinstance(dev, torch.device) else dev)
        if f is None:
            return 0
        return self._note(f, int(f.item()))

    def poll_async(self, dev):
        dev = torch.device(dev) if not isinstance(dev, torch.device) else dev
        f = self._flags.get(dev)
        if f is None:
            return 0
        n = 0
        if self._async is not None and self._async[1].query():
            n = self._note(f, int(self._async[0][0]))
            self._async = None
        if self._async is None:
            host = torch.zeros(1, dtype=torch.int32).pin_memory()
            host.copy_(f, non_blocking=True)
            ev = torch.cuda.Event()
            ev.record()
            self._async = (host, ev)
        return n

    def reset(self):
        self.fallback, self.events, self._async = False, 0, None
        self.retry_after, self._polls_in_fallback, self._probation = self.RETRY_AFTER, 0, 0
        for f in self._flags.values():
            f.zero_()


class StepContext:
    __slots__ = ("rng", "grad_sink", "wgrad", "chain", "reduce", "range_guard", "name")

    def __init__(self, name="default"):
        self.name = name
        self.rng = RngState(self)
        self.grad_sink = GradSinkState(self)
        self.wgrad = WgradStreamState(self)
        self.chain = WgradChainState(self)
        self.reduce = ReduceQueueState(self)
        self.range_guard = RangeGuardState(self)


_default = StepContext()
_cur = _default


def current():
    return _cur


@contextlib.contextmanager
def use(ctx):
    global _cur
    if ctx is None or ctx is _cur:
        yield
        return
    prev, _cur = _cur, ctx
    try:
        yield
    finally:
        _cur = prev


def scoped(backward):
    def wrapper(ctx, *grads):
        global _cur
        sc = getattr(ctx, "scope", None)
        if sc is None or sc is _cur:
            return backward(ctx, *grads)
        prev, _cur = _cur, sc
        try:
            return backward(ctx, *grads)
        finally:
            _cur = prev
    wrapper.__doc__ = backward.__doc__
    return staticmethod(wrapper)


def remember(ctx):
    ctx.scope = _cur


class _Scoped:
    __slots__ = ("_field", "_cls")

    def __init__(self, field, cls):
        object.__setattr__(self, "_field", field)
        object.__setattr__(self, "_cls", cls)

    def __getattr__(self, name):
        return getattr(getattr(_cur, self._field), name)

    def __setattr__(self, name, value):
        inst = getattr(_cur, self._field)
        if name in inst.__dict__:
            setattr(inst, name, value)
        else:
            setattr(self._cls, name, value)

# ... 8 lines not shown
```

Baseline: 8493.

## Skip dropped row groups in wgrad GEMM K-loop with balanced split-K

Adds a KSKIP variant of the fp16 weight-gradient kernel. It computes the drop-path keep mask per 16-row group with a wavefront ballot and walks only the kept K chunks, so rows zeroed by drop path or the row skip are no longer loaded or multiplied. An optional balance mode spreads the surviving chunks evenly across split-K slices. When the range guard is on, it still scans the amax of skipped rows. Python plumbing routes the plain, chained and fused-linear backward paths to the new entry points. The cost is extra mask-evaluation setup per block and more complex indexing in the load loop.

```diff
diff --git a/include/npvp_hip.h b/include/npvp_hip.h
--- a/include/npvp_hip.h
+++ b/include/npvp_hip.h
@@ -37,6 +37,14 @@
                        float* c_amax, unsigned int* range_flag, float adrop_p, int adrop_g1, int adrop_g2, unsigned int adrop_salt,
                        float skip_p, int skip_g1, int skip_g2, unsigned int skip_salt, void* workspace, long long ws_bytes,
                        npvp_stream_t stream);
+int npvp_gemm_f32_kskip(int a_kc, int b_kc, int M, int N, int K, const float* A, long long lda, const float* B, long long ldb,
+                        float* C, long long ldc, const float* bias, int act, const float* aux_in, float* aux_out,
+                        const float* residual, long long ldr, float drop_p, int drop_mode, int drop_g1, int drop_g2,
+                        const unsigned long long* seed, unsigned int salt, float alpha, int precision, float* colsum_a,
+                        const void* b_pre, int accumulate, float* rowstats, const float* a_amax, const float* b_amax,
+                        float* c_amax, unsigned int* range_flag, float adrop_p, int adrop_g1, int adrop_g2, unsigned int adrop_salt,
+                        float skip_p, int skip_g1, int skip_g2, unsigned int skip_salt, int wgrad_kskip, void* workspace,
+                        long long ws_bytes, npvp_stream_t stream);
 int npvp_frame_stats_finalize(const float* part, int parts_per_frame, float values_per_part, float* mean, float* rstd,
                               int frames, float eps, npvp_stream_t stream);
 int npvp_split_weight(const float* w, long long ld, int N, int K, void* F, void* D, npvp_stream_t stream);
@@ -53,6 +61,11 @@
                            unsigned int* range_flag, float adrop_p, int adrop_g1, int adrop_g2, unsigned int adrop_salt,
                            const unsigned long long* seed, const void* prev_job, void* my_job, void* workspace,
                            long long ws_bytes, npvp_stream_t stream);
+int npvp_wgrad_f16_chained_skip(int M, int N, int K, const float* dy, long long lda, const float* x, long long ldb, float* dw,
+                                long long ldc, float* db, int accumulate, const float* a_amax, const float* b_amax,
+                                unsigned int* range_flag, float adrop_p, int adrop_g1, int adrop_g2, unsigned int adrop_salt,
+                                int adrop_kskip, const unsigned long long* seed, const void* prev_job, void* my_job, void* workspace,
+                                long long ws_bytes, npvp_stream_t stream);
 int npvp_splitk_reduce_job(const void* job, npvp_stream_t stream);
 int npvp_splitk_reduce_multi(const void* jobs, int n, npvp_stream_t stream);
 int npvp_linear_bwd_f16_takes(int R, int N, int K);
@@ -70,6 +83,14 @@
                              unsigned int* range_flag, float adrop_p, int adrop_g1, int adrop_g2, unsigned int adrop_salt,
                              float skip_p, int skip_g1, int skip_g2, unsigned int skip_salt, const unsigned long long* seed,
                              const void* prev_job, void* my_job, void* workspace, long long ws_bytes, npvp_stream_t stream);
+int npvp_linear_bwd_f16_kskip(int R, int N, int K, const float* dy, long long ldy, const float* dy_amax, const void* w_planes_d,
+                              const float* w_amax, float* dx, long long ldx, int act, const float* aux_in, const float* residual,
+                              long long ldr, float drop_p, int drop_mode, int drop_g1, int drop_g2, unsigned int drop_salt,
+                              float* dx_amax, const float* x, long long ldxx, const float* x_amax, float* dw, long long ldw, float* db,
+                              unsigned int* range_flag, float adrop_p, int adrop_g1, int adrop_g2, unsigned int adrop_salt,
+                              float skip_p, int skip_g1, int skip_g2, unsigned int skip_salt, int wgrad_kskip,
+                              const unsigned long long* seed, const void* prev_job, void* my_job, void* workspace, long long ws_bytes,
+                              npvp_stream_t stream);
 int npvp_split_weight_f16(const float* w, long long ld, int N, int K, void* F, void* D, float* amax_slot, npvp_stream_t stream);
 int npvp_split_weights_f16(const void* desc, int count, void* amax_table, long long amax_bytes, npvp_stream_t stream);
 
diff --git a/npvp_amd/csrc/gemm.h b/npvp_amd/csrc/gemm.h
--- a/npvp_amd/csrc/gemm.h
+++ b/npvp_amd/csrc/gemm.h
@@ -37,6 +37,7 @@
   const float* a_amax; const float* b_amax; float* c_amax;
   unsigned int* range_flag;
   ReduceJob prev;
+  int kskip;
 };
 
 __device__ __forceinline__ void splitk_reduce_body(const ReduceJob& j, int bid, int nblocks, float& cmax) {
@@ -311,6 +312,16 @@
   return p >= 0.f && p < 0.5f && (p == 0.f || (seed && g1 > 0 && g2 > 0 && (!rows16 || g1 % 16 == 0)));
 }
 
+inline bool wgrad_kskip_args_ok(int kind, float adrop_p, const DropSpec& spec, const unsigned long long* seed) {
+  const int k = kind & 3;
+  return kind == 0 || ((kind & ~7) == 0 && ((k == 1 && adrop_p > 0.f) || (k == 2 && adrop_p == 0.f && (spec.thresh == 0u || (seed && spec.g1 % 16 == 0)))));
+}
+inline void set_wgrad_kskip(GemmParams& p, int kind, const DropSpec& spec) {
+  p.kskip = kind;
+  if ((kind & 3) == 2) { p.adrop = spec; p.adrop.inv_keep = 1.f; }
+}
+inline bool wgrad_kskips(const GemmParams& p) { return p.kskip != 0 && p.adrop.thresh != 0u; }
+
 int wide_variant(int M, int N, int K);
 void launch_gemm_wide(GemmParams& p, int variant, hipStream_t stream);
 void launch_gemm_wgrad_wide(GemmParams& p, hipStream_t stream);
diff --git a/npvp_amd/csrc/gemm.hip b/npvp_amd/csrc/gemm.hip
--- a/npvp_amd/csrc/gemm.hip
+++ b/npvp_amd/csrc/gemm.hip
@@ -519,17 +519,19 @@
   return finish_partials(make_partials(p.colsum, 0, p.splits, p.splits, p.M, colsum_a, p.accum).job, 0, stream, "gemm: column-sum reduce launch failed");
 }
 
-extern "C" int npvp_gemm_f32_skip(int a_kc, int b_kc, int M, int N, int K, const float* A, long long lda, const float* B,
-                                  long long ldb, float* C, long long ldc, const float* bias, int act, const float* aux_in,
-                                  float* aux_out, const float* residual, long long ldr, float drop_p, int drop_mode,
-                                  int drop_g1, int drop_g2, const unsigned long long* seed, unsigned int salt, float alpha,
-                                  int precision, float* colsum_a, const void* b_pre, int accumulate, float* rowstats,
-                                  const float* a_amax, const float* b_amax, float* c_amax, unsigned int* range_flag,
-                                  float adrop_p, int adrop_g1, int adrop_g2, unsigned int adrop_salt,
-                                  float skip_p, int skip_g1, int skip_g2, unsigned int skip_salt,
-                                  void* workspace, long long ws_bytes, hipStream_t stream) {
-  NPVP_CHECK_ARG(skip_p >= 0.f && skip_p < 1.f && (skip_p == 0.f || (seed && skip_g1 > 0 && skip_g2 > 0 && a_kc)),
+extern "C" int npvp_gemm_f32_kskip(int a_kc, int b_kc, int M, int N, int K, const float* A, long long lda, const float* B,
+                                   long long ldb, float* C, long long ldc, const float* bias, int act, const float* aux_in,
+                                   float* aux_out, const float* residual, long long ldr, float drop_p, int drop_mode,
+                                   int drop_g1, int drop_g2, const unsigned long long* seed, unsigned int salt, float alpha,
+                                   int precision, float* colsum_a, const void* b_pre, int accumulate, float* rowstats,
+                                   const float* a_amax, const float* b_amax, float* c_amax, unsigned int* range_flag,
+                                   float adrop_p, int adrop_g1, int adrop_g2, unsigned int adrop_salt,
+                                   float skip_p, int skip_g1, int skip_g2, unsigned int skip_salt, int wgrad_kskip,
+                                   void* workspace, long long ws_bytes, hipStream_t stream) {
+  NPVP_CHECK_ARG(skip_p >= 0.f && skip_p < 1.f && (skip_p == 0.f || (seed && skip_g1 > 0 && skip_g2 > 0 && (a_kc || (wgrad_kskip & 3) == 2))),
                  "gemm: the row skip needs a device seed, row groups and a row-major A");
+  NPVP_CHECK_ARG(wgrad_kskip == 0 || (!a_kc && !b_kc && precision == 6 && wgrad_kskip_args_ok(wgrad_kskip, adrop_p, make_drop_spec(skip_p, skip_salt, 1, skip_g1, skip_g2), seed)),
+                 "gemm: wgrad_kskip is for precision-6 weight gradients: 1 with adrop, 2 with a skip spec of groups of a multiple of 16 rows");
   NPVP_CHECK_ARG(M > 0 && N > 0 && K > 0, "gemm: empty problem");
   NPVP_CHECK_ARG(precision == 0 || precision == 4 || precision == 5 || precision == 6,
                  "gemm: precision must be 0 (exact fp32-input MFMA), 4 (three-term bf16 split, 6 MFMAs per product: "
@@ -568,6 +570,8 @@
   p.drop = make_drop_spec(drop_p, salt, drop_mode, drop_g1, drop_g2);
   p.adrop = make_drop_spec(adrop_p, adrop_salt, 1, adrop_g1, adrop_g2);
   p.rskip = make_drop_spec(skip_p, skip_salt, 1, skip_g1, skip_g2);
+  p.kskip = 0;
+  if (plan.id == 6) set_wgrad_kskip(p, wgrad_kskip, p.rskip);
   p.alpha = alpha;
   p.rowstats = rowstats;
   p.a_amax = a_amax; p.b_amax = b_amax; p.c_amax = c_amax; p.range_flag = range_flag;
@@ -607,6 +611,20 @@
   return plan.splits > 1 ? finish_splitk(p, C, ldc, colsum_a, stream) : NPVP_OK;
 }
 
+extern "C" int npvp_gemm_f32_skip(int a_kc, int b_kc, int M, int N, int K, const float* A, long long lda, const float* B,
+                                  long long ldb, float* C, long long ldc, const float* bias, int act, const float* aux_in,
+                                  float* aux_out, const float* residual, long long ldr, float drop_p, int drop_mode,
+                                  int drop_g1, int drop_g2, const unsigned long long* seed, unsigned int salt, float alpha,
+                                  int precision, float* colsum_a, const void* b_pre, int accumulate, float* rowstats,
+                                  const float* a_amax, const float* b_amax, float* c_amax, unsigned int* range_flag,
+                                  float adrop_p, int adrop_g1, int adrop_g2, unsigned int adrop_salt,
+                                  float skip_p, int skip_g1, int skip_g2, unsigned int skip_salt,
+                                  void* workspace, long long ws_bytes, hipStream_t stream) {
+  return npvp_gemm_f32_kskip(a_kc, b_kc, M, N, K, A, lda, B, ldb, C, ldc, bias, act, aux_in, aux_out, residual, ldr, drop_p, drop_mode,
+                             drop_g1, drop_g2, seed, salt, alpha, precision, colsum_a, b_pre, accumulate, rowstats, a_amax, b_amax, c_amax,
+                             range_flag, adrop_p, adrop_g1, adrop_g2, adrop_salt, skip_p, skip_g1, skip_g2, skip_salt, 0, workspace, ws_bytes, stream);
+}
+
 extern "C" int npvp_gemm_f32(int a_kc, int b_kc, int M, int N, int K, const float* A, long long lda, const float* B,
                              long long ldb, float* C, long long ldc, const float* bias, int act, const float* aux_in,
                              float* aux_out, const float* residual, long long ldr, float drop_p, int drop_mode,
diff --git a/npvp_amd/csrc/gemm_f16.hip b/npvp_amd/csrc/gemm_f16.hip
--- a/npvp_amd/csrc/gemm_f16.hip
+++ b/npvp_amd/csrc/gemm_f16.hip
@@ -313,7 +313,7 @@
 
 constexpr int GEMM_WGRAD_F16_LDS_BYTES = 2 * (2 * 16 * 128 * 2 + 2 * 16 * 256 * 2);
 
-template <int TM, int TN, int WM, int WN>
+template <int TM, int TN, int WM, int WN, bool KSKIP = false>
 __device__ __forceinline__ void gemm_wgrad_f16_body(const GemmParams& p, char* lds, const int bx, const int by, const int gx) {
   constexpr int NW = WM * WN, THREADS = 64 * NW;
   constexpr int BM = WM * TM * 32, BN = WN * TN * 32;
@@ -373,8 +373,50 @@
   f32x4 cs = {0.f, 0.f, 0.f, 0.f};
   f32x4 cm4 = {0.f, 0.f, 0.f, 0.f};
   f32x4 ra[2], rb[4];
+  const int c0 = z * nk;
+  int nv = nk, kcur = c0, kq = 0, kleft = nk, spg = nk, gbase = c0, lo = c0, hi = c0 + nk;
+  unsigned long long keep = 1ull;
+  if constexpr (KSKIP) {
+    const int spg_ = p.adrop.g1 >> 4;
+    const bool bal = (p.kskip & 4) != 0;
+    if (bal) { lo = 0; hi = nk * p.splits; }
+    const int q_lo = lo / spg_, ng = (hi - 1) / spg_ - q_lo + 1;
+    int j0 = 0;
+    if (ng <= 64) {
+      spg = spg_; gbase = q_lo * spg_;
+      keep = __builtin_amdgcn_ballot_w64(lane < ng && drop_spec_scale(p.adrop, *p.seed, (long long)(q_lo + min(lane, ng - 1)) * p.adrop.g1, 0, 1) != 0.f);
+      int nvt = 0;
+      for (unsigned long long m_ = keep; m_; m_ &= m_ - 1ull) {
+        const int i_ = __builtin_ctzll(m_);
+        nvt += min(gbase + (i_ + 1) * spg, hi) - max(gbase + i_ * spg, lo);
+      }
+      nv = nvt;
+      if (bal) { j0 = (int)((long long)z * nvt / p.splits); nv = (int)((long long)(z + 1) * nvt / p.splits) - j0; }
+    }
+    for (unsigned long long m_ = keep; m_; m_ &= m_ - 1ull) {
+      kq = __builtin_ctzll(m_);
+      const int g0_ = max(gbase + kq * spg, lo), n_ = min(gbase + (kq + 1) * spg, hi) - g0_;
+      if (j0 < n_) { kcur = g0_ + j0; kleft = n_ - j0; break; }
+      j0 -= n_;
+    }
+    if ((p.kskip & 3) == 1 && p.range_flag && ng <= 64) {
+      for (int q_ = 0; q_ < ng; ++q_) {
+        if ((keep >> q_) & 1ull) continue;
+        for (int a_ = max(gbase + q_ * spg, c0); a_ < min(gbase + (q_ + 1) * spg, c0 + nk); ++a_) {
+          const char* pa_ = a_base + (long long)(a_ - c0) * a_step + a_voff;
+          const f32x4 v0_ = *reinterpret_cast<const f32x4*>(pa_), v1_ = *reinterpret_cast<const f32x4*>(pa_ + a_row8);
+          cm4 = __builtin_elementwise_max(cm4, __builtin_elementwise_max(__builtin_elementwise_abs(v0_), __builtin_elementwise_abs(v1_)));
+        }
+      }
+    }
+  }
+#define NPVP_G_NEXT                                                                                         \
+  { if (--kleft > 0) ++kcur;                                                                                \
+    else { const unsigned long long m_ = kq < 63 ? keep >> (kq + 1) : 0ull;                                 \
+           kq += 1 + (m_ ? __builtin_ctzll(m_) : 0); kcur = gbase + kq * spg; kleft = spg; } }
 #define NPVP_G_LOAD(KT)                                                                                     \
-  { const int kt_ = min((KT), nk - 1);                                                                      \
+  { int kt_;                                                                                                \
+    if constexpr (KSKIP) { if ((KT) > 0 && (KT) < nv) NPVP_G_NEXT  kt_ = kcur - c0; } else kt_ = min((KT), nk - 1);  \
     const char* pa_ = a_base + (long long)kt_ * a_step; const char* pb_ = b_base + (long long)kt_ * b_step;  \
     asm volatile("global_load_dwordx4 %0, %1, %2" : "=v"(ra[0]) : "v"(a_voff), "s"(pa_) : "memory");        \
     asm volatile("global_load_dwordx4 %0, %1, %2" : "=v"(ra[1]) : "v"(a_voff), "s"(pa_ + a_row8) : "memory"); \
@@ -387,12 +429,13 @@
   const unsigned long long aseed = p.adrop.thresh ? *p.seed : 0ull;
   const long long arow0 = (long long)z * p.K;
   float am_ = 1.f;
-#define NPVP_G_AMASK(KT) { if (p.adrop.thresh) am_ = drop_spec_scale(p.adrop, aseed, arow0 + 16ll * min((KT), nk - 1), 0, 1); }
+#define NPVP_G_AMASK(KT) { if (p.adrop.thresh) am_ = drop_spec_scale(p.adrop, aseed, KSKIP ? 16ll * kcur : arow0 + 16ll * min((KT), nk - 1), 0, 1); }
 #define NPVP_G_STORE_A(ST) { const float sam_ = sa * am_;                                                                        \
     if (p.range_flag) cm4 = __builtin_elementwise_max(cm4, __builtin_elementwise_max(__builtin_elementwise_abs(ra[0]), __builtin_elementwise_abs(ra[1]))); \
     NPVP_G_STORE((ST) + a_dst, ra[0], sam_, A_PLANE) NPVP_G_STORE((ST) + a_dst + 8 * ROWA, ra[1], sam_, A_PLANE) }
 #define NPVP_G_STORE_B(ST, I) NPVP_G_STORE((ST) + b_dst + (I) * 4 * ROWB, rb[I], sb, B_PLANE)
 
+  if (!KSKIP || nv > 0) {
   NPVP_G_LOAD(0)
   NPVP_G_AMASK(0)
   NPVP_G_WAIT(0, "+v"(ra[0]), "+v"(ra[1]), "+v"(rb[0]), "+v"(rb[1]), "+v"(rb[2]), "+v"(rb[3]))
@@ -408,7 +451,7 @@
     char* nx_ = lds + (NXT) * STAGE;                                                                         \
     NPVP_G_WAIT(3, "+v"(ra[0]), "+v"(ra[1]), "+v"(rb[0]))                                                    \
     NPVP_G_AMASK((KT) + 1)                                                         \
-    if (want_cs && (KT) + 1 < nk) { asm volatile("" ::: "memory"); cs += (ra[0] + ra[1]) * am_; }   \
+    if (want_cs && (KT) + 1 < nv) { asm volatile("" ::: "memory"); cs += (ra[0] + ra[1]) * am_; }   \
     f16x8 fa_[TM][2];                                                                                        \
     _Pragma("unroll") for (int i_ = 0; i_ < TM; ++i_)                                                        \
       _Pragma("unroll") for (int s_ = 0; s_ < 2; ++s_) fa_[i_][s_] = lds_read_tr_pair_h(st_ + fa[i_] + s_ * A_PLANE, 4 * ROWA); \
@@ -429,11 +472,12 @@
   }
 
   int kt = 0;
-  for (; kt + 1 < nk; kt += 2) {
+  for (; kt + 1 < nv; kt += 2) {
     NPVP_G_STEP(kt, 0, 1)
     NPVP_G_STEP(kt + 1, 1, 0)
   }
-  if (kt < nk) NPVP_G_STEP(kt, 0, 1)
+  if (kt < nv) NPVP_G_STEP(kt, 0, 1)
+  }
   asm volatile("s_waitcnt vmcnt(0)" : "+v"(ra[0]), "+v"(ra[1]), "+v"(rb[0]), "+v"(rb[1]), "+v"(rb[2]), "+v"(rb[3]) :: "memory");
   if (p.range_flag) {
     float* red = reinterpret_cast<float*>(lds);
@@ -459,6 +503,7 @@
 #undef NPVP_G_AMASK
 #undef NPVP_G_STORE
 #undef NPVP_G_LOAD
+#undef NPVP_G_NEXT
 
   if (want_cs) {
     float* red = reinterpret_cast<float*>(lds);
@@ -492,15 +537,15 @@
   });
 }
 
-template <int TM, int TN, int WM, int WN>
+template <int TM, int TN, int WM, int WN, bool KSKIP = false>
 __global__ __launch_bounds__(64 * WM * WN, (WM * WN) / 2) void gemm_wgrad_f16_kernel(GemmParams p) {
   __shared__ __attribute__((aligned(16))) char lds[GEMM_WGRAD_F16_LDS_BYTES];
-  gemm_wgrad_f16_body<TM, TN, WM, WN>(p, lds, blockIdx.x, blockIdx.y, gridDim.x);
+  gemm_wgrad_f16_body<TM, TN, WM, WN, KSKIP>(p, lds, blockIdx.x, blockIdx.y, gridDim.x);
 }
 
 struct GemmGroup { GemmParams p[2]; int first[3]; int count[2]; int gx; };
 
-template <int TM, int TN>
+template <int TM, int TN, bool KSKIP = false>
 __global__ __launch_bounds__(256, 2) void gemm_f16_group_kernel(GemmGroup g) {
   constexpr int L0 = gemm_f16_lds_bytes<TM, TN, 2, 2, 3>();
   __shared__ __attribute__((aligned(16))) char lds[L0 > GEMM_WGRAD_F16_LDS_BYTES ? L0 : GEMM_WGRAD_F16_LDS_BYTES];
@@ -511,7 +556,7 @@
     const int lb = b - g.first[1];
     if (lb < g.count[1]) {
       const int by = lb / g.gx;
-      gemm_wgrad_f16_body<2, 4, 2, 2>(g.p[1], lds, lb - by * g.gx, by, g.gx);
+      gemm_wgrad_f16_body<2, 4, 2, 2, KSKIP>(g.p[1], lds, lb - by * g.gx, by, g.gx);
     }
   }
 }
@@ -528,6 +573,7 @@
 static dim3 size_gemm_wgrad_f16(GemmParams& p) {
   p.tiles_m = (p.M + 127) / 128;
   p.tiles_n = (p.N + 255) / 256;
+  if ((p.kskip & 4) && (p.K < 1024 || ((long long)p.K * p.splits + p.adrop.g1 - 1) / p.adrop.g1 > 64)) p.kskip &= 3;
   const int tiles = p.tiles_m * p.tiles_n, rr = reduce_rows_for(p.prev, tiles);
   p.prev.blocks = rr * tiles;
   return dim3(tiles, p.splits + rr);
@@ -535,7 +581,8 @@
 
 void launch_gemm_wgrad_f16(GemmParams& p, hipStream_t stream) {
   const dim3 grid = size_gemm_wgrad_f16(p);
-  NPVP_LAUNCH((gemm_wgrad_f16_kernel<2, 4, 2, 2>), grid, dim3(256), 0, stream, p);
+  if (wgrad_kskips(p)) NPVP_LAUNCH((gemm_wgrad_f16_kernel<2, 4, 2, 2, true>), grid, dim3(256), 0, stream, p);
+  else NPVP_LAUNCH((gemm_wgrad_f16_kernel<2, 4, 2, 2>), grid, dim3(256), 0, stream, p);
 }
 
 static bool deferred_wgrad_args_ok(const char* who, const float* dy, long long lda, const float* x, long long ldb, const float* dw, long long ldc, float adrop_p,
@@ -721,22 +768,36 @@
   return s > 1 ? splitk_workspace_bytes(s, M, N) : 0;
 }
 
+extern "C" int npvp_wgrad_f16_chained_skip(int M, int N, int K, const float* dy, long long lda, const float* x, long long ldb, float* dw,
+                                           long long ldc, float* db, int accumulate, const float* a_amax, const float* b_amax,
+                                           unsigned int* range_flag, float adrop_p, int adrop_g1, int adrop_g2, unsigned int adrop_salt,
+                                           int adrop_kskip, const unsigned long long* seed, const void* prev_job, void* my_job,
+                                           void* workspace, long long ws_bytes, hipStream_t stream) {
+  NPVP_CHECK_ARG(npvp_wgrad_f16_chainable(M, N, K), "wgrad_f16_chained: shape not taken (npvp_wgrad_f16_chainable tells)");
+  NPVP_CHECK_ARG(dy && x && dw && a_amax && b_amax && my_job, "wgrad_f16_chained: null operand / amax slot / job");
+  const int kkind = adrop_kskip & 3;
+  NPVP_CHECK_ARG(adrop_kskip == 0 || ((adrop_kskip & ~7) == 0 && (kkind == 1 || kkind == 2) && adrop_p > 0.f && adrop_p < 1.f && seed && adrop_g1 > 0 && adrop_g2 > 0 &&
+                                      adrop_g1 % 16 == 0),
+                 "wgrad_f16_chained: the K-step skip (1, 2) needs a row-group spec of a multiple of 16 rows and a device seed");
+  if (!deferred_wgrad_args_ok("wgrad_f16_chained", dy, lda, x, ldb, dw, ldc, kkind == 2 ? 0.f : adrop_p, adrop_g1, adrop_g2, seed, workspace, ws_bytes,
+                              npvp_wgrad_f16_chain_workspace_bytes(M, N, K))) return NPVP_ERR_ARG;
+  NPVP_CHECK_ARG(!db || ((uintptr_t)db % 16) == 0, "wgrad_f16_chained: the bias gradient must be 16-byte aligned");
+  const DropSpec spec = make_drop_spec(adrop_p, adrop_salt, 1, adrop_g1, adrop_g2);
+  GemmParams p = deferred_wgrad_params(M, N, K, dy, lda, x, ldb, a_amax, b_amax, range_flag, spec, seed, prev_job, workspace, db != nullptr, accumulate);
+  set_wgrad_kskip(p, adrop_kskip, spec);
+  launch_gemm_wgrad_f16(p, stream);
+  NPVP_CHECK_LAUNCH();
+  leave_reduce_job(p, dw, ldc, db, my_job);
+  return NPVP_OK;
+}
+
 extern "C" int npvp_wgrad_f16_chained(int M, int N, int K, const float* dy, long long lda, const float* x, long long ldb, float* dw,
                                       long long ldc, float* db, int accumulate, const float* a_amax, const float* b_amax,
                                       unsigned int* range_flag, float adrop_p, int adrop_g1, int adrop_g2, unsigned int adrop_salt,
                                       const unsigned long long* seed, const void* prev_job, void* my_job, void* workspace,
                                       long long ws_bytes, hipStream_t stream) {
-  NPVP_CHECK_ARG(npvp_wgrad_f16_chainable(M, N, K), "wgrad_f16_chained: shape not taken (npvp_wgrad_f16_chainable tells)");
-  NPVP_CHECK_ARG(dy && x && dw && a_amax && b_amax && my_job, "wgrad_f16_chained: null operand / amax slot / job");
-  if (!deferred_wgrad_args_ok("wgrad_f16_chained", dy, lda, x, ldb, dw, ldc, adrop_p, adrop_g1, adrop_g2, seed, workspace, ws_bytes,
-                              npvp_wgrad_f16_chain_workspace_bytes(M, N, K))) return NPVP_ERR_ARG;
-  NPVP_CHECK_ARG(!db || ((uintptr_t)db % 16) == 0, "wgrad_f16_chained: the bias gradient must be 16-byte aligned");
-  GemmParams p = deferred_wgrad_params(M, N, K, dy, lda, x, ldb, a_amax, b_amax, range_flag, make_drop_spec(adrop_p, adrop_salt, 1, adrop_g1, adrop_g2),
-                                       seed, prev_job, workspace, db != nullptr, accumulate);
-  launch_gemm_wgrad_f16(p, stream);
-  NPVP_CHECK_LAUNCH();
-  leave_reduce_job(p, dw, ldc, db, my_job);
-  return NPVP_OK;
+  return npvp_wgrad_f16_chained_skip(M, N, K, dy, lda, x, ldb, dw, ldc, db, accumulate, a_amax, b_amax, range_flag, adrop_p, adrop_g1, adrop_g2,
+                                     adrop_salt, 0, seed, prev_job, my_job, workspace, ws_bytes, stream);
 }
 
 extern "C" int npvp_linear_bwd_f16_takes(int R, int N, int K) {
@@ -744,14 +805,14 @@
   return ((v == 2 || v == 3 || v == 4) && npvp_wgrad_f16_chainable(N, K, R)) ? 1 : 0;
 }
 
-extern "C" int npvp_linear_bwd_f16_skip(int R, int N, int K, const float* dy, long long ldy, const float* dy_amax, const void* w_planes_d,
-                                        const float* w_amax, float* dx, long long ldx, int act, const float* aux_in, const float* residual,
-                                        long long ldr, float drop_p, int drop_mode, int drop_g1, int drop_g2, unsigned int drop_salt,
-                                        float* dx_amax, const float* x, long long ldxx, const float* x_amax, float* dw, long long ldw, float* db,
-                                        unsigned int* range_flag, float adrop_p, int adrop_g1, int adrop_g2, unsigned int adrop_salt,
-                                        float skip_p, int skip_g1, int skip_g2, unsigned int skip_salt,
-                                        const unsigned long long* seed, const void* prev_job, void* my_job, void* workspace,
-                                        long long ws_bytes, hipStream_t stream) {
+extern "C" int npvp_linear_bwd_f16_kskip(int R, int N, int K, const float* dy, long long ldy, const float* dy_amax, const void* w_planes_d,
+                                         const float* w_amax, float* dx, long long ldx, int act, const float* aux_in, const float* residual,
+                                         long long ldr, float drop_p, int drop_mode, int drop_g1, int drop_g2, unsigned int drop_salt,
+                                         float* dx_amax, const float* x, long long ldxx, const float* x_amax, float* dw, long long ldw, float* db,
+                                         unsigned int* range_flag, float adrop_p, int adrop_g1, int adrop_g2, unsigned int adrop_salt,
+                                         float skip_p, int skip_g1, int skip_g2, unsigned int skip_salt, int wgrad_kskip,
+                                         const unsigned long long* seed, const void* prev_job, void* my_job, void* workspace,
+                                         long long ws_bytes, hipStream_t stream) {
   NPVP_CHECK_ARG(skip_p >= 0.f && skip_p < 1.f && (skip_p == 0.f || (seed && skip_g1 > 0 && skip_g2 > 0)),
                  "linear_bwd_f16: the row skip needs a device seed and row groups");
   NPVP_CHECK_ARG(npvp_linear_bwd_f16_takes(R, N, K), "linear_bwd_f16: shape not taken (npvp_linear_bwd_f16_takes tells)");
@@ -771,9 +832,12 @@
   d.drop = make_drop_spec(drop_p, drop_salt, drop_mode, drop_g1, drop_g2);
   d.adrop = make_drop_spec(adrop_p, adrop_salt, 1, adrop_g1, adrop_g2);
   d.rskip = make_drop_spec(skip_p, skip_salt, 1, skip_g1, skip_g2);
+  NPVP_CHECK_ARG(wgrad_kskip_args_ok(wgrad_kskip, adrop_p, d.rskip, seed),
+                 "linear_bwd_f16: wgrad_kskip is 0, 1 (with adrop) or 2 (without; the row skip's groups then hold a multiple of 16 rows)");
   d.b_pre = w_planes_d; d.b_pre_plane = (long long)N * K;
   d.a_amax = dy_amax; d.b_amax = w_amax; d.c_amax = dx_amax;
   GemmParams& w = g.p[1] = deferred_wgrad_params(N, K, R, dy, ldy, x, ldxx, dy_amax, x_amax, range_flag, d.adrop, seed, prev_job, workspace, db != nullptr, 1);
+  set_wgrad_kskip(w, wgrad_kskip, d.rskip);
   const dim3 wgrid = size_gemm_wgrad_f16(w);
   const int t128 = ((R + 127) / 128) * ((K + 127) / 128), wwg = (int)wgrid.x * w.splits;
   int v = gemm_f16_variant(R, K, N);
@@ -784,12 +848,31 @@
   g.count[1] = wgrid.x * wgrid.y;
   g.first[2] = g.first[1] + ((g.count[1] + 7) & ~7);
   g.gx = wgrid.x;
-  if (v == 2) NPVP_LAUNCH((gemm_f16_group_kernel<2, 2>), dim3(g.first[2]), dim3(256), 0, stream, g);
-  else if (v == 4) NPVP_LAUNCH((gemm_f16_group_kernel<1, 2>), dim3(g.first[2]), dim3(256), 0, stream, g);
-  else NPVP_LAUNCH((gemm_f16_group_kernel<2, 1>), dim3(g.first[2]), dim3(256), 0, stream, g);
+  const dim3 ggrid(g.first[2]), gblock(256);
+  if (wgrad_kskips(w)) {
+    if (v == 2) NPVP_LAUNCH((gemm_f16_group_kernel<2, 2, true>), ggrid, gblock, 0, stream, g);
+    else if (v == 4) NPVP_LAUNCH((gemm_f16_group_kernel<1, 2, true>), ggrid, gblock, 0, stream, g);
+    else NPVP_LAUNCH((gemm_f16_group_kernel<2, 1, true>), ggrid, gblock, 0, stream, g);
+  } else if (v == 2) NPVP_LAUNCH((gemm_f16_group_kernel<2, 2>), ggrid, gblock, 0, stream, g);
+  else if (v == 4) NPVP_LAUNCH((gemm_f16_group_kernel<1, 2>), ggrid, gblock, 0, stream, g);
+  else NPVP_LAUNCH((gemm_f16_group_kernel<2, 1>), ggrid, gblock, 0, stream, g);
   NPVP_CHECK_LAUNCH();
   leave_reduce_job(w, dw, ldw, db, my_job);
   return NPVP_OK;
+}
+
+extern "C" int npvp_linear_bwd_f16_skip(int R, int N, int K, const float* dy, long long ldy, const float* dy_amax, const void* w_planes_d,
+                                        const float* w_amax, float* dx, long long ldx, int act, const float* aux_in, const float* residual,
+                                        long long ldr, float drop_p, int drop_mode, int drop_g1, int drop_g2, unsigned int drop_salt,
+                                        float* dx_amax, const float* x, long long ldxx, const float* x_amax, float* dw, long long ldw, float* db,
+                                        unsigned int* range_flag, float adrop_p, int adrop_g1, int adrop_g2, unsigned int adrop_salt,
+                                        float skip_p, int skip_g1, int skip_g2, unsigned int skip_salt,
+                                        const unsigned long long* seed, const void* prev_job, void* my_job, void* workspace,
+                                        long long ws_bytes, hipStream_t stream) {
+  return npvp_linear_bwd_f16_kskip(R, N, K, dy, ldy, dy_amax, w_planes_d, w_amax, dx, ldx, act, aux_in, residual, ldr, drop_p, drop_mode,
+                                   drop_g1, drop_g2, drop_salt, dx_amax, x, ldxx, x_amax, dw, ldw, db, range_flag, adrop_p, adrop_g1, adrop_g2,
+                                   adrop_salt, skip_p, skip_g1, skip_g2, skip_salt, (adrop_p == 0.f && skip_p > 0.f && skip_g1 > 0 && skip_g1 % 16 == 0) ? 6 : 0,
+                                   seed, prev_job, my_job, workspace, ws_bytes, stream);
 }
 
 extern "C" int npvp_linear_bwd_f16(int R, int N, int K, const float* dy, long long ldy, const float* dy_amax, const void* w_planes_d,
diff --git a/npvp_amd/ops.py b/npvp_amd/ops.py
--- a/npvp_amd/ops.py
+++ b/npvp_amd/ops.py
@@ -51,11 +51,12 @@
 
 
 class Drop:
-    __slots__ = ("p", "mode", "g1", "g2", "salt")
+    __slots__ = ("p", "mode", "g1", "g2", "salt", "kskip")
 
     def __init__(self, p=0.0, mode=0, g1=1, g2=1):
         self.p, self.mode, self.g1, self.g2 = float(p), mode, g1, g2
         self.salt = _S._cur.rng.next_salt() if p > 0 else 0
+        self.kskip = 0
 
     @property
     def on(self):
@@ -64,7 +65,7 @@
     @classmethod
     def _like(cls, other, mode, g1, g2):
         d = cls.__new__(cls)
-        d.p, d.mode, d.g1, d.g2, d.salt = other.p, mode, g1, g2, other.salt
+        d.p, d.mode, d.g1, d.g2, d.salt, d.kskip = other.p, mode, g1, g2, other.salt, 0
         return d
 
 
@@ -255,7 +256,7 @@
 
 def gemm(a_kc, b_kc, M, N, K, A, lda, B, ldb, out, bias=None, act=0, aux_in=None, aux_out=None, residual=None,
          drop=NO_DROP, alpha=1.0, colsum_a=None, b_pre=None, accumulate=False, rowstats=None, precision=None,
-         replay=False, a_amax=None, b_amax=None, c_amax=None, a_drop=NO_DROP, range_flag=None, row_skip=NO_DROP):
+         replay=False, a_amax=None, b_amax=None, c_amax=None, a_drop=NO_DROP, range_flag=None, row_skip=NO_DROP, wgrad_kskip=0):
     for t in (A, B, out, bias, aux_in, aux_out, residual, colsum_a):
         if t is not None and not (t.is_cuda and t.dtype is torch.float32):
             _chk(t)
@@ -287,7 +288,7 @@
     if GemmProbe.armed:
         kid = _gemm_kernel_id(a_kc, b_kc, M, N, K, prec, planes is not None)
         pe = GemmProbe.begin(kid)
-    rc = lib().npvp_gemm_f32_skip(
+    head = (
         a_kc, b_kc, M, N, K, A.data_ptr(), lda, B.data_ptr(), ldb, out.data_ptr(), out.stride(0),
         None if bias is None else bias.data_ptr(), act, None if aux_in is None else aux_in.data_ptr(),
         None if aux_out is None else aux_out.data_ptr(), None if residual is None else residual.data_ptr(),
@@ -296,10 +297,11 @@
         None if planes is None else planes.data_ptr(), 1 if accumulate else 0, None if rowstats is None else rowstats.data_ptr(),
         None if a_amax is None else a_amax.data_ptr(), None if b_amax is None else b_amax.data_ptr(),
         None if c_amax is None else c_amax.data_ptr(), None if range_flag is None else range_flag.data_ptr(),
-        a_drop.p, a_drop.g1, a_drop.g2, a_drop.salt, row_skip.p, row_skip.g1, row_skip.g2, row_skip.salt,
-        None if ws is None else ws.data_ptr(), wsn, _stream())
+        a_drop.p, a_drop.g1, a_drop.g2, a_drop.salt, row_skip.p, row_skip.g1, row_skip.g2, row_skip.salt)
+    tail = (None if ws is None else ws.data_ptr(), wsn, _stream())
+    rc = lib().npvp_gemm_f32_kskip(*head, wgrad_kskip, *tail) if wgrad_kskip else lib().npvp_gemm_f32_skip(*head, *tail)
     if rc:
-        check(rc, "npvp_gemm_f32_skip")
+        check(rc, "npvp_gemm_f32_kskip" if wgrad_kskip else "npvp_gemm_f32_skip")
     if pe is not None:
         GemmProbe.end(pe, 2.0 * M * N * K, 4.0 * (M * K + N * K + M * N), (a_kc, b_kc), kid)
     return out
@@ -396,7 +398,19 @@
 DROP_PATH_IN_GEMM_ROWS = 1 << 30
 
 
-def linear_wgrad(dy, x, with_bias_grad=False, into=None, into_b=None, dy_amax=None, x_amax=None, a_drop=NO_DROP):
+def wgrad_skip_spec(a_drop, row_skip=NO_DROP):
+    if not (DROP_PATH_SKIP and DROP_PATH_SKIP_WGRAD) or a_drop.kskip:
+        return a_drop
+    src = a_drop if a_drop.on else row_skip
+    if not (src.on and src.mode == 1 and src.g1 % 16 == 0):
+        return a_drop
+    d = Drop._like(src, 1, src.g1, src.g2)
+    d.kskip = (1 if a_drop.on else 2) + (4 if DROP_PATH_SKIP_WGRAD_BALANCE else 0)
+    return d
+
+
+def linear_wgrad(dy, x, with_bias_grad=False, into=None, into_b=None, dy_amax=None, x_amax=None, a_drop=NO_DROP, row_skip=NO_DROP):
+    a_drop = wgrad_skip_spec(a_drop, row_skip)
     R, N = dy.shape
     K = x.shape[1]
     acc = into is not None
@@ -404,7 +418,9 @@
     db = (into_b if acc else torch.empty(N, dtype=torch.float32, device=dy.device)) if with_bias_grad else None
     c = _S._cur
     g = c.range_guard
-    plan = wgrad_plan(N, K, R, GEMM_PRECISION, WGRAD_PRECISION, acc, a_drop.on, g.fallback, g.strict, c.wgrad.in_flush, c.wgrad.enabled,
+    skip_only = a_drop.kskip & 3 == 2
+    mask = NO_DROP if skip_only else a_drop
+    plan = wgrad_plan(N, K, R, GEMM_PRECISION, WGRAD_PRECISION, acc, mask.on, g.fallback, g.strict, c.wgrad.in_flush, c.wgrad.enabled,
                       c.grad_sink.listener is not None, c.chain.enabled, dy.stride(1) == 1 and x.stride(1) == 1 and dw.stride(1) == 1)
     flag = g.flag(dy.device) if plan.watch else None
     if plan.route == "strict":
@@ -423,8 +439,9 @@
     elif plan.route == "chained":
         c.chain.launch(dy, x, dw, db, amax_of(dy, dy_amax), amax_of(x, x_amax), a_drop, flag)
     else:
+        ks = a_drop.kskip if plan.watch else 0
         gemm(0, 0, N, K, R, dy, dy.stride(0), x, x.stride(0), dw, colsum_a=db, accumulate=acc, precision=plan.precision, a_amax=dy_amax,
-             b_amax=x_amax, a_drop=a_drop, range_flag=flag)
+             b_amax=x_amax, a_drop=mask, range_flag=flag, row_skip=a_drop if ks & 3 == 2 else NO_DROP, wgrad_kskip=ks)
     return (dw, db) if with_bias_grad else dw
 
 
@@ -452,7 +469,7 @@
     if not plan.fused:
         dx = linear_dgrad(dy, w, act=act, aux_in=aux_in, drop=drop, residual=residual, dy_amax=dy_amax, dx_amax=dx_amax, a_drop=a_drop,
                           row_skip=row_skip)
-        gw, gb = _lin_grads(dy, x, w, b, sk, a_drop=a_drop, plan=plan)
+        gw, gb = _lin_grads(dy, x, w, b, sk, a_drop=a_drop, plan=plan, row_skip=row_skip)
         return dx, gw, gb
     planes, w_amax = pl
     gw, gb = sk[0][0], (sk[1][0] if has_b else None)
@@ -471,8 +488,12 @@
             drop.salt, _ptr(dx_amax), x.data_ptr(), x.stride(0), x_amax.data_ptr(), gw.data_ptr(), gw.stride(0), _ptr(gb),
             _ptr(c.range_guard.flag(dev)), a_drop.p, a_drop.g1, a_drop.g2, a_drop.salt)
     tail = (_ptr(seed), prev_addr, job_addr, ws.data_ptr(), wsn, st)
-    if row_skip.on:
-        check(lib().npvp_linear_bwd_f16_skip(*head, row_skip.p, row_skip.g1, row_skip.g2, row_skip.salt, *tail), "npvp_linear_bwd_f16_skip")
+    ks = wgrad_skip_spec(a_drop, row_skip).kskip
+    skip = (row_skip.p, row_skip.g1, row_skip.g2, row_skip.salt)
+    if ks not in (0, 6) or (row_skip.on and ks == 0 and row_skip.g1 % 16 == 0):
+        check(lib().npvp_linear_bwd_f16_kskip(*head, *skip, ks, *tail), "npvp_linear_bwd_f16_kskip")
+    elif row_skip.on:
+        check(lib().npvp_linear_bwd_f16_skip(*head, *skip, *tail), "npvp_linear_bwd_f16_skip")
     else:
         check(lib().npvp_linear_bwd_f16(*head, *tail), "npvp_linear_bwd_f16")
     GemmProbe.end(pe, 4.0 * R * N * K, 4.0 * (2 * R * N + 2 * R * K + 2 * N * K), (1, 0), 8)
@@ -901,8 +922,9 @@
         return dx, dw, db, dres, None, None
 
 
-def _lin_grads(dy, x, w, b, sk, a_drop=NO_DROP, plan=None):
+def _lin_grads(dy, x, w, b, sk, a_drop=NO_DROP, plan=None, row_skip=NO_DROP):
     has_b = b is not None
+    a_drop = wgrad_skip_spec(a_drop, row_skip)
     if plan is None:
         plan = linear_bwd_plan(dy.shape[0], dy.shape[1], x.shape[1], GEMM_PRECISION, _sunk(sk, has_b), _S._cur.wgrad.enabled)
     if not plan.sunk:
@@ -1391,6 +1413,8 @@
 
 MID_BWD_N2 = True
 DROP_PATH_SKIP = True
+DROP_PATH_SKIP_WGRAD = True
+DROP_PATH_SKIP_WGRAD_BALANCE = True
 
 
 def mlpdwbn_fused_supported(R, C, hid, Co, H, W):
diff --git a/npvp_amd/sched.py b/npvp_amd/sched.py
--- a/npvp_amd/sched.py
+++ b/npvp_amd/sched.py
@@ -487,9 +487,13 @@
         job_addr, prev_addr = self.job_slot(st)
         seed = self.ctx.rng.seed_tensor(dy.device) if a_drop.on else None
         pe = GemmProbe.begin(6)
-        check(lib().npvp_wgrad_f16_chained(N, K, R, _ptr(dy), dy.stride(0), _ptr(x), x.stride(0), _ptr(dw), dw.stride(0), _ptr(db), 1,
-                                           _ptr(dy_amax), _ptr(x_amax), _ptr(flag), a_drop.p, a_drop.g1, a_drop.g2, a_drop.salt,
-                                           _ptr(seed), prev_addr, job_addr, _ptr(ws), wsn, st), "npvp_wgrad_f16_chained")
+        head = (N, K, R, _ptr(dy), dy.stride(0), _ptr(x), x.stride(0), _ptr(dw), dw.stride(0), _ptr(db), 1, _ptr(dy_amax), _ptr(x_amax),
+                _ptr(flag), a_drop.p, a_drop.g1, a_drop.g2, a_drop.salt)
+        tail = (_ptr(seed), prev_addr, job_addr, _ptr(ws), wsn, st)
+        if a_drop.on and a_drop.kskip:
+            check(lib().npvp_wgrad_f16_chained_skip(*head, a_drop.kskip, *tail), "npvp_wgrad_f16_chained_skip")
+        else:
+            check(lib().npvp_wgrad_f16_chained(*head, *tail), "npvp_wgrad_f16_chained")
         GemmProbe.end(pe, 2.0 * N * K * R, 4.0 * (N * R + K * R + N * K), (0, 0), 6)
         self.job_added(st, None, (ws, dw, db), None)
 
```

Result: no change. 8527 (median of 6 runs) (+0.4%).
